# vanilladucky/sde_sampler_lrds

Hardware: AMD Instinct MI355X
Metric: particle-steps/sec (batch*n_steps/wall) + log-Z abs-err vs ref (higher is better)
Workload: dtype f32; 1 GPU; ManyModes d=128 K=4, RDS gmm-ref, VP(0.1,10), EI integrator, 65536 particles x 256 steps per GPU, FourierMLP(4x64) drift, x0 and noise drawn by the engine (Philox); particles_per_gpu=65536, sde_steps=256, parallelism=particle-sharded x1

## Files before the change

### sde_sampler_lrds_amd/csrc/cmcd_inst.hip

```cpp
#include "cmcd_kernel.hpp"

__device__ inline void block_coords(int local, int KB, int& part, int& o, int& i) {
  const int j = local & 7, lane = (local >> 3) & 63, blk = local >> 10;
  part = (local >> 9) & 1;
  const int kb = blk % KB, to = blk / KB;
  o = 16 * to + (lane & 15);
  i = 16 * (2 * kb + (j >> 2)) + 4 * (lane >> 4) + (j & 3);
}
__device__ inline _Float16 split_part(float w, int part) {
  const _Float16 hi = static_cast<_Float16>(w);
  return part == 0 ? hi : static_cast<_Float16>((w - static_cast<float>(hi)) * 2048.0f);
}
__global__ void k_logreg_images(const float* X, const float* y, int n, int dw, int NT, float* image, float* y_pad) {
  const int KB = sd_kb(NT), RKB = sd_lr_row_kb(n);
  const int n_logit = sd_lr_logit_floats(NT, n) * 2, n_grad = sd_lr_grad_floats(NT, n) * 2;
  _Float16* img = reinterpret_cast<_Float16*>(image);
  for (int idx = blockIdx.x * blockDim.x + threadIdx.x; idx < n_logit + n_grad; idx += gridDim.x * blockDim.x) {
    int part, o, i, row, col;
    if (idx < n_logit) {
      block_coords(idx, KB, part, o, i);
      row = o; col = i;
    } else {
      block_coords(idx - n_logit, RKB, part, o, i);
      row = i; col = o;
    }
    float v = 0.0f;
    if (row < n) v = (col < dw) ? X[static_cast<size_t>(row) * dw + col] : (col == dw ? 1.0f : 0.0f);
    img[idx] = split_part(v, part);
    if (idx < 32 * RKB) y_pad[idx] = (idx < n) ? y[idx] : 0.0f;
  }
}
__global__ void k_pack_square(const float* P, const float* loc, int d, int NT, float* out, float* loc_pad) {
  const int KB = sd_kb(NT);
  _Float16* img = reinterpret_cast<_Float16*>(out);
  for (int idx = blockIdx.x * blockDim.x + threadIdx.x; idx < NT * KB * 1024; idx += gridDim.x * blockDim.x) {
    int part, o, i;
    block_coords(idx, KB, part, o, i);
    img[idx] = split_part((o < d && i < d) ? P[static_cast<size_t>(o) * d + i] : 0.0f, part);
    if (idx < 16 * NT) loc_pad[idx] = idx < d ? loc[idx] : 0.0f;
  }
}
int sd_launch_logreg_images(const float* X, const float* y, int n, int dw, int NT, float* image, float* y_pad, hipStream_t s) {
  hipLaunchKernelGGL(k_logreg_images, dim3(96), dim3(256), 0, s, X, y, n, dw, NT, image, y_pad);
  return static_cast<int>(hipGetLastError());
}
int sd_launch_pack_square(const float* P, const float* loc, int d, int NT, float* out, float* loc_pad, hipStream_t s) {
  hipLaunchKernelGGL(k_pack_square, dim3(NT * sd_kb(NT) * 4), dim3(256), 0, s, P, loc, d, NT, out, loc_pad);
  return static_cast<int>(hipGetLastError());
}
```

### sde_sampler_lrds_amd/csrc/prep_kernels.hip

```cpp
#include "sim_device.hpp"
#include "prep_kernels.hpp"

__global__ void __launch_bounds__(256) k_weight_scales(PackArgs a) {
  __shared__ float red[256];
  float* sc = a.out + sd_off_scales(a.NT);
  {
    const int l = blockIdx.x;
    const float* W = l == 0 ? a.w_in : (l == 1 ? a.w_h1 : (l == 2 ? a.w_h2 : a.w_out));
    const int n = (l == 0 || l == 3) ? SD_H * a.d : SD_H * SD_H;
    float m = 0.0f;
    for (int i = threadIdx.x; i < n; i += 256) {
      const float v = __builtin_fabsf(W[i]);
      m = (v <= 3.0e38f) ? fmaxf(m, v) : m;
    }
    red[threadIdx.x] = m;
    __syncthreads();
    for (int s = 128; s > 0; s >>= 1) {
      if (threadIdx.x < s) red[threadIdx.x] = fmaxf(red[threadIdx.x], red[threadIdx.x + s]);
      __syncthreads();
    }
    if (threadIdx.x == 0) {
      const float mx = red[0];
      int e = 0;
      if (mx > 0.0f && (mx < 9.765625e-4f || mx >= 16384.0f)) {
        int ex;
        frexpf(mx, &ex);
        e = 1 - ex;
        e = e > 100 ? 100 : (e < -100 ? -100 : e);
      }
      sc[l] = ldexpf(1.0f, e);
      sc[4 + l] = ldexpf(1.0f, -e);
    }
    __syncthreads();
  }
}

__global__ void k_pack_mlp(PackArgs a) {
  const int NT = a.NT;
  const float* scales = a.transpose ? a.scales : a.out + sd_off_scales(NT);
  const int n_half = sd_lds_weight_floats(NT) * 2;
  const int n_bias = a.transpose ? 0 : 3 * 64 + 16 * NT;
  _Float16* img = reinterpret_cast<_Float16*>(a.out);
  for (int idx = blockIdx.x * blockDim.x + threadIdx.x; idx < n_half + n_bias; idx += gridDim.x * blockDim.x) {
    if (idx < n_half) {
      const int fl = idx >> 1;
      const float* W;
      int n_out, n_in, KB, base, layer;
      if (fl < sd_off_wh1(NT)) {
        W = a.w_in; n_out = SD_H; n_in = a.d; KB = sd_kb(NT); base = sd_off_win(NT); layer = 0;
      } else if (fl < sd_off_wh2(NT)) {
        W = a.w_h1; n_out = SD_H; n_in = SD_H; KB = 2; base = sd_off_wh1(NT); layer = 1;
      } else if (fl < sd_off_wout(NT)) {
        W = a.w_h2; n_out = SD_H; n_in = SD_H; KB = 2; base = sd_off_wh2(NT); layer = 2;
      } else {
        W = a.w_out; n_out = a.d; n_in = SD_H; KB = 2; base = sd_off_wout(NT); layer = 3;
      }
      const int local = idx - 2 * base;
      const int j = local & 7;
      const int lane = (local >> 3) & 63;
      const int part = (local >> 9) & 1;
      const int blk = local >> 10;
      const int kb = blk % KB, to = blk / KB;
      const int o = 16 * to + (lane & 15);
      const int i = 16 * (2 * kb + (j >> 2)) + 4 * (lane >> 4) + (j & 3);
      float w = 0.0f;
      if (o < n_out && i < n_in) {
        if (!a.transpose) {
          w = W[static_cast<size_t>(o) * n_in + i] * scales[layer];
        } else {
          const float* Wt = layer == 0 ? a.w_out : (layer == 1 ? a.w_h2 : (layer == 2 ? a.w_h1 : a.w_in));
          w = Wt[static_cast<size_t>(i) * n_out + o] * scales[3 - layer];
        }
      }
      const _Float16 hi = static_cast<_Float16>(w);
      img[idx] = part == 0 ? hi : static_cast<_Float16>((w - static_cast<float>(hi)) * 2048.0f);
    } else {
      const int b = idx - n_half;
      float v;
      if (b < 64) v = a.b_in[b] * scales[0];
      else if (b < 128) v = a.b_h1[b - 64] * scales[1];
      else if (b < 192) v = a.b_h2[b - 128] * scales[2];
      else v = (b - 192 < a.d) ? a.b_out[b - 192] * scales[3] : 0.0f;
      a.out[sd_off_bias(NT) + b] = v;
    }
  }
}

__device__ inline float gelu_exact(float v) { return (v * 0.5f) * (1.0f + erff(v * 0.70710678118654752440f)); }

__global__ void __launch_bounds__(64) k_time_embed(TimeEmbedArgs a) {
  __shared__ float e[128];
  __shared__ float hbuf[2][64];
  const int k = blockIdx.x, j = threadIdx.x;
  const float t = a.t_direct ? a.t_value : a.coef[static_cast<size_t>(k) * SDENG_NCOEF + a.col];
  const float arg = (a.te.coeff[j] * t) + a.te.phase[j];
  e[j] = sinf(arg);
  e[64 + j] = cosf(arg);
  __syncthreads();
  const float* in = e;
  int n_in = 128, cur = 0;
  for (int l = 0; l < a.te.n_hidden; ++l) {
    const float* W = a.te.w[l] + static_cast<size_t>(j) * n_in;
    float acc = 0.0f;
    for (int i = 0; i < n_in; ++i) acc = __builtin_fmaf(W[i], in[i], acc);
    acc += a.te.b[l][j];
    hbuf[cur][j] = gelu_exact(acc);
    __syncthreads();
    in = hbuf[cur];
    n_in = 64;
    cur ^= 1;
  }
  if (j < a.te.dim_out) {
    const float* W = a.te.w_out + static_cast<size_t>(j) * 64;
    float acc = 0.0f;
    for (int i = 0; i < 64; ++i) acc = __builtin_fmaf(W[i], in[i], acc);
    acc += a.te.b_out[j];
    if (a.clip > 0.0f) acc = clampf(acc, a.clip);
    a.out[static_cast<size_t>(k) * a.te.dim_out + j] = acc;
  }
}

__global__ void __launch_bounds__(128) k_same_var(const float* vars, int K, int d, float* same_var) {
  int differ = 0;
  for (int i = threadIdx.x; i < K * d; i += 128) differ |= vars[i] != vars[i % d];
  differ = __syncthreads_or(differ);
  if (threadIdx.x == 0) same_var[0] = differ ? 0.0f : 1.0f;
}

__global__ void __launch_bounds__(128) k_ref_tables(RefTabArgs a) {
  __shared__ float red[128];
  const int k = blockIdx.x / a.K, c = blockIdx.x % a.K;
  const float S = a.coef[static_cast<size_t>(k) * SDENG_NCOEF + 9];
  const float VA = a.coef[static_cast<size_t>(k) * SDENG_NCOEF + 10];
  const float S2 = a.coef[static_cast<size_t>(k) * SDENG_NCOEF + 11];
  const bool centred = a.centred && a.K == SD_KREG && a.same_var[0] != 0.0f;
  float* tm = a.tab + (static_cast<size_t>(k) * a.K + c) * 2 * a.dpad;
  float* tv = tm + a.dpad;
  float ls = 0.0f, quad = 0.0f;
  for (int f = threadIdx.x; f < a.dpad; f += 128) {
    float mean = 0.0f, iv = 0.0f, cen = 0.0f;
    if (f < a.d) {
      mean = S * a.means[static_cast<size_t>(c) * a.d + f];
      const float var = VA + S2 * a.vars[static_cast<size_t>(c) * a.d + f];
      iv = 1.0f / var;
      ls += logf(var);
      if (centred) {
        float sum = 0.0f;
        for (int j = 0; j < SD_KREG; ++j) sum += a.means[static_cast<size_t>(j) * a.d + f];
        cen = S * (sum * (1.0f / SD_KREG));
      }
    }
    if (centred) {
      const float dm = mean - cen;
      quad = __builtin_fmaf(dm * dm, iv, quad);
      tm[f] = dm * iv;
      tv[f] = c == 0 ? iv : (c == 1 ? cen : 0.0f);
    } else {
      tm[f] = mean;
      tv[f] = iv;
    }
  }
  red[threadIdx.x] = ls;
  __syncthreads();
  for (int s = 64; s > 0; s >>= 1) {
    if (threadIdx.x < s) red[threadIdx.x] += red[threadIdx.x + s];
    __syncthreads();
  }
  const float ls_sum = red[0];
  __syncthreads();
  red[threadIdx.x] = quad;
  __syncthreads();
  for (int s = 64; s > 0; s >>= 1) {
    if (threadIdx.x < s) red[threadIdx.x] += red[threadIdx.x + s];
    __syncthreads();
  }
  if (threadIdx.x == 0) {
    float wsum = 0.0f;
    for (int i = 0; i < a.K; ++i) wsum += a.weights ? a.weights[i] : 1.0f;
    const float w = (a.weights ? a.weights[c] : 1.0f) / wsum;
    float* cs = a.consts + (static_cast<size_t>(k) * a.K + c) * 2;
    cs[0] = 0.5f * ls_sum;
    cs[1] = centred ? logf(w) - 0.5f * red[0] : logf(w);
  }
}

__global__ void __launch_bounds__(256) k_ref_full_tables(RefFullArgs a) {
  __shared__ float invd[128];
  __shared__ float red[256];
  const int k = blockIdx.x / a.K, c = blockIdx.x % a.K;
  const float S = a.coef ? a.coef[static_cast<size_t>(k) * SDENG_NCOEF + 9] : 1.0f;
  const float VA = a.coef ? a.coef[static_cast<size_t>(k) * SDENG_NCOEF + 10] : 0.0f;
  const float S2 = a.coef ? a.coef[static_cast<size_t>(k) * SDENG_NCOEF + 11] : 1.0f;
  const int KB = sd_kb(a.NT);
  const int img_floats = a.NT * KB * 512;
  float ls = 0.0f;
  for (int j = threadIdx.x; j < 128; j += 256) {
    float iv = 0.0f;
    if (j < a.d) {
      const float var = VA + S2 * a.eigvals[static_cast<size_t>(c) * a.d + j];
      iv = 1.0f / var;
      ls += logf(var);
    }
    invd[j] = iv;
  }
  red[threadIdx.x] = ls;
  __syncthreads();
  for (int s = 128; s > 0; s >>= 1) {
    if (threadIdx.x < s) red[threadIdx.x] += red[threadIdx.x + s];
    __syncthreads();
  }
  const size_t blk = static_cast<size_t>(k) * a.K + c;
  if (threadIdx.x == 0) {
    float wsum = 0.0f;
    for (int i = 0; i < a.K; ++i) wsum += a.weights ? a.weights[i] : 1.0f;
    a.consts[blk * 2 + 0] = 0.5f * red[0];
    a.consts[blk * 2 + 1] = logf((a.weights ? a.weights[c] : 1.0f) / wsum);
  }
  for (int f = threadIdx.x; f < a.dpad; f += 256) a.means_out[blk * a.dpad + f] = f < a.d ? S * a.means[static_cast<size_t>(c) * a.d + f] : 0.0f;
  const float* U = a.eigvecs + static_cast<size_t>(c) * a.d * a.d;
  _Float16* img = reinterpret_cast<_Float16*>(a.images + blk * img_floats);
  for (int idx = threadIdx.x; idx < img_floats * 2; idx += 256) {
    const int j8 = idx & 7, lane = (idx >> 3) & 63, part = (idx >> 9) & 1, tb = idx >> 10;
    const int kb = tb % KB, to = tb / KB;
    const int o = 16 * to + (lane & 15);
    const int i = 16 * (2 * kb + (j8 >> 2)) + 4 * (lane >> 4) + (j8 & 3);
    float p = 0.0f;
    if (o < a.d && i < a.d) {
      const float* uo = U + static_cast<size_t>(o) * a.d;
      const float* ui = U + static_cast<size_t>(i) * a.d;
      for (int j = 0; j < a.d; ++j) p = __builtin_fmaf(uo[j] * invd[j], ui[j], p);
    }
    const _Float16 hi = static_cast<_Float16>(p);
    img[idx] = part == 0 ? hi : static_cast<_Float16>((p - static_cast<float>(hi)) * 2048.0f);
  }
}

__global__ void __launch_bounds__(256) k_ref_mm_tables(RefMMArgs a) {
  __shared__ float cbar[128], ivs[128];
  const int k = blockIdx.x;
  const float S = a.coef[static_cast<size_t>(k) * SDENG_NCOEF + 9];
  const float VA = a.coef[static_cast<size_t>(k) * SDENG_NCOEF + 10];
  const float S2 = a.coef[static_cast<size_t>(k) * SDENG_NCOEF + 11];
  const int KBX = sd_kb(a.NT), KBK = (a.kt + 1) / 2;
  for (int f = threadIdx.x; f < 128; f += 256) {
    float c = 0.0f, iv = 0.0f;
    if (f < a.d) {
      for (int j = 0; j < a.K; ++j) c += a.means[static_cast<size_t>(j) * a.d + f];
      c = S * (c / static_cast<float>(a.K));
      iv = 1.0f / (VA + S2 * a.vars[f]);
      if (a.same_var[0] == 0.0f) iv = __builtin_nanf("");
    }
    cbar[f] = c;
    ivs[f] = iv;
    if (f < a.dpad) {
      a.centre[(static_cast<size_t>(k) * 2 + 0) * a.dpad + f] = c;
      a.centre[(static_cast<size_t>(k) * 2 + 1) * a.dpad + f] = iv;
    }
  }
  __syncthreads();
  if (threadIdx.x < 64) {
    const int c = threadIdx.x;
    float b = -INFINITY;
    if (c < a.K) {
      float wsum = 0.0f;
      for (int i = 0; i < a.K; ++i) wsum += a.weights ? a.weights[i] : 1.0f;
      double q = 0.0;
      for (int f = 0; f < a.d; ++f) {
        const float mu = S * a.means[static_cast<size_t>(c) * a.d + f] - cbar[f];
        q += static_cast<double>(mu * mu) * ivs[f];
      }
      b = logf((a.weights ? a.weights[c] : 1.0f) / wsum) - 0.5f * static_cast<float>(q);
    }
    a.consts[static_cast<size_t>(k) * 64 + c] = b;
  }
  const int n_logit = a.kt * KBX * 1024, n_mean = a.NT * KBK * 1024;
  _Float16* img = reinterpret_cast<_Float16*>(a.images + static_cast<size_t>(k) * ((n_logit + n_mean) / 2));
  for (int idx = threadIdx.x; idx < n_logit + n_mean; idx += 256) {
    const bool logit = idx < n_logit;
    const int local = logit ? idx : idx - n_logit, KB = logit ? KBX : KBK;
    const int j8 = local & 7, lane = (local >> 3) & 63, part = (local >> 9) & 1, blk = local >> 10;
    const int kb = blk % KB, to = blk / KB;
    const int o = 16 * to + (lane & 15);
    const int i = 16 * (2 * kb + (j8 >> 2)) + 4 * (lane >> 4) + (j8 & 3);
    const int comp = logit ? o : i, f = logit ? i : o;
    float v = 0.0f;
    if (comp < a.K && f < a.d) {
      const float mu = S * a.means[static_cast<size_t>(comp) * a.d + f] - cbar[f];
      v = logit ? mu * ivs[f] : mu;
    }
    const _Float16 hi = static_cast<_Float16>(v);
    img[idx] = part == 0 ? hi : static_cast<_Float16>((v - static_cast<float>(hi)) * 2048.0f);
  }
}

__global__ void __launch_bounds__(128) k_dist_tables(DistTabArgs a) {
  __shared__ float red[2][128];
  const int c = blockIdx.x;
  float* tm = a.tab + static_cast<size_t>(c) * 2 * a.dpad;
  float* tv = tm + a.dpad;
  float lv = 0.0f, lsig = 0.0f;
  for (int f = threadIdx.x; f < a.dpad; f += 128) {
    float mean = 0.0f, iv = 0.0f;
    if (f < a.d) {
      mean = a.loc[static_cast<size_t>(c) * a.d + f];
      const float sc = a.scale[static_cast<size_t>(c) * a.d + f];
      const float var = sc * sc;
      iv = 1.0f / var;
      lv += logf(var);
      lsig += logf(sc);
    }
    tm[f] = mean;
    tv[f] = iv;
  }
  red[0][threadIdx.x] = lv;
  red[1][threadIdx.x] = lsig;
  __syncthreads();
  for (int s = 64; s > 0; s >>= 1) {
    if (threadIdx.x < s) {
      red[0][threadIdx.x] += red[0][threadIdx.x + s];
      red[1][threadIdx.x] += red[1][threadIdx.x + s];
    }
    __syncthreads();
  }
  if (threadIdx.x == 0) {
    float* cs = a.consts + static_cast<size_t>(c) * 4;
    cs[0] = 0.5f * red[0][0];
    cs[2] = red[1][0] + static_cast<float>(a.d) * 0.91893853320467274178f;
    if (a.weights) {
      float wsum = 0.0f;
      for (int i = 0; i < a.K; ++i) wsum += a.weights[i];
      const float pr = a.weights[c] / wsum;
      cs[1] = logf(pr);
      const float eps = 1.1920928955078125e-07f;
      float lse_m = -INFINITY, lse_s = 0.0f;
      for (int i = 0; i < a.K; ++i) {
        const float li = logf(fminf(fmaxf(a.weights[i] / wsum, eps), 1.0f - eps));
        const float m = fmaxf(lse_m, li);
        lse_s = lse_s * expf(lse_m - m) + expf(li - m);
        lse_m = m;
      }
      const float lc = logf(fminf(fmaxf(pr, eps), 1.0f - eps));
      cs[3] = lc - (lse_m + logf(lse_s));
    } else {
      cs[1] = 0.0f;
      cs[3] = 0.0f;
    }
  }
}

__device__ void gmm_logp_partial(const DistEvalArgs& a, const float* x, int c0, int cs, float& m_run, float& l_run) {
  const DistDev& ds = a.ds;
  m_run = -INFINITY;
  l_run = 0.0f;
  for (int c = c0; c < ds.k; c += cs) {
    const float* tm = ds.tab + static_cast<size_t>(c) * 2 * a.dpad;
    const float* tv = tm + a.dpad;
    double acc = 0.0;
    for (int f = 0; f < a.d; ++f) {
      const float dl = x[f] - tm[f];
      acc += static_cast<double>(dl * dl) * tv[f];
    }
    const float part = static_cast<float>(acc);
    float lp = (-0.5f * part) - ds.consts[4 * c + 2];
    if (ds.kind == SDENG_DIST_GAUSS_DIAG) { m_run = lp; l_run = 1.0f; break; }
    lp += ds.consts[4 * c + 3];
    const float m_new = fmaxf(m_run, lp);
    l_run = l_run * expf(m_run - m_new) + expf(lp - m_new);
    m_run = m_new;
  }
}

__device__ float logreg_loglik_partial(const DistEvalArgs& a, const float* x, int n0, int ns) {
  const DistDev& ds = a.ds;
  const int dw = a.d - 1;
  const float c = x[dw];
  const float eps = 1.1920928955078125e-07f;
  float ll = 0.0f;
  for (int n = n0; n < ds.k; n += ns) {
    const float* Xn = ds.aux0 + static_cast<size_t>(n) * dw;
    float lg = 0.0f;
    for (int f = 0; f < dw; ++f) lg = __builtin_fmaf(Xn[f], x[f], lg);
    lg += c;
    float p = 1.0f / (1.0f + expf(-lg));
    p = fminf(fmaxf(p, ds.p3), 1.0f - ds.p3);
    p = fminf(fmaxf(p, eps), 1.0f - eps);
    const float l2 = logf(p) - log1pf(-p);
    const float y = ds.aux1[n];
    ll -= (1.0f - y) * l2 + (fmaxf(-l2, 0.0f) + log1pf(expf(-fabsf(l2))));
  }
  return ll;
}

__device__ float logreg_logprior(const DistEvalArgs& a, const float* x) {
  const DistDev& ds = a.ds;
  const int dw = a.d - 1;
  float prior = 0.0f;
  const float lws = logf(ds.p0), two_ws2 = 2.0f * (ds.p0 * ds.p0);
  for (int f = 0; f < dw; ++f) prior += (-(x[f] * x[f]) / two_ws2 - lws) - 0.91893853320467274178f;
  const float dc = x[dw] - ds.p1;
  prior += (-(dc * dc) / (2.0f * (ds.p2 * ds.p2)) - logf(ds.p2)) - 0.91893853320467274178f;
  return prior;
}

__device__ float gauss_full_m2_partial(const DistEvalArgs& a, const float* x, int i0, int is) {
  const DistDev& ds = a.ds;
  float m2 = 0.0f;
  for (int i = i0; i < a.d; i += is) {
    float yi = 0.0f;
    const float* Li = ds.aux1 + static_cast<size_t>(i) * a.d;
    for (int j = 0; j <= i; ++j) yi = __builtin_fmaf(Li[j], x[j] - ds.aux0[j], yi);
    m2 = __builtin_fmaf(yi, yi, m2);
  }
  return m2;
}

__device__ float dist_logp_row(const DistEvalArgs& a, const float* x) {
  const int d = a.d;
  const DistDev& ds = a.ds;
  float out = 0.0f;
  if (ds.kind == SDENG_DIST_GMM_DIAG || ds.kind == SDENG_DIST_GAUSS_DIAG) {
    float m_run, l_run;
    gmm_logp_partial(a, x, 0, 1, m_run, l_run);
    out = m_run + logf(l_run);
  } else if (ds.kind == SDENG_DIST_ISO_GAUSS) {
    double acc = 0.0;
    for (int f = 0; f < d; ++f) {
      const float dl = x[f] - ds.p0;
      acc += static_cast<double>(dl) * dl;
    }
    const float part = static_cast<float>(acc);
    out = ds.p2 - (0.5f * part) / ds.p3;
  } else if (ds.kind == SDENG_DIST_PHI4) {
    const float coef = ds.p0 * static_cast<float>(d);
    double gsum = 0.0, vsum = 0.0;
    float prev = 0.0f;
    for (int f = 0; f < d; ++f) {
      const float xv = x[f];
      const float dl = xv - prev;
      gsum += (dl * dl) * 0.5f;
      const float om = 1.0f - xv * xv;
      vsum += (om * om) * 0.25f + ds.p1 * xv;
      prev = xv;
    }
    gsum += (prev * prev) * 0.5f;
    const float grad = static_cast<float>(gsum), V = static_cast<float>(vsum);
    out = (-ds.p2) * (grad * coef + V / coef);
  } else if (ds.kind == SDENG_DIST_GAUSS_FULL) {
    const float m2 = gauss_full_m2_partial(a, x, 0, 1);
    out = -0.5f * (static_cast<float>(d) * 1.8378770664093453f + m2) - ds.p0;
  } else if (ds.kind == SDENG_DIST_LOGREG) {
    out = logreg_loglik_partial(a, x, 0, 1) + logreg_logprior(a, x);
  }
  else if (ds.kind == SDENG_DIST_RINGS) {
    const float r = sqrtf(x[0] * x[0] + x[1] * x[1]);
    float wsum = 0.0f;
    for (int k = 0; k < ds.k; ++k) wsum += ds.aux1[k];
    const float ls = logf(ds.p0), var = ds.p0 * ds.p0;
    float m_run = -INFINITY, l_run = 0.0f;
    for (int k = 0; k < ds.k; ++k) {
      const float dl = r - ds.aux0[k];
      const float lp = ((-(dl * dl) / (2.0f * var)) - ls) - 0.91893853320467274178f + logf(ds.aux1[k] / wsum);
      const float m_new = fmaxf(m_run, lp);
      l_run = l_run * expf(m_run - m_new) + expf(lp - m_new);
      m_run = m_new;
    }
    out = ((m_run + logf(l_run)) - 1.8378770664093453f) - logf(r);
  } else if (ds.kind == SDENG_DIST_CHECKERBOARD) {
    out = -INFINITY;
    for (int k = 0; k < ds.k; ++k) {
      const float* lo = ds.aux0 + 2 * k;
      const float* hi = ds.aux1 + 2 * k;
      const bool in = (lo[0] <= x[0]) & (hi[0] > x[0]) & (lo[1] <= x[1]) & (hi[1] > x[1]);
      out = in ? ds.tab[k] : out;
    }
  }
  if (ds.clip > 0.0f) out = clampf(out, ds.clip);
  return out;
}

__device__ void dist_score_row(const DistEvalArgs& a, const float* x, float* sc) {
  const int d = a.d;
  const DistDev& ds = a.ds;
  if (ds.kind == SDENG_DIST_GMM_DIAG) {
    float m_run = -INFINITY, l_run = 0.0f;
    for (int f = 0; f < d; ++f) sc[f] = 0.0f;
    for (int c = 0; c < ds.k; ++c) {
      const float* tm = ds.tab + static_cast<size_t>(c) * 2 * a.dpad;
      const float* tv = tm + a.dpad;
      float part = 0.0f;
      for (int f = 0; f < d; ++f) {
        const float dl = x[f] - tm[f];
        part = __builtin_fmaf(dl * dl, tv[f], part);
      }
      float lp = ((-0.5f * part) - ds.p0) - ds.consts[4 * c + 0];
      lp = ds.consts[4 * c + 1] + lp;
      const float m_new = fmaxf(m_run, lp);
      const float so = expf(m_run - m_new), pk = expf(lp - m_new);
      l_run = l_run * so + pk;
      m_run = m_new;
      for (int f = 0; f < d; ++f) sc[f] = __builtin_fmaf(pk, (tm[f] - x[f]) * tv[f], sc[f] * so);
    }
    const float inv = 1.0f / l_run;
    for (int f = 0; f < d; ++f) sc[f] *= inv;
  } else if (ds.kind == SDENG_DIST_GAUSS_DIAG) {
    for (int f = 0; f < d; ++f) sc[f] = -((x[f] - ds.tab[f]) * ds.tab[a.dpad + f]);
  } else if (ds.kind == SDENG_DIST_ISO_GAUSS) {
    for (int f = 0; f < d; ++f) sc[f] = (ds.p0 - x[f]) / (ds.p1 * ds.p1);
  } else if (ds.kind == SDENG_DIST_PHI4) {
    const float coef = ds.p0 * static_cast<float>(d);
    for (int f = 0; f < d; ++f) {
      const float xv = x[f];
      const float xl = f > 0 ? x[f - 1] : 0.0f, xr = f < d - 1 ? x[f + 1] : 0.0f;
      float g = (ds.p1 - xv * (1.0f - xv * xv)) / coef;
      g = g + coef * ((2.0f * xv - xr) - xl);
      sc[f] = (-ds.p2) * g;
    }
  } else if (ds.kind == SDENG_DIST_GAUSS_FULL) {
    for (int i = 0; i < d; ++i) {
      float acc = 0.0f;
      const float* Pi = ds.tab + static_cast<size_t>(i) * d;
      for (int j = 0; j < d; ++j) acc = __builtin_fmaf(Pi[j], x[j] - ds.aux0[j], acc);
      sc[i] = -acc;
    }
  } else if (ds.kind == SDENG_DIST_LOGREG) {
    const int dw = d - 1;
    const float c = x[dw];
    const float eps = 1.1920928955078125e-07f;
    for (int f = 0; f < dw; ++f) sc[f] = -x[f] / (ds.p0 * ds.p0);
    float gc = -(c - ds.p1) / (ds.p2 * ds.p2);
    for (int n = 0; n < ds.k; ++n) {
      const float* Xn = ds.aux0 + static_cast<size_t>(n) * dw;
      float lg = 0.0f;
      for (int f = 0; f < dw; ++f) lg = __builtin_fmaf(Xn[f], x[f], lg);
      lg += c;
      const float p = 1.0f / (1.0f + expf(-lg));
      const float pc = fminf(fmaxf(p, ds.p3), 1.0f - ds.p3);
      const float pcc = fminf(fmaxf(pc, eps), 1.0f - eps);
      const bool pass = (p >= ds.p3) && (p <= 1.0f - ds.p3) && (pc >= eps) && (pc <= 1.0f - eps);
      const float l2 = logf(pcc) - log1pf(-pcc);
      const float sg = 1.0f / (1.0f + expf(-l2));
      float r = (ds.aux1[n] - sg) * (1.0f / pcc + 1.0f / (1.0f - pcc)) * (p * (1.0f - p));
      r = pass ? r : 0.0f;
      for (int f = 0; f < dw; ++f) sc[f] = __builtin_fmaf(r, Xn[f], sc[f]);
      gc += r;
    }
    sc[dw] = gc;
  } else if (ds.kind == SDENG_DIST_RINGS) {
    const f32x4 r = rings_score(f32x4{x[0], x[1], 0.0f, 0.0f}, ds, 0);
    sc[0] = r[0];
    sc[1] = r[1];
  } else if (ds.kind == SDENG_DIST_CHECKERBOARD) {
    sc[0] = 0.0f;
    sc[1] = 0.0f;
  }
}

#define SD_EVAL_ROWS 64
#define SD_EVAL_THREADS 256
#define SD_EVAL_RED_FLOATS (SD_EVAL_THREADS * 2)

__device__ inline const float* stage_rows(const float* x, int B, int d, float* sh) {
  const int row0 = blockIdx.x * SD_EVAL_ROWS, stride = d | 1, tid = threadIdx.x;
  const int rows = B - row0 < SD_EVAL_ROWS ? B - row0 : SD_EVAL_ROWS;
  const float* src = x + static_cast<size_t>(row0) * d;
  if ((d & 3) == 0) {
    const int d4 = d >> 2, n4 = rows * d4;
    const float inv = 1.0f / static_cast<float>(d4);
    const f32x4* src4 = reinterpret_cast<const f32x4*>(src);
    for (int base = tid; base < n4; base += 4 * SD_EVAL_THREADS) {
      f32x4 v[4];
#pragma unroll
      for (int j = 0; j < 4; ++j) {
        const int i4 = base + j * SD_EVAL_THREADS;
        v[j] = i4 < n4 ? src4[i4] : f32x4{0.0f, 0.0f, 0.0f, 0.0f};
      }
#pragma unroll
      for (int j = 0; j < 4; ++j) {
        const int i4 = base + j * SD_EVAL_THREADS;
        if (i4 < n4) {
          const int r = static_cast<int>((static_cast<float>(i4) + 0.5f) * inv);
          float* dst = sh + r * stride + 4 * (i4 - r * d4);
          dst[0] = v[j][0]; dst[1] = v[j][1]; dst[2] = v[j][2]; dst[3] = v[j][3];
        }
      }
    }
  } else {
    const int n = rows * d;
    const float inv = 1.0f / static_cast<float>(d);
    for (int base = tid; base < n; base += 8 * SD_EVAL_THREADS) {
      float v[8];
#pragma unroll
      for (int j = 0; j < 8; ++j) {
        const int i = base + j * SD_EVAL_THREADS;
        v[j] = i < n ? src[i] : 0.0f;
      }
#pragma unroll
      for (int j = 0; j < 8; ++j) {
        const int i = base + j * SD_EVAL_THREADS;
        if (i < n) {
          const int r = static_cast<int>((static_cast<float>(i) + 0.5f) * inv);
          sh[r * stride + (i - r * d)] = v[j];
        }
      }
    }
  }
  __syncthreads();
  return sh + (tid & 63) * stride;
}

__device__ float dist_logp_block(const DistEvalArgs& a, const float* x, float* red) {
  const int w = threadIdx.x >> 6, lane = threadIdx.x & 63;
  constexpr int NW = SD_EVAL_THREADS / 64;
  const DistDev& ds = a.ds;
  if (ds.kind == SDENG_DIST_GMM_DIAG && ds.k > 1) {
    float m_run, l_run;
    gmm_logp_partial(a, x, w, NW, m_run, l_run);
    red[2 * threadIdx.x] = m_run;
    red[2 * threadIdx.x + 1] = l_run;
    __syncthreads();
    float out = 0.0f;
    if (w == 0) {
      for (int j = 1; j < NW; ++j) {
        const float mj = red[2 * (64 * j + lane)], lj = red[2 * (64 * j + lane) + 1];
        const float m_new = fmaxf(m_run, mj);
        l_run = l_run * expf(m_run - m_new) + lj * expf(mj - m_new);
        m_run = m_new;
      }
      out = m_run + logf(l_run);
      if (ds.clip > 0.0f) out = clampf(out, ds.clip);
    }
    __syncthreads();
    return out;
  }
  if (ds.kind == SDENG_DIST_LOGREG) {
    const float ll = logreg_loglik_partial(a, x, w, NW);
    red[threadIdx.x] = ll;
    __syncthreads();
    float out = 0.0f;
    if (w == 0) {
      float sum = ll;
      for (int j = 1; j < NW; ++j) sum += red[64 * j + lane];
      out = sum + logreg_logprior(a, x);
      if (ds.clip > 0.0f) out = clampf(out, ds.clip);
    }
    __syncthreads();
    return out;
  }
  if (ds.kind == SDENG_DIST_GAUSS_FULL) {
    const float m2 = gauss_full_m2_partial(a, x, w, NW);
    red[threadIdx.x] = m2;
    __syncthreads();
    float out = 0.0f;
    if (w == 0) {
      float sum = m2;
      for (int j = 1; j < NW; ++j) sum += red[64 * j + lane];
      out = -0.5f * (static_cast<float>(a.d) * 1.8378770664093453f + sum) - ds.p0;
      if (ds.clip > 0.0f) out = clampf(out, ds.clip);
    }
    __syncthreads();
    return out;
  }
  return w == 0 ? dist_logp_row(a, x) : 0.0f;
}

__global__ void __launch_bounds__(SD_EVAL_THREADS) k_dist_eval(DistEvalArgs a) {
  extern __shared__ float sh[];
  float* red = sh + SD_EVAL_ROWS * (a.d | 1);
  const float* x = stage_rows(a.x, a.B, a.d, sh);
  const int row = blockIdx.x * SD_EVAL_ROWS + (threadIdx.x & 63);
  const bool writer = threadIdx.x < 64 && row < a.B;
  if (a.logp_out) {
    const float lp = dist_logp_block(a, x, red);
    if (writer) a.logp_out[row] = lp;
  }
  if (a.score_out && writer) dist_score_row(a, x, a.score_out + static_cast<size_t>(row) * a.d);
}

constexpr int sd_move_rows(int move) { return move == SD_MOVE_RWMH ? 2 : 5; }
__device__ inline void tempered_eval(const MovesArgs& a, float w, const float* y, float* g_out, float* tmp, float& lp_out) {
  const bool both = a.prior.ds.kind != SDENG_DIST_NONE;
  const float lp1 = dist_logp_row(a.target, y);
  dist_score_row(a.target, y, g_out);
  if (!both) {
    lp_out = lp1;
    return;
  }
  const float lp0 = dist_logp_row(a.prior, y);
  dist_score_row(a.prior, y, tmp);
  lp_out = (1.0f - w) * lp0 + w * lp1;
  for (int f = 0; f < a.d; ++f) g_out[f] = (1.0f - w) * tmp[f] + w * g_out[f];
}

template <int MOVE>
__global__ void __launch_bounds__(64) k_chain_moves(MovesArgs a, int chains_per_block) {
  constexpr bool LANGEVIN = MOVE == SD_MOVE_LANGEVIN;
  constexpr uint32_t Z_STREAM = LANGEVIN ? 2u : 6u, U_STREAM = Z_STREAM + 1u;
  extern __shared__ float sh[];
  const int tid = threadIdx.x, d = a.d, stride = d | 1;
  const int chain = blockIdx.x * chains_per_block + tid;
  if (tid >= chains_per_block || chain >= a.B) return;
  const bool ula = LANGEVIN && a.ula;
  float* xr = sh + (tid * sd_move_rows(MOVE) + 0) * stride;
  float* gr = xr + stride;
  float* pr = xr + (LANGEVIN ? 2 : 1) * stride;
  float* gp = pr + stride;
  float* tmp = gp + stride;
  for (int f = 0; f < d; ++f) {
    xr[f] = a.x[static_cast<size_t>(chain) * d + f];
    if constexpr (LANGEVIN) gr[f] = a.grad[static_cast<size_t>(chain) * d + f];
  }
  float lp = a.lp[chain], step = a.step[chain], acc = 0.0f, last = 1.0f;
  const float w = LANGEVIN && a.t ? a.t[chain] : 1.0f;
  const uint32_t cidx = static_cast<uint32_t>(a.chain0 + chain);
  const float log_target = a.target_acc > 0.0f ? logf(a.target_acc) : 0.0f;
  for (int m = 0; m < a.K; ++m) {
    const float sd = sqrtf(2.0f * step);
    for (int f0 = 0; f0 < d; f0 += 4) {
      f32x4 z;
      if (a.z) {
        for (int r = 0; r < 4; ++r) z[r] = f0 + r < d ? a.z[(static_cast<size_t>(m) * a.B + chain) * d + f0 + r] : 0.0f;
      } else {
        z = philox_normal4(cidx, static_cast<uint32_t>(m), static_cast<uint32_t>(f0 >> 2), Z_STREAM, a.seed_lo, a.seed_hi);
      }
      for (int r = 0; r < 4 && f0 + r < d; ++r) {
        if constexpr (LANGEVIN) pr[f0 + r] = sd * z[r] + (xr[f0 + r] + step * gr[f0 + r]);
        else pr[f0 + r] = xr[f0 + r] + step * z[r];
      }
    }
    float lp_p, log_acc = 0.0f;
    if constexpr (LANGEVIN) {
      tempered_eval(a, w, pr, gp, tmp, lp_p);
      if (!ula) {
        float qf = 0.0f, qb = 0.0f;
        for (int f = 0; f < d; ++f) {
          const float df = pr[f] - (xr[f] + step * gr[f]);
          const float db = xr[f] - (pr[f] + step * gp[f]);
          qf += df * df;
          qb += db * db;
        }
        const float var = 2.0f * step;
        const float joint_prop = lp_p - (-0.5f * qf) / var, joint_orig = lp - (-0.5f * qb) / var;
        log_acc = joint_prop - joint_orig;
      }
    } else {
      lp_p = dist_logp_row(a.target, pr);
      log_acc = lp_p - lp;
    }
    bool accept = true;
    if (!ula) {
      float uu;
      if (a.u) {
        uu = a.u[static_cast<size_t>(m) * a.B + chain];
      } else {
        uint32_t r4[4];
        philox4x32_10(cidx, 0u, static_cast<uint32_t>(m), U_STREAM, a.seed_lo, a.seed_hi, r4);
        uu = u01(r4[0]);
      }
      accept = logf(uu) < log_acc;
    }
    if (accept) {
      for (int f = 0; f < d; ++f) {
        xr[f] = pr[f];
        if constexpr (LANGEVIN) gr[f] = gp[f];
      }
      lp = lp_p;
    }
    if (!ula && a.target_acc > 0.0f) {
      if (log_acc - log_target > 0.04879016416943205f) step = step * 1.01f;
      if (log_target - log_acc > 0.05129329438755058f) step = step / 1.01f;
    }
    if (!ula) last = expf(fminf(0.0f, log_acc));
    if (m >= a.keep_from) {
      if (!ula) acc += last;
      if (a.samples) {
        float* dst = a.samples + (static_cast<size_t>(m - a.keep_from) * a.B + chain) * d;
        for (int f = 0; f < d; ++f) dst[f] = xr[f];
      }
    }
  }
  for (int f = 0; f < d; ++f) {
    a.x[static_cast<size_t>(chain) * d + f] = xr[f];
    if constexpr (LANGEVIN) a.grad[static_cast<size_t>(chain) * d + f] = gr[f];
  }
  a.lp[chain] = lp;
  a.step[chain] = step;
  if (a.acc_sum) a.acc_sum[chain] = acc;
  if (a.acc_last) a.acc_last[chain] = last;
}

__global__ void __launch_bounds__(SD_EVAL_THREADS) k_terminal(TerminalArgs a) {
  extern __shared__ float sh[];
  float* red = sh + SD_EVAL_ROWS * (a.d | 1);
  const float* x = stage_rows(a.x, a.B, a.d, sh);
  const int row = blockIdx.x * SD_EVAL_ROWS + (threadIdx.x & 63);
  float term = 0.0f;
  if (a.use_ref) {
    DistEvalArgs e;
    e.ds = a.ref; e.B = a.B; e.d = a.d; e.dpad = a.dpad;
    term = dist_logp_block(e, x, red);
  }
  if (a.use_target) {
    DistEvalArgs e;
    e.ds = a.target; e.B = a.B; e.d = a.d; e.dpad = a.dpad;
    term = term - dist_logp_block(e, x, red);
  }
  if (threadIdx.x < 64 && row < a.B) a.rnd[row] += term;
}

__device__ inline float block_reduce(float v, float* sh, bool is_max) {
  const int lane = threadIdx.x & 63, w = threadIdx.x >> 6;
  for (int o = 32; o > 0; o >>= 1) {
    const float t = __shfl_xor(v, o, 64);
    v = is_max ? fmaxf(v, t) : v + t;
  }
  if (lane == 0) sh[w] = v;
  __syncthreads();
  float r = sh[0];
  for (int i = 1; i < (blockDim.x >> 6); ++i) r = is_max ? fmaxf(r, sh[i]) : r + sh[i];
  __syncthreads();
  return r;
}

__global__ void __launch_bounds__(256) k_logz_partial(const float* rnd, long long B, float* partials) {
  __shared__ float sh[4];
  float mx = -INFINITY, s1 = 0.0f;
  for (long long i = blockIdx.x * 256ll + threadIdx.x; i < B; i += gridDim.x * 256ll) {
    const float v = -rnd[i];
    mx = fmaxf(mx, v);
    s1 += v;
  }
  mx = block_reduce(mx, sh, true);
  s1 = block_reduce(s1, sh, false);
  if (threadIdx.x == 0) {
    partials[2 * blockIdx.x + 0] = mx;
    partials[2 * blockIdx.x + 1] = s1;
  }
}

__global__ void __launch_bounds__(256) k_logz_partial2(const float* rnd, long long B, const float* partials, int nb,
                                                      float* partials2) {
  __shared__ float sh[4];
  float mx = -INFINITY, s1 = 0.0f;
  for (int i = 0; i < nb; ++i) {
    mx = fmaxf(mx, partials[2 * i]);
    s1 += partials[2 * i + 1];
  }
  const float mean = s1 / static_cast<float>(B);
  float se = 0.0f, se2 = 0.0f, sv = 0.0f;
  for (long long i = blockIdx.x * 256ll + threadIdx.x; i < B; i += gridDim.x * 256ll) {
    const float v = -rnd[i];
    const float ex = expf(v - mx);
    se += ex;
    se2 = __builtin_fmaf(ex, ex, se2);
    const float dv = v - mean;
    sv = __builtin_fmaf(dv, dv, sv);
  }
  se = block_reduce(se, sh, false);
  se2 = block_reduce(se2, sh, false);
  sv = block_reduce(sv, sh, false);
  if (threadIdx.x == 0) {
    partials2[3 * blockIdx.x + 0] = se;
    partials2[3 * blockIdx.x + 1] = se2;
    partials2[3 * blockIdx.x + 2] = sv;
  }
}

__global__ void k_logz_final(const float* partials, const float* partials2, int nb, long long B, float* stats) {
  if (threadIdx.x != 0 || blockIdx.x != 0) return;
  float mx = -INFINITY, s1 = 0.0f, se = 0.0f, se2 = 0.0f, sv = 0.0f;
  for (int i = 0; i < nb; ++i) {
    mx = fmaxf(mx, partials[2 * i]);
    s1 += partials[2 * i + 1];
    se += partials2[3 * i];
    se2 += partials2[3 * i + 1];
    sv += partials2[3 * i + 2];
  }
  const float fB = static_cast<float>(B);
  stats[0] = s1 / fB;
  stats[1] = (__builtin_isinf(mx) ? mx : (mx + logf(se))) - logf(fB);
  stats[2] = B > 1 ? sv / (fB - 1.0f) : 0.0f;
  stats[3] = (se * se) / se2 / fB;
  stats[4] = mx;
  stats[5] = se;
  stats[6] = se2;
  stats[7] = s1;
}

__global__ void k_softmax_weights(const float* rnd, long long B, const float* stats, float* w) {
  const long long i = blockIdx.x * static_cast<long long>(blockDim.x) + threadIdx.x;
  if (i >= B) return;
  w[i] = expf((-rnd[i]) - stats[4]) / stats[5];
}

__global__ void k_philox(unsigned seed_lo, unsigned seed_hi, int step, long long particle0, int B, int d, unsigned stream_id,
                         float* out) {
  const int nj = (d + 3) / 4;
  const long long idx = blockIdx.x * static_cast<long long>(blockDim.x) + threadIdx.x;
  if (idx >= static_cast<long long>(B) * nj) return;
  const int row = static_cast<int>(idx / nj), jb = static_cast<int>(idx % nj);
  const f32x4 z = philox_normal4(static_cast<uint32_t>(particle0 + row), static_cast<uint32_t>(step) + blockIdx.y, static_cast<uint32_t>(jb),
                                 stream_id, seed_lo, seed_hi);
  float* o = out + static_cast<size_t>(blockIdx.y) * B * d;
  for (int e = 0; e < 4; ++e)
    if (4 * jb + e < d) o[static_cast<size_t>(row) * d + 4 * jb + e] = z[e];
}

__global__ void k_sample_x0(X0Dev q, unsigned seed_lo, unsigned seed_hi, long long particle0, int B, int d, float* out) {
  const int nj = (d + 3) / 4;
  const long long idx = blockIdx.x * static_cast<long long>(blockDim.x) + threadIdx.x;
  if (idx >= static_cast<long long>(B) * nj) return;
  const int row = static_cast<int>(idx / nj), jb = static_cast<int>(idx % nj);
  const f32x4 x = x0_quad(q, static_cast<uint32_t>(particle0 + row), jb, d, seed_lo, seed_hi);
  for (int e = 0; e < 4; ++e)
    if (4 * jb + e < d) out[static_cast<size_t>(row) * d + 4 * jb + e] = x[e];
}
#define SD_X0_FULL_ROWS 64
__global__ void __launch_bounds__(256) k_sample_x0_full(const float* loc, const float* L, unsigned seed_lo, unsigned seed_hi, long long particle0,
                                                       int B, int d, float* out) {
  extern __shared__ float sh[];
  const int nj = (d + 3) / 4, zs = 4 * nj + 1, ls = d | 1;
  float* z = sh;
  float* Lt = sh + SD_X0_FULL_ROWS * zs;
  const int row0 = blockIdx.x * SD_X0_FULL_ROWS;
  for (int i = threadIdx.x; i < d * d; i += 256) {
    const int f = i / d, j = i - f * d;
    Lt[j * ls + f] = L[i];
  }
  for (int i = threadIdx.x; i < SD_X0_FULL_ROWS * nj; i += 256) {
    const int r = i / nj, jb = i - r * nj;
    const f32x4 v = philox_normal4(static_cast<uint32_t>(particle0 + row0 + r), 0u, static_cast<uint32_t>(jb), SD_X0_STREAM, seed_lo, seed_hi);
    for (int e = 0; e < 4; ++e) z[r * zs + 4 * jb + e] = v[e];
  }
  __syncthreads();
  const int rows = B - row0 < SD_X0_FULL_ROWS ? B - row0 : SD_X0_FULL_ROWS;
  for (int i = threadIdx.x; i < rows * d; i += 256) {
    const int r = i / d, f = i - r * d;
    float acc = 0.0f;
    for (int j = 0; j <= f; ++j) acc = __builtin_fmaf(Lt[j * ls + f], z[r * zs + j], acc);
    out[static_cast<size_t>(row0) * d + i] = loc[f] + acc;
  }
}
int sd_launch_sample_x0(const sdeng_dist& ds, unsigned lo, unsigned hi, long long p0, int B, int d, float* out, hipStream_t s) {
  if (ds.kind == SDENG_DIST_GAUSS_FULL) {
    const size_t lds = (static_cast<size_t>(SD_X0_FULL_ROWS) * (4 * ((d + 3) / 4) + 1) + static_cast<size_t>(d) * (d | 1)) * sizeof(float);
    if (lds > 160 * 1024) return static_cast<int>(hipErrorInvalidValue);
    if (lds > 64 * 1024) (void)hipFuncSetAttribute(reinterpret_cast<const void*>(k_sample_x0_full), hipFuncAttributeMaxDynamicSharedMemorySize, static_cast<int>(lds));
    hipLaunchKernelGGL(k_sample_x0_full, dim3((B + SD_X0_FULL_ROWS - 1) / SD_X0_FULL_ROWS), dim3(256), lds, s, ds.loc, ds.aux, lo, hi, p0, B, d, out);
  } else {
    X0Dev q;
    q.kind = ds.kind; q.loc = ds.loc; q.scale = ds.scale; q.p0 = ds.p0; q.p1 = ds.p1;
    const long long n = static_cast<long long>(B) * ((d + 3) / 4);
    hipLaunchKernelGGL(k_sample_x0, dim3(static_cast<unsigned>((n + 255) / 256)), dim3(256), 0, s, q, lo, hi, p0, B, d, out);
  }
  return static_cast<int>(hipGetLastError());
}

int sd_launch_pack(const PackArgs& a, hipStream_t s) {
  const int total = sd_lds_weight_floats(a.NT) * 2 + (a.transpose ? 0 : 3 * 64 + 16 * a.NT);
  if (!a.transpose) hipLaunchKernelGGL(k_weight_scales, dim3(4), dim3(256), 0, s, a);
  hipLaunchKernelGGL(k_pack_mlp, dim3((total + 255) / 256), dim3(256), 0, s, a);
  return static_cast<int>(hipGetLastError());
}
int sd_launch_time_embed(const TimeEmbedArgs& a, int N, hipStream_t s) {
  hipLaunchKernelGGL(k_time_embed, dim3(N), dim3(64), 0, s, a);
  return static_cast<int>(hipGetLastError());
}
int sd_launch_ref_tables(const RefTabArgs& a, int N, hipStream_t s) {
  hipLaunchKernelGGL(k_same_var, dim3(1), dim3(128), 0, s, a.vars, a.K, a.d, a.same_var);
  hipLaunchKernelGGL(k_ref_tables, dim3(N * a.K), dim3(128), 0, s, a);
  return static_cast<int>(hipGetLastError());
}
int sd_launch_ref_full_tables(const RefFullArgs& a, int N, hipStream_t s) {
  hipLaunchKernelGGL(k_ref_full_tables, dim3(N * a.K), dim3(256), 0, s, a);
  return static_cast<int>(hipGetLastError());
}
int sd_launch_ref_mm_tables(const RefMMArgs& a, int N, hipStream_t s) {
  hipLaunchKernelGGL(k_same_var, dim3(1), dim3(128), 0, s, a.vars, a.K, a.d, a.same_var);
  hipLaunchKernelGGL(k_ref_mm_tables, dim3(N), dim3(256), 0, s, a);
  return static_cast<int>(hipGetLastError());
}
int sd_launch_dist_tables(const DistTabArgs& a, hipStream_t s) {
  hipLaunchKernelGGL(k_dist_tables, dim3(a.K), dim3(128), 0, s, a);
  return static_cast<int>(hipGetLastError());
}
int sd_launch_dist_eval(const DistEvalArgs& a, hipStream_t s) {
  hipLaunchKernelGGL(k_dist_eval, dim3((a.B + SD_EVAL_ROWS - 1) / SD_EVAL_ROWS), dim3(SD_EVAL_THREADS), (SD_EVAL_ROWS * (a.d | 1) + SD_EVAL_RED_FLOATS) * sizeof(float), s, a);
  return static_cast<int>(hipGetLastError());
}
int sd_launch_moves(const MovesArgs& a, int move, hipStream_t s) {
  const size_t row_bytes = static_cast<size_t>(sd_move_rows(move)) * (a.d | 1) * sizeof(float);
  int cpb = 64;
  while (cpb > 8 && cpb * row_bytes > 150 * 1024) cpb /= 2;
  return sd_launch_kernel(move == SD_MOVE_RWMH ? k_chain_moves<SD_MOVE_RWMH> : k_chain_moves<SD_MOVE_LANGEVIN>, (a.B + cpb - 1) / cpb, 64,
                          cpb * row_bytes, s, a, cpb);
}
int sd_launch_terminal(const TerminalArgs& a, hipStream_t s) {
  hipLaunchKernelGGL(k_terminal, dim3((a.B + SD_EVAL_ROWS - 1) / SD_EVAL_ROWS), dim3(SD_EVAL_THREADS), (SD_EVAL_ROWS * (a.d | 1) + SD_EVAL_RED_FLOATS) * sizeof(float), s, a);
  return static_cast<int>(hipGetLastError());
}
int sd_launch_logz(const float* rnd, long long B, float* stats, float* weights, float* scratch, hipStream_t s) {
  int nb = static_cast<int>((B + 256 * 8 - 1) / (256 * 8));
  if (nb > SD_LOGZ_MAX_BLOCKS) nb = SD_LOGZ_MAX_BLOCKS;
  if (nb < 1) nb = 1;
  float* p1 = scratch;
  float* p2 = scratch + 2 * SD_LOGZ_MAX_BLOCKS;
  hipLaunchKernelGGL(k_logz_partial, dim3(nb), dim3(256), 0, s, rnd, B, p1);
  hipLaunchKernelGGL(k_logz_partial2, dim3(nb), dim3(256), 0, s, rnd, B, p1, nb, p2);
  hipLaunchKernelGGL(k_logz_final, dim3(1), dim3(64), 0, s, p1, p2, nb, B, stats);
  if (weights) hipLaunchKernelGGL(k_softmax_weights, dim3(static_cast<unsigned>((B + 255) / 256)), dim3(256), 0, s, rnd, B, stats, weights);
  return static_cast<int>(hipGetLastError());
}
int sd_launch_philox(unsigned lo, unsigned hi, int step, int n_steps, long long p0, int B, int d, unsigned stream_id, float* out, hipStream_t s) {
  const long long n = static_cast<long long>(B) * ((d + 3) / 4);
  for (int done = 0; done < n_steps; done += 65535) {
    const int chunk = n_steps - done < 65535 ? n_steps - done : 65535;
    hipLaunchKernelGGL(k_philox, dim3(static_cast<unsigned>((n + 255) / 256), chunk), dim3(256), 0, s, lo, hi, step + done, p0, B, d, stream_id,
                       out + static_cast<size_t>(done) * B * d);
  }
  return static_cast<int>(hipGetLastError());
}
```

### sde_sampler_lrds_amd/csrc/prep_kernels.hpp

```cpp
#pragma once
#include "sim_common.hpp"
#include "../../include/sdeng.h"

#define SD_LOGZ_MAX_BLOCKS 1024

struct PackArgs {
  int NT, d;
  const float *w_in, *b_in, *w_h1, *b_h1, *w_h2, *b_h2, *w_out, *b_out;
  float* out;
  int transpose;
  const float* scales;
};

struct TimeEmbedArgs {
  sdeng_time_embed te;
  const float* coef;
  int col;
  int t_direct;
  float t_value;
  float clip;
  float* out;
};

struct RefTabArgs {
  int K, d, dpad;
  const float* coef;
  const float *means, *vars, *weights;
  float* tab;
  float* consts;
  float* same_var;
  int centred;
};

struct RefFullArgs {
  int K, d, dpad, NT;
  const float* coef;
  const float *means, *eigvals, *eigvecs, *weights;
  float* images;
  float* means_out;
  float* consts;
};

struct RefMMArgs {
  int K, d, dpad, NT, kt;
  const float* coef;
  const float *means, *vars, *weights;
  float* images;
  float* centre;
  float* consts;
  float* same_var;
};

struct DistTabArgs {
  int K, d, dpad;
  const float *loc, *scale, *weights;
  float* tab;
  float* consts;
};

struct DistEvalArgs {
  DistDev ds;
  int B, d, dpad;
  const float* x;
  float* logp_out;
  float* score_out;
};

enum { SD_MOVE_LANGEVIN = 0, SD_MOVE_RWMH = 1 };
struct MovesArgs {
  DistEvalArgs prior, target;
  int B, d, K, keep_from, ula;
  float target_acc;
  const float* t;
  float *x, *lp, *grad, *step;
  const float *z, *u;
  unsigned seed_lo, seed_hi;
  long long chain0;
  float* samples;
  float* acc_sum;
  float* acc_last;
};
int sd_launch_moves(const MovesArgs& a, int move, hipStream_t s);

struct TerminalArgs {
  DistDev ref, target;
  int use_ref, use_target;
  int B, d, dpad;
  const float* x;
  float* rnd;
};

int sd_launch_pack(const PackArgs& a, hipStream_t s);
int sd_launch_time_embed(const TimeEmbedArgs& a, int N, hipStream_t s);
int sd_launch_ref_tables(const RefTabArgs& a, int N, hipStream_t s);
int sd_launch_ref_full_tables(const RefFullArgs& a, int N, hipStream_t s);
int sd_launch_dist_tables(const DistTabArgs& a, hipStream_t s);
int sd_launch_dist_eval(const DistEvalArgs& a, hipStream_t s);
int sd_launch_terminal(const TerminalArgs& a, hipStream_t s);
int sd_launch_logz(const float* rnd, long long B, float* stats, float* weights, float* scratch, hipStream_t s);
int sd_launch_philox(unsigned lo, unsigned hi, int step, int n_steps, long long p0, int B, int d, unsigned stream_id, float* out, hipStream_t s);
int sd_launch_sample_x0(const sdeng_dist& ds, unsigned lo, unsigned hi, long long p0, int B, int d, float* out, hipStream_t s);
int sd_launch_ref_mm_tables(const RefMMArgs& a, int N, hipStream_t s);
```

### sde_sampler_lrds_amd/csrc/sdeng_api.hip

```cpp
#include <hip/hip_runtime.h>

#include <algorithm>
#include <cmath>
#include <cstdarg>
#include <cstdio>
#include <cstring>
#include <cstdlib>

#include "../../include/sdeng.h"
#include "prep_kernels.hpp"
#include "sim_kernel.hpp"
#include "cmcd_kernel.hpp"
#include "grad_kernel.hpp"
#include "cmcd_adjoint_kernel.hpp"
#include "metric_kernels.hpp"
#include "tilted_kernel.hpp"

int sd_launch_logreg_images(const float* X, const float* y, int n, int dw, int NT, float* image, float* y_pad, hipStream_t s);
int sd_launch_pack_square(const float* P, const float* loc, int d, int NT, float* out, float* loc_pad, hipStream_t s);

static thread_local char g_err[512] = "";
static int fail(int code, const char* fmt, ...) {
  va_list ap;
  va_start(ap, fmt);
  vsnprintf(g_err, sizeof(g_err), fmt, ap);
  va_end(ap);
  return code;
}
#define SD_HIP(expr)                                                                  \
  do {                                                                                \
    int e_ = (expr);                                                                  \
    if (e_ != 0) return fail(SDENG_E_HIP, "%s failed: %s", #expr, hipGetErrorString(static_cast<hipError_t>(e_))); \
  } while (0)
#define SD_TRY(expr)      \
  do {                    \
    int rc_ = (expr);     \
    if (rc_) return rc_;  \
  } while (0)

extern "C" int sdeng_abi_version(void) { return SDENG_ABI_VERSION; }
extern "C" const char* sdeng_last_error(void) { return g_err; }

static inline size_t align64(size_t n_floats) { return (n_floats + 63) & ~static_cast<size_t>(63); }
static inline int pad16(int d) { return 16 * ((d + 15) / 16); }
static inline float half_d_log_2pi(int d) { return static_cast<float>(0.5 * d * std::log(2.0 * M_PI)); }
struct Seed {
  unsigned lo, hi;
};
static inline Seed split_seed(uint64_t seed) { return {static_cast<unsigned>(seed & 0xFFFFFFFFull), static_cast<unsigned>(seed >> 32)}; }
static int check_abi(const sdeng_desc* d) {
  return d->abi_version == SDENG_ABI_VERSION ? 0 : fail(SDENG_E_INVALID, "ABI version %d, library has %d", d->abi_version, SDENG_ABI_VERSION);
}
static int check_lerp_prior(const sdeng_desc* d) {
  if (d->net.ctrl_kind == SDENG_CTRL_LERP && d->prior.kind != SDENG_DIST_ISO_GAUSS)
    return fail(SDENG_E_UNSUPPORTED, "LerpCtrl needs an IsotropicGauss prior (kind %d given)", d->prior.kind);
  return 0;
}
static int ref_components(const sdeng_desc* d) {
  return d->ref.kind == SDENG_REF_NONE ? 0 : (d->ref.kind == SDENG_REF_GAUSS_DIAG ? 1 : d->ref.k);
}
static bool score_like(int ctrl_kind) {
  return ctrl_kind == SDENG_CTRL_SCORE || ctrl_kind == SDENG_CTRL_LERP || ctrl_kind == SDENG_CTRL_CANCEL_DRIFT;
}
static int in_loop_score(int target_kind) {
  if (target_kind == SDENG_DIST_GMM_DIAG || target_kind == SDENG_DIST_RINGS) return SC_GMM;
  if (target_kind == SDENG_DIST_PHI4) return SC_PHI4;
  if (target_kind == SDENG_DIST_LOGREG) return SC_LOGREG;
  return -1;
}

struct KernelKey {
  int fam, nt, p[4];
  sd_launcher fn;
};
static int select_kernel(KernelKey& k, int fam, int nt, int p0 = 0, int p1 = 0, int p2 = 0, int p3 = 0) {
  static const char* const kFamily[] = {"k_simulate", "k_ctrl_forward", "k_simulate_split", "k_euler", "k_simulate_cmcd", "k_ctrl_vjp", "k_kl_adjoint", "k_cmcd_kl_adjoint"};
  k = KernelKey{fam, nt, {p0, p1, p2, p3}, nullptr};
  const uint32_t key = sd_key(fam, nt, p0, p1, p2, p3);
  const SdKernelEntry* end = sd_registry + sd_registry_size;
  const SdKernelEntry* e = std::lower_bound(sd_registry, end, key, [](const SdKernelEntry& x, uint32_t v) { return x.key < v; });
  if (e == end || e->key != key)
    return fail(SDENG_E_UNSUPPORTED, "no kernel instance %s<NT=%d, %d, %d, %d, %d>", kFamily[fam], nt, p0, p1, p2, p3);
  k.fn = e->fn;
  return 0;
}
static int launch_timed(const sdeng_desc* d, const KernelKey& k, const void* args, hipStream_t s) {
  if (d->ev_start) SD_HIP(hipEventRecord(static_cast<hipEvent_t>(d->ev_start), s));
  SD_HIP(k.fn(args, s));
  if (d->ev_stop) SD_HIP(hipEventRecord(static_cast<hipEvent_t>(d->ev_stop), s));
  return 0;
}

static int tiles_exact(int d) { return (d + 15) / 16; }
static int tiles_of(const sdeng_desc* d) {
  const int nt = tiles_exact(d->d);
  return (d->ref.kind == SDENG_REF_GMM_FULL && (nt == 5 || nt == 7)) ? nt + 1 : nt;
}

static size_t dist_floats(const sdeng_dist& ds, int dpad) {
  if (ds.kind == SDENG_DIST_GMM_DIAG) return align64(static_cast<size_t>(ds.k) * 2 * dpad) + align64(static_cast<size_t>(ds.k) * 4);
  if (ds.kind == SDENG_DIST_GAUSS_DIAG) return align64(2 * dpad) + align64(4);
  return 0;
}

static bool split_eligible(const sdeng_desc* d, int DT) {
  return (d->flags & SDENG_FLAG_SPLIT_TILES) && d->B <= 8192 && DT >= 5 && d->net.ctrl_kind == SDENG_CTRL_CLIPPED &&
         (d->form == SDENG_FORM_LIN || d->form == SDENG_FORM_EM) && !d->noise_in &&
         (d->ref.kind == SDENG_REF_NONE || d->ref.kind == SDENG_REF_GAUSS_DIAG || (d->ref.kind == SDENG_REF_GMM_DIAG && d->ref.k <= 4));
}

static int share_room(int DT) { return (160 * 1024 - static_cast<int>(sizeof(float)) * sd_lds_weight_floats(DT)) / 2 / static_cast<int>(sizeof(float)); }
static int mm_piece(int K, int DT) {
  const int kt = (K + 15) / 16;
  return std::max(kt * sd_kb(DT), DT * ((kt + 1) / 2)) * 512;
}
static bool use_mm(const sdeng_desc* d, int DT) {
  static const bool allow = [] { const char* e = getenv("SDENG_REF_MM"); return !(e && e[0] == '0'); }();
  if (!allow || d->ref.kind != SDENG_REF_GMM_DIAG || !d->ref.shared_var) return false;
  const int K = d->ref.k;
  if (K <= 4 && K * 2 * 16 * DT <= SD_REFTAB_FLOATS) return false;
  if (K > 64) return false;
  if (d->net.ctrl_kind != SDENG_CTRL_CLIPPED || (d->form != SDENG_FORM_LIN && d->form != SDENG_FORM_EM)) return false;
  const int piece = mm_piece(K, DT);
  return piece <= share_room(DT) && piece <= sd_share_buf_floats(SD_SHARE_MAX);
}

struct Layout {
  size_t wpack, temb, stheta, ref_tab, ref_mean, ref_consts, target, ref_dist, prior, rnd_init, trash, logz, cmcd, x0, total;
};

static bool make_layout(const sdeng_desc* d, Layout& L) {
  if (!d || d->d < 1 || d->d > 128 || d->N < 0 || d->B < 0) return false;
  const int DT = tiles_of(d), dpad = 16 * DT;
  size_t o = 0;
  L.wpack = o; o += align64(sd_pack_floats(DT));
  L.temb = o; o += align64(static_cast<size_t>(d->N + 1) * SD_H);
  L.stheta = o; o += align64(d->N + 1);
  const int K = ref_components(d);
  if (d->ref.kind == SDENG_REF_GMM_FULL) {
    L.ref_tab = o; o += align64(static_cast<size_t>(d->N) * K * DT * sd_kb(DT) * 512 + 256);
    L.ref_mean = o; o += align64(static_cast<size_t>(d->N) * K * dpad);
  } else if (use_mm(d, DT)) {
    const int kt = (K + 15) / 16;
    L.ref_tab = o; o += align64(static_cast<size_t>(d->N) * (kt * sd_kb(DT) + DT * ((kt + 1) / 2)) * 512 + 1024);
    L.ref_mean = o; o += align64(static_cast<size_t>(d->N) * 2 * dpad);
  } else {
    L.ref_tab = o; o += align64(static_cast<size_t>(d->N) * K * 2 * dpad);
    L.ref_mean = o;
  }
  L.ref_consts = o; o += align64(static_cast<size_t>(d->N) * (K * 2 > 64 ? K * 2 : 64) + 1);
  L.target = o; o += dist_floats(d->target, dpad);
  L.ref_dist = o; o += dist_floats(d->ref_dist, dpad);
  L.prior = o; o += dist_floats(d->prior, dpad);
  L.rnd_init = o; o += align64(d->B);
  L.trash = o; o += align64((SD_WAVES_MAX > SD_WAVES ? SD_WAVES_MAX : SD_WAVES) * 64 * 4);
  L.logz = o; o += align64(5 * SD_LOGZ_MAX_BLOCKS);
  L.cmcd = o;
  {
    const bool lr_used = d->target.kind == SDENG_DIST_LOGREG && d->target.k > 0 &&
                         (d->form == SDENG_FORM_CMCD || d->form == SDENG_FORM_CMCD_EUBO || d->net.ctrl_kind != SDENG_CTRL_CLIPPED);
    const int n = lr_used ? d->target.k : 0;
    o += align64(sd_lr_floats(DT, n)) + align64(32 * sd_lr_row_kb(n));
    if (d->form == SDENG_FORM_CMCD || d->form == SDENG_FORM_CMCD_EUBO) o += align64(DT * sd_kb(DT) * 512) + align64(16 * DT);
  }
  L.x0 = o;
  if (!d->x_in && !d->x0_out) o += align64(static_cast<size_t>(d->B) * d->d);
  L.total = o;
  return true;
}

static bool slot_target(const sdeng_desc* d, sdeng_desc& out) {
  if (!d || d->target.kind != SDENG_DIST_GMM_FULL) return false;
  out = *d;
  out.ref.kind = SDENG_REF_GMM_FULL;
  out.ref.k = d->target.k;
  out.ref.means_init = d->target.loc;
  out.ref.vars_init = d->target.scale;
  out.ref.eigvecs = d->target.aux;
  out.ref.weights = d->target.w;
  out.ref.shared_var = 0;
  memset(&out.target, 0, sizeof(out.target));
  return true;
}
static int check_slot_target(const sdeng_desc* d) {
  if (d->ref.kind != SDENG_REF_NONE)
    return fail(SDENG_E_UNSUPPORTED, "full-covariance mixture target of a score control together with a reference drift (ref.kind %d)", d->ref.kind);
  if (!score_like(d->net.ctrl_kind))
    return fail(SDENG_E_UNSUPPORTED, "SDENG_DIST_GMM_FULL is the target of a Score / Lerp / CancelDrift control only (ctrl_kind %d)", d->net.ctrl_kind);
  if (d->form != SDENG_FORM_LIN && d->form != SDENG_FORM_EM)
    return fail(SDENG_E_UNSUPPORTED, "full-covariance mixture target of a score control: forward forms only (form %d)", d->form);
  if (d->flags & (SDENG_FLAG_TERM_TARGET | SDENG_FLAG_REMOVE_REF))
    return fail(SDENG_E_UNSUPPORTED, "SDENG_DIST_GMM_FULL: no log-density kernel (FLAG_TERM_TARGET) and no RemoveReferenceCtrl");
  if (d->target.k < 1 || !d->target.loc || !d->target.scale || !d->target.aux)
    return fail(SDENG_E_INVALID, "SDENG_DIST_GMM_FULL: null means / eigenvalues / eigenvectors or k < 1");
  return 0;
}

extern "C" size_t sdeng_workspace_bytes(const sdeng_desc* desc) {
  Layout L;
  sdeng_desc ds;
  if (slot_target(desc, ds)) desc = &ds;
  if (!make_layout(desc, L)) return 0;
  return L.total * sizeof(float);
}

static int check_dist(const sdeng_dist& in, int d) {
  switch (in.kind) {
    case SDENG_DIST_NONE:
    case SDENG_DIST_ISO_GAUSS:
    case SDENG_DIST_PHI4:
      return 0;
    case SDENG_DIST_GMM_DIAG:
    case SDENG_DIST_GAUSS_DIAG: {
      const int K = in.kind == SDENG_DIST_GMM_DIAG ? in.k : 1;
      if (K < 1 || !in.loc || !in.scale || (in.kind == SDENG_DIST_GMM_DIAG && !in.w))
        return fail(SDENG_E_INVALID, "diagonal Gaussian/mixture needs loc, scale%s", in.kind == SDENG_DIST_GMM_DIAG ? ", w and k >= 1" : "");
      return 0;
    }
    case SDENG_DIST_GAUSS_FULL:
      return (in.loc && in.scale && in.w) ? 0 : fail(SDENG_E_INVALID, "GAUSS_FULL needs loc, precision, inverse Cholesky factor");
    case SDENG_DIST_LOGREG:
      return (in.loc && in.scale && in.k >= 1) ? 0 : fail(SDENG_E_INVALID, "LOGREG needs X, y and k >= 1 rows");
    case SDENG_DIST_RINGS:
      if (d != 2) return fail(SDENG_E_INVALID, "RINGS is two-dimensional (d = %d)", d);
      if (!in.loc || !in.w || in.k < 1 || in.k > 8 || !(in.p0 > 0.0f)) return fail(SDENG_E_INVALID, "RINGS needs radii, weights, 1 <= k <= 8, scale > 0");
      return 0;
    case SDENG_DIST_CHECKERBOARD:
      if (d != 2) return fail(SDENG_E_INVALID, "CHECKERBOARD is two-dimensional (d = %d)", d);
      if (!in.loc || !in.scale || !in.w || in.k < 1) return fail(SDENG_E_INVALID, "CHECKERBOARD needs the low / high corner tables, the per-square constants and k >= 1");
      return 0;
    default:
      return fail(SDENG_E_UNSUPPORTED, "unknown distribution kind %d", in.kind);
  }
}
static int build_dist(const sdeng_dist& in, int d, int dpad, float* ws, DistDev& out, hipStream_t s) {
  SD_TRY(check_dist(in, d));
  memset(&out, 0, sizeof(out));
  out.kind = in.kind;
  out.k = in.k;
  out.p0 = in.p0; out.p1 = in.p1; out.p2 = in.p2; out.p3 = in.p3;
  out.clip = in.clip;
  switch (in.kind) {
    case SDENG_DIST_GMM_DIAG:
    case SDENG_DIST_GAUSS_DIAG: {
      DistTabArgs t;
      t.K = in.kind == SDENG_DIST_GMM_DIAG ? in.k : 1; t.d = d; t.dpad = dpad;
      t.loc = in.loc; t.scale = in.scale; t.weights = in.kind == SDENG_DIST_GMM_DIAG ? in.w : nullptr;
      t.tab = ws; t.consts = ws + align64(static_cast<size_t>(t.K) * 2 * dpad);
      SD_HIP(sd_launch_dist_tables(t, s));
      out.k = t.K;
      out.tab = t.tab; out.consts = t.consts;
      out.p0 = half_d_log_2pi(d);
      return 0;
    }
    case SDENG_DIST_GAUSS_FULL: out.aux0 = in.loc; out.tab = in.scale; out.aux1 = in.w; return 0;
    case SDENG_DIST_LOGREG: out.aux0 = in.loc; out.aux1 = in.scale; return 0;
    case SDENG_DIST_RINGS: out.aux0 = in.loc; out.aux1 = in.w; return 0;
    case SDENG_DIST_CHECKERBOARD: out.aux0 = in.loc; out.aux1 = in.scale; out.tab = in.w; return 0;
    default: return 0;
  }
}
static int dist_eval(const DistDev& ds, int B, int d, int dpad, const float* x, float* logp, float* score, hipStream_t s) {
  DistEvalArgs e;
  e.ds = ds; e.B = B; e.d = d; e.dpad = dpad; e.x = x; e.logp_out = logp; e.score_out = score;
  SD_HIP(sd_launch_dist_eval(e, s));
  return 0;
}
static int terminal(const sdeng_desc* d, int dpad, const DistDev& ref, const DistDev& target, bool use_ref, bool use_target, const float* x,
                    float* rnd, hipStream_t s) {
  TerminalArgs t;
  t.ref = ref; t.target = target; t.use_ref = use_ref; t.use_target = use_target;
  t.B = d->B; t.d = d->d; t.dpad = dpad; t.x = x; t.rnd = rnd;
  SD_HIP(sd_launch_terminal(t, s));
  return 0;
}

static int check_net(const sdeng_net& n) {
  if (!n.w_in || !n.b_in || !n.w_h1 || !n.b_h1 || !n.w_h2 || !n.b_h2 || !n.w_out || !n.b_out)
    return fail(SDENG_E_INVALID, "drift net: null weight pointer");
  const sdeng_time_embed& te = n.t_embed;
  if (!te.coeff || !te.phase || te.n_hidden != 1 || te.dim_out != SD_H || !te.w[0] || !te.b[0] || !te.w_out || !te.b_out)
    return fail(SDENG_E_UNSUPPORTED, "drift net time embedding must be TimeEmbed(num_layers=2, channels=64)");
  if (n.ctrl_kind != SDENG_CTRL_CLIPPED) {
    const sdeng_time_embed& sm = n.score_model;
    if (sm.n_hidden > 0) {
      if (sm.n_hidden > 4 || sm.dim_out != 1 || !sm.coeff || !sm.phase || !sm.w_out || !sm.b_out)
        return fail(SDENG_E_UNSUPPORTED, "score_model must be TimeEmbed(dim_out=1, num_layers<=5)");
      for (int i = 0; i < sm.n_hidden; ++i)
        if (!sm.w[i] || !sm.b[i]) return fail(SDENG_E_INVALID, "score_model: null weight pointer");
    }
  }
  return 0;
}
static int pack_net(const sdeng_desc* d, int DT, float* out, float* out_t, hipStream_t s) {
  const sdeng_net& n = d->net;
  PackArgs pk;
  pk.NT = DT; pk.d = d->d;
  pk.w_in = n.w_in; pk.b_in = n.b_in; pk.w_h1 = n.w_h1; pk.b_h1 = n.b_h1; pk.w_h2 = n.w_h2; pk.b_h2 = n.b_h2; pk.w_out = n.w_out; pk.b_out = n.b_out;
  pk.out = out; pk.transpose = 0; pk.scales = nullptr;
  SD_HIP(sd_launch_pack(pk, s));
  if (out_t) {
    pk.out = out_t; pk.transpose = 1; pk.scales = out + sd_off_scales(DT);
    SD_HIP(sd_launch_pack(pk, s));
  }
  return 0;
}
static int embed_times(const sdeng_desc* d, int n_times, bool t_direct, float t_value, float* temb, float* stheta_ws, const float** stheta,
                       hipStream_t s) {
  TimeEmbedArgs te;
  te.te = d->net.t_embed; te.coef = d->coef; te.col = 0; te.t_direct = t_direct; te.t_value = t_value; te.clip = 0.0f; te.out = temb;
  SD_HIP(sd_launch_time_embed(te, n_times, s));
  *stheta = nullptr;
  if (d->net.ctrl_kind != SDENG_CTRL_CLIPPED && d->net.score_model.n_hidden > 0) {
    te.te = d->net.score_model;
    te.clip = d->net.clip_model;
    te.out = stheta_ws;
    SD_HIP(sd_launch_time_embed(te, n_times, s));
    *stheta = stheta_ws;
  }
  return 0;
}
static int prepare_net(const sdeng_desc* d, const Layout& L, float* ws, int DT, SimArgs& a, hipStream_t s, int n_times, bool t_direct,
                       float t_value) {
  SD_TRY(pack_net(d, DT, ws + L.wpack, nullptr, s));
  a.wpack = ws + L.wpack;
  if (n_times > 0) SD_TRY(embed_times(d, n_times, t_direct, t_value, ws + L.temb, ws + L.stheta, &a.stheta, s));
  a.temb = ws + L.temb;
  a.ctrl_kind = d->net.ctrl_kind;
  a.clip_model = d->net.clip_model;
  a.clip_score = d->net.clip_score;
  a.scale_score = d->net.scale_score;
  return 0;
}

static int score_kind(const sdeng_desc* d, int& sc) {
  sc = SC_NONE;
  if (d->net.ctrl_kind == SDENG_CTRL_CLIPPED) return 0;
  if (!score_like(d->net.ctrl_kind)) return fail(SDENG_E_UNSUPPORTED, "unknown ctrl_kind %d", d->net.ctrl_kind);
  sc = in_loop_score(d->target.kind);
  if (sc < 0) return fail(SDENG_E_UNSUPPORTED, "ScoreCtrl/LerpCtrl: no in-loop score kernel for target kind %d", d->target.kind);
  return check_lerp_prior(d);
}

static int prepare_logreg(const sdeng_desc* d, const Layout& L, float* ws, int DT, SimArgs& a, hipStream_t s, float** next) {
  const int n = d->target.k;
  float* image = ws + L.cmcd;
  float* y_pad = image + align64(sd_lr_floats(DT, n));
  *next = y_pad + align64(32 * sd_lr_row_kb(n));
  SD_HIP(sd_launch_logreg_images(d->target.loc, d->target.scale, n, d->d - 1, DT, image, y_pad, s));
  a.lr.image = image; a.lr.y_pad = y_pad; a.lr.n_rows = n;
  a.lr.in_lds = static_cast<size_t>(cmcd_lds_floats(DT, n)) * sizeof(float) <= 160 * 1024 ? 1 : 0;
  a.lr.inv_w_scale2 = 1.0f / (d->target.p0 * d->target.p0); a.lr.c_mean = d->target.p1; a.lr.inv_c_scale2 = 1.0f / (d->target.p2 * d->target.p2);
  const float thr = d->target.p3, eps = 1.1920928955078125e-07f;
  a.lr.p_lo = thr > eps ? thr : eps;
  a.lr.p_hi = (1.0f - thr) < (1.0f - eps) ? (1.0f - thr) : (1.0f - eps);
  return 0;
}

static int check_x0_dist(const sdeng_desc* d) {
  const sdeng_dist& q = d->x0_dist;
  if (d->form == SDENG_FORM_EUBO || d->form == SDENG_FORM_CMCD_EUBO)
    return fail(SDENG_E_INVALID, "the noising loops start from samples of the TARGET: x_in is required");
  if (q.kind == SDENG_DIST_ISO_GAUSS) return 0;
  if (q.kind == SDENG_DIST_GAUSS_DIAG) return q.loc ? 0 : fail(SDENG_E_INVALID, "x0_dist GAUSS_DIAG needs loc (scale may be NULL: x0 = loc)");
  if (q.kind == SDENG_DIST_GAUSS_FULL) return (q.loc && q.aux) ? 0 : fail(SDENG_E_INVALID, "x0_dist GAUSS_FULL needs loc and the Cholesky factor (aux)");
  return fail(SDENG_E_UNSUPPORTED, "x_in == NULL: no sampler for x0_dist kind %d (ISO_GAUSS, GAUSS_DIAG, GAUSS_FULL)", q.kind);
}

struct SimPlan {
  const sdeng_desc* d;
  sdeng_desc slot;
  bool in_slot;
  Layout L;
  int DT, rf, sc;
  KernelKey k;
};

static int plan_cmcd(SimPlan& p) {
  const sdeng_desc* d = p.d;
  const bool logreg = d->target.kind == SDENG_DIST_LOGREG;
  const bool toy = d->target.kind == SDENG_DIST_RINGS || d->target.kind == SDENG_DIST_CHECKERBOARD;
  if (!logreg && !toy && d->target.kind != SDENG_DIST_GMM_DIAG && d->target.kind != SDENG_DIST_GAUSS_DIAG && d->target.kind != SDENG_DIST_PHI4)
    return fail(SDENG_E_UNSUPPORTED, "CMCD kernel: target must be LOGREG, GMM_DIAG, GAUSS_DIAG, PHI4, RINGS or CHECKERBOARD (kind %d)", d->target.kind);
  if (logreg && p.DT > 4) return fail(SDENG_E_UNSUPPORTED, "CMCD kernel: logistic regression with d <= 64 (got %d)", d->d);
  if (logreg && d->target.k < 1) return fail(SDENG_E_INVALID, "CMCD kernel: logistic regression without data rows");
  if (d->prior.kind != SDENG_DIST_GAUSS_FULL && d->prior.kind != SDENG_DIST_ISO_GAUSS && d->prior.kind != SDENG_DIST_GAUSS_DIAG)
    return fail(SDENG_E_UNSUPPORTED, "CMCD kernel: prior must be GAUSS_FULL, GAUSS_DIAG or ISO_GAUSS (kind %d)", d->prior.kind);
  if (d->net.ctrl_kind != SDENG_CTRL_CLIPPED && d->net.ctrl_kind != SDENG_CTRL_SCORE)
    return fail(SDENG_E_UNSUPPORTED, "CMCD kernel: ClippedCtrl or ScoreCtrl");
  if (!(d->flags & SDENG_FLAG_INIT_LOGP) || !(d->flags & SDENG_FLAG_TERM_TARGET))
    return fail(SDENG_E_UNSUPPORTED, "CMCD kernel implements the eval path (rnd0 = log p_prior, terminal -log pi)");
  SD_TRY(check_net(d->net));
  SD_TRY(check_dist(d->target, d->d));
  SD_TRY(check_dist(d->prior, d->d));
  const bool eubo = d->form == SDENG_FORM_CMCD_EUBO;
  if (eubo && d->target.kind != SDENG_DIST_GMM_DIAG && d->target.kind != SDENG_DIST_GAUSS_DIAG && !toy)
    return fail(SDENG_E_UNSUPPORTED, "CMCD compute_eubo kernels: diagonal Gaussian / mixture, rings or checkerboard targets (kind %d)", d->target.kind);
  const int tgt = d->target.kind == SDENG_DIST_RINGS ? CT_RINGS : d->target.kind == SDENG_DIST_CHECKERBOARD ? CT_ZERO : eubo ? CT_GMM :
                  d->target.kind == SDENG_DIST_PHI4 ? CT_PHI4 : logreg ? CT_LOGREG : CT_GMM;
  return select_kernel(p.k, SD_FAM_CMCD, p.DT, tgt, eubo, (d->noise_in || d->xs_out) ? 1 : 0);
}

static int plan_euler(SimPlan& p) {
  const sdeng_desc* d = p.d;
  if (d->form != SDENG_FORM_EM) return fail(SDENG_E_UNSUPPORTED, "CTRL_NONE (no drift net) runs the Euler-Maruyama form only (form %d given)", d->form);
  if (d->ref.kind != SDENG_REF_NONE) return fail(SDENG_E_UNSUPPORTED, "CTRL_NONE with a reference drift");
  if (d->flags & (SDENG_FLAG_TERM_REF | SDENG_FLAG_TERM_TARGET | SDENG_FLAG_INIT_LOGP))
    return fail(SDENG_E_UNSUPPORTED, "CTRL_NONE carries no log-weight: terminal / initial cost flags are not accepted");
  SD_TRY(check_dist(d->target, d->d));
  const int sc = d->target.kind == SDENG_DIST_NONE ? SC_NONE : in_loop_score(d->target.kind);
  if (sc < 0 || sc == SC_LOGREG) return fail(SDENG_E_UNSUPPORTED, "Langevin drift: no in-loop score kernel for target kind %d", d->target.kind);
  return select_kernel(p.k, SD_FAM_EULER, p.DT, sc);
}

static int plan_sim(SimPlan& p) {
  const sdeng_desc* d = p.d;
  const int DT = p.DT;
  SD_TRY(check_net(d->net));
  if (p.in_slot) {
    p.sc = SC_REFSLOT;
    SD_TRY(check_lerp_prior(d));
  } else {
    SD_TRY(score_kind(d, p.sc));
  }
  const int sc = p.sc;
  int& rf = p.rf;
  if (d->ref.kind == SDENG_REF_GAUSS_DIAG || d->ref.kind == SDENG_REF_GMM_DIAG) {
    const int K = ref_components(d);
    rf = d->ref.kind == SDENG_REF_GAUSS_DIAG ? RF_GAUSS : ((K <= 4 && K * 2 * 16 * DT <= SD_REFTAB_FLOATS) ? RF_GMM : RF_GMM_BIG);
    if (K < 1 || !d->ref.means_init || !d->ref.vars_init) return fail(SDENG_E_INVALID, "reference: null means/vars or k < 1");
    if (use_mm(d, DT)) rf = RF_GMM_MM;
  } else if (d->ref.kind == SDENG_REF_GMM_FULL) {
    rf = RF_GMM_FULL;
    if (d->ref.k < 1 || !d->ref.means_init || !d->ref.vars_init || !d->ref.eigvecs)
      return fail(SDENG_E_INVALID, "full-covariance reference: null means / eigenvalues / eigenvectors or k < 1");
  } else if (d->ref.kind != SDENG_REF_NONE) {
    return fail(SDENG_E_UNSUPPORTED, "reference kind %d", d->ref.kind);
  }
  SD_TRY(check_dist(d->target, d->d));
  SD_TRY(check_dist(d->ref_dist, d->d));
  SD_TRY(check_dist(d->prior, d->d));
  const bool eubo = d->form == SDENG_FORM_EUBO, init_logp = d->flags & SDENG_FLAG_INIT_LOGP;
  if (init_logp && !eubo && d->prior.kind == SDENG_DIST_NONE) return fail(SDENG_E_INVALID, "FLAG_INIT_LOGP without a prior");
  if ((d->flags & SDENG_FLAG_TERM_REF) && d->ref_dist.kind == SDENG_DIST_NONE) return fail(SDENG_E_INVALID, "FLAG_TERM_REF without ref_dist");
  if ((d->flags & SDENG_FLAG_TERM_TARGET) && d->target.kind == SDENG_DIST_NONE) return fail(SDENG_E_INVALID, "FLAG_TERM_TARGET without target");
  if ((d->flags & SDENG_FLAG_REMOVE_REF) && (sc == SC_NONE || sc == SC_LOGREG || sc == SC_REFSLOT || rf == RF_NONE || rf == RF_GMM_MM || eubo))
    return fail(SDENG_E_UNSUPPORTED, "FLAG_REMOVE_REF (RemoveReferenceCtrl): forward forms with a Score / Lerp / CancelDrift control on a mixture or "
                                     "phi^4 target and a Gaussian / mixture reference (ctrl_kind %d, ref.kind %d, form %d)",
                d->net.ctrl_kind, d->ref.kind, d->form);
  if (eubo) {
    if (rf == RF_NONE && sc == SC_NONE)
      return fail(SDENG_E_UNSUPPORTED, "compute_eubo kernels: a reference drift, or no reference with a Score/LerpCtrl "
                                       "(ref.kind %d, ctrl_kind %d)", d->ref.kind, d->net.ctrl_kind);
    if (sc == SC_LOGREG) return fail(SDENG_E_UNSUPPORTED, "compute_eubo kernels: no logistic-regression control score");
    if (init_logp && d->prior.kind == SDENG_DIST_NONE) return fail(SDENG_E_INVALID, "FLAG_INIT_LOGP without a prior");
  } else if (sc == SC_LOGREG) {
    if (rf != RF_NONE) return fail(SDENG_E_UNSUPPORTED, "in-loop logistic-regression score together with a reference drift");
    if (DT > 4) return fail(SDENG_E_UNSUPPORTED, "in-loop logistic-regression score: d <= 64 (got %d)", d->d);
  }
  if (rf == RF_GMM_MM && (sc != SC_NONE || eubo))
    return fail(SDENG_E_UNSUPPORTED, "matrix-pipe mixture reference: forward forms with a ClippedCtrl only");
  const bool pert = d->flags & (SDENG_FLAG_CTRL_NOISE | SDENG_FLAG_CTRL_DROPOUT);
  if (split_eligible(d, DT) && (rf == RF_NONE || rf == RF_GAUSS || rf == RF_GMM)) return select_kernel(p.k, SD_FAM_SPLIT, DT, rf, d->form, pert);
  return select_kernel(p.k, SD_FAM_SIM, DT, rf, sc, d->form, pert ? 2 : (d->noise_in || d->xs_out) ? 1 : 0);
}

static int plan_simulate(const sdeng_desc* d, SimPlan& p) {
  if (!d) return fail(SDENG_E_INVALID, "null descriptor");
  SD_TRY(check_abi(d));
  p.in_slot = d->target.kind == SDENG_DIST_GMM_FULL;
  if (p.in_slot) {
    SD_TRY(check_slot_target(d));
    slot_target(d, p.slot);
    d = &p.slot;
  }
  p.d = d;
  if (!make_layout(d, p.L)) return fail(SDENG_E_INVALID, "bad sizes: B=%d d=%d N=%d (need 1 <= d <= 128)", d->B, d->d, d->N);
  if (d->B == 0) return 0;
  if ((!d->coef && d->N > 0) || !d->x_out || !d->rnd_out) return fail(SDENG_E_INVALID, "null coef/x_out/rnd_out");
  if (!d->x_in) SD_TRY(check_x0_dist(d));
  if (static_cast<long long>(d->B) * d->d >= (1ll << 31)) return fail(SDENG_E_UNSUPPORTED, "B*d >= 2^31");
  if (d->form != SDENG_FORM_LIN && d->form != SDENG_FORM_EM && d->form != SDENG_FORM_CMCD && d->form != SDENG_FORM_EUBO &&
      d->form != SDENG_FORM_CMCD_EUBO)
    return fail(SDENG_E_INVALID, "unknown form %d", d->form);
  if ((d->flags & (SDENG_FLAG_CTRL_NOISE | SDENG_FLAG_CTRL_DROPOUT)) &&
      ((d->form != SDENG_FORM_LIN && d->form != SDENG_FORM_EM) || d->net.ctrl_kind == SDENG_CTRL_NONE))
    return fail(SDENG_E_UNSUPPORTED, "FLAG_CTRL_NOISE / FLAG_CTRL_DROPOUT: forward forms (LIN / EM) with a drift net only (form %d, ctrl_kind %d)",
                d->form, d->net.ctrl_kind);
  p.DT = tiles_of(d);
  p.rf = RF_NONE;
  p.sc = SC_NONE;
  if (d->form == SDENG_FORM_CMCD || d->form == SDENG_FORM_CMCD_EUBO) return plan_cmcd(p);
  if (d->net.ctrl_kind == SDENG_CTRL_NONE) return plan_euler(p);
  return plan_sim(p);
}

static int run_cmcd(const SimPlan& p, const sdeng_desc* d, float* ws, SimArgs& a, hipStream_t s) {
  const Layout& L = p.L;
  const int DT = p.DT, dpad = 16 * DT;
  SD_TRY(prepare_net(d, L, ws, DT, a, s, d->N + 1, false, 0.0f));
  DistDev target, prior;
  SD_TRY(build_dist(d->target, d->d, dpad, ws + L.target, target, s));
  SD_TRY(build_dist(d->prior, d->d, dpad, ws + L.prior, prior, s));
  CmcdArgs c;
  memset(&c, 0, sizeof(c));
  float* prec = ws + L.cmcd;
  if (d->target.kind == SDENG_DIST_LOGREG) SD_TRY(prepare_logreg(d, L, ws, DT, a, s, &prec));
  float* locp = prec + align64(DT * sd_kb(DT) * 512);
  if (d->prior.kind == SDENG_DIST_GAUSS_FULL) {
    SD_HIP(sd_launch_pack_square(d->prior.scale, d->prior.loc, d->d, DT, prec, locp, s));
    c.prec_pack = prec; c.prior_loc = locp;
  } else if (d->prior.kind == SDENG_DIST_ISO_GAUSS) {
    c.iso_loc = d->prior.p0; c.inv_iso_var = 1.0f / d->prior.p3;
  }
  const bool eubo = d->form == SDENG_FORM_CMCD_EUBO;
  if (eubo) {
    SD_HIP(hipMemsetAsync(ws + L.rnd_init, 0, sizeof(float) * d->B, s));
    SD_TRY(terminal(d, dpad, target, target, false, true, d->x_in, ws + L.rnd_init, s));
  } else {
    SD_TRY(dist_eval(prior, d->B, d->d, dpad, d->x_in, ws + L.rnd_init, nullptr, s));
  }
  a.rnd_init = ws + L.rnd_init;
  a.cmcd_g = d->cmcd_g; a.cmcd_clip = d->cmcd_clip;
  a.target = target; a.prior = prior;
  c.s = a;
  SD_TRY(launch_timed(d, p.k, &c, s));
  if (eubo) return terminal(d, dpad, prior, prior, true, false, d->x_out, d->rnd_out, s);
  return terminal(d, dpad, target, target, false, true, d->x_out, d->rnd_out, s);
}

static int run_euler(const SimPlan& p, const sdeng_desc* d, float* ws, SimArgs& a, hipStream_t s) {
  SD_TRY(build_dist(d->target, d->d, 16 * p.DT, ws + p.L.target, a.target, s));
  a.clip_score = d->net.clip_score;
  return launch_timed(d, p.k, &a, s);
}

static int prepare_ref(const SimPlan& p, const sdeng_desc* d, float* ws, SimArgs& a, hipStream_t s) {
  const Layout& L = p.L;
  const int DT = p.DT, dpad = 16 * DT, K = ref_components(d), rf = p.rf;
  if (rf == RF_NONE) return 0;
  a.ref_k = K;
  a.ref_tab = ws + L.ref_tab; a.ref_consts = ws + L.ref_consts;
  a.ref_c1 = half_d_log_2pi(d->d);
  if (rf == RF_GMM_FULL) {
    if (d->N > 0) {
      RefFullArgs r;
      r.K = K; r.d = d->d; r.dpad = dpad; r.NT = DT; r.coef = p.in_slot ? nullptr : d->coef;
      r.means = d->ref.means_init; r.eigvals = d->ref.vars_init; r.eigvecs = d->ref.eigvecs; r.weights = d->ref.weights;
      r.images = ws + L.ref_tab; r.means_out = ws + L.ref_mean; r.consts = ws + L.ref_consts;
      SD_HIP(sd_launch_ref_full_tables(r, d->N, s));
    }
    a.ref_mean = ws + L.ref_mean;
    const int piece = (DT > 4 ? DT / 2 : DT) * sd_kb(DT) * 512;
    a.ref_share = (piece / 256 + SD_WAVES - 1) / SD_WAVES;
    return 0;
  }
  if (rf == RF_GMM_MM) {
    const int kt = (K + 15) / 16;
    if (d->N > 0) {
      RefMMArgs r;
      r.K = K; r.d = d->d; r.dpad = dpad; r.NT = DT; r.kt = kt; r.coef = d->coef;
      r.means = d->ref.means_init; r.vars = d->ref.vars_init; r.weights = d->ref.weights;
      r.images = ws + L.ref_tab; r.centre = ws + L.ref_mean; r.consts = ws + L.ref_consts;
      r.same_var = ws + L.ref_consts + static_cast<size_t>(d->N) * 64;
      SD_HIP(sd_launch_ref_mm_tables(r, d->N, s));
    }
    a.ref_kc = kt;
    a.ref_mean = ws + L.ref_mean;
    a.ref_share = (mm_piece(K, DT) / 256 + SD_WAVES - 1) / SD_WAVES;
    return 0;
  }
  if (d->N > 0) {
    RefTabArgs r;
    r.K = K; r.d = d->d; r.dpad = dpad; r.coef = d->coef;
    r.means = d->ref.means_init; r.vars = d->ref.vars_init; r.weights = rf != RF_GAUSS ? d->ref.weights : nullptr;
    r.tab = ws + L.ref_tab; r.consts = ws + L.ref_consts;
    r.same_var = ws + L.ref_consts + static_cast<size_t>(d->N) * K * 2;
    r.centred = (rf == RF_GMM && p.k.fam != SD_FAM_SPLIT) ? 1 : 0;
    SD_HIP(sd_launch_ref_tables(r, d->N, s));
  }
  a.ref_same_var = ws + L.ref_consts + static_cast<size_t>(d->N) * K * 2;
  if (rf == RF_GMM_BIG) {
    static const bool allow = [] { const char* e = getenv("SDENG_REF_SHARE"); return !(e && e[0] == '0'); }();
    const int cap = std::min(share_room(DT), sd_share_buf_floats(SD_SHARE_MAX)) / 256 * 256;
    const int kc_max = cap / (2 * dpad);
    if (allow && kc_max >= 1) {
      const int nch = (K + kc_max - 1) / kc_max;
      const int kc = (K + nch - 1) / nch;
      const int chunks = (kc * 2 * dpad + 255) / 256;
      a.ref_share = (chunks + SD_WAVES - 1) / SD_WAVES;
      a.ref_kc = kc;
    }
  }
  return 0;
}

static int run_sim(const SimPlan& p, const sdeng_desc* d, float* ws, SimArgs& a, hipStream_t s) {
  const Layout& L = p.L;
  const int DT = p.DT, dpad = 16 * DT;
  SD_TRY(prepare_net(d, L, ws, DT, a, s, d->N, false, 0.0f));
  SD_TRY(prepare_ref(p, d, ws, a, s));
  DistDev target, ref_dist, prior;
  SD_TRY(build_dist(d->target, d->d, dpad, ws + L.target, target, s));
  SD_TRY(build_dist(d->ref_dist, d->d, dpad, ws + L.ref_dist, ref_dist, s));
  SD_TRY(build_dist(d->prior, d->d, dpad, ws + L.prior, prior, s));
  a.target = target;
  a.prior = prior;
  const bool eubo = d->form == SDENG_FORM_EUBO;
  const bool tr = d->flags & SDENG_FLAG_TERM_REF, tt = d->flags & SDENG_FLAG_TERM_TARGET;
  if ((d->flags & SDENG_FLAG_INIT_LOGP) && !eubo) {
    SD_TRY(dist_eval(prior, d->B, d->d, dpad, d->x_in, ws + L.rnd_init, nullptr, s));
    a.rnd_init = ws + L.rnd_init;
  }
  if (eubo && (tr || tt)) {
    SD_HIP(hipMemsetAsync(ws + L.rnd_init, 0, sizeof(float) * d->B, s));
    SD_TRY(terminal(d, dpad, ref_dist, target, tr, tt, d->x_in, ws + L.rnd_init, s));
    a.rnd_init = ws + L.rnd_init;
  }
  if (p.sc == SC_LOGREG) {
    float* unused;
    SD_TRY(prepare_logreg(d, L, ws, DT, a, s, &unused));
  }
  SD_TRY(launch_timed(d, p.k, &a, s));
  if (!eubo && (tr || tt)) SD_TRY(terminal(d, dpad, ref_dist, target, tr, tt, d->x_out, d->rnd_out, s));
  if (eubo && (d->flags & SDENG_FLAG_INIT_LOGP)) SD_TRY(terminal(d, dpad, prior, prior, true, false, d->x_out, d->rnd_out, s));
  return 0;
}

extern "C" int sdeng_simulate(const sdeng_desc* desc, void* stream) {
  hipStream_t s = static_cast<hipStream_t>(stream);
  SimPlan p;
  int rc = plan_simulate(desc, p);
  if (rc || desc->B == 0) return rc;
  const sdeng_desc* d = p.d;
  if (!d->workspace || d->workspace_bytes < p.L.total * sizeof(float))
    return fail(SDENG_E_WORKSPACE, "workspace %zu bytes, need %zu", d->workspace_bytes, p.L.total * sizeof(float));
  float* ws = static_cast<float*>(d->workspace);
  SimArgs a;
  memset(&a, 0, sizeof(a));
  a.form = d->form; a.flags = d->flags;
  a.B = d->B; a.d = d->d; a.N = d->N;
  a.particle0 = d->particle0;
  const Seed seed = split_seed(d->seed);
  a.seed_lo = seed.lo; a.seed_hi = seed.hi;
  a.coef = d->coef; a.x_in = d->x_in; a.x_out = d->x_out; a.rnd_out = d->rnd_out;
  a.xs_out = d->xs_out; a.noise_in = d->noise_in;
  a.trash = ws + p.L.trash;
  a.ntiles = (d->B + 15) / 16;
  sdeng_desc dm;
  if (!d->x_in) {
    float* x0 = d->x0_out ? d->x0_out : ws + p.L.x0;
    SD_HIP(sd_launch_sample_x0(d->x0_dist, seed.lo, seed.hi, d->particle0, d->B, d->d, x0, s));
    dm = *d;
    dm.x_in = x0;
    d = &dm;
    a.x_in = x0;
  }
  if (p.k.fam == SD_FAM_CMCD) return run_cmcd(p, d, ws, a, s);
  if (p.k.fam == SD_FAM_EULER) return run_euler(p, d, ws, a, s);
  return run_sim(p, d, ws, a, s);
}

extern "C" int sdeng_sample_x0(const sdeng_dist* dist, uint64_t seed, int64_t particle0, int32_t B, int32_t d, float* out, void* stream) {
  if (!dist || !out || B < 0 || d < 1 || d > 128) return fail(SDENG_E_INVALID, "bad argument");
  if (B == 0) return 0;
  sdeng_desc tmp;
  memset(&tmp, 0, sizeof(tmp));
  tmp.x0_dist = *dist;
  SD_TRY(check_x0_dist(&tmp));
  const Seed sd = split_seed(seed);
  SD_HIP(sd_launch_sample_x0(*dist, sd.lo, sd.hi, particle0, B, d, out, static_cast<hipStream_t>(stream)));
  return 0;
}

extern "C" int sdeng_ctrl_forward(const sdeng_desc* d, float t_net, float score_gain, float lerp_w, const float* x, float* u_out,
                                  void* stream) {
  hipStream_t s = static_cast<hipStream_t>(stream);
  if (!d || !x || !u_out) return fail(SDENG_E_INVALID, "null argument");
  Layout L;
  if (!make_layout(d, L)) return fail(SDENG_E_INVALID, "bad sizes");
  const bool ws_ok = d->workspace && d->workspace_bytes >= L.total * sizeof(float);
  if (d->B == 0) return ws_ok ? 0 : fail(SDENG_E_WORKSPACE, "workspace too small");
  const int DT = tiles_of(d), dpad = 16 * DT;
  int sc;
  KernelKey k;
  SD_TRY(check_net(d->net));
  SD_TRY(score_kind(d, sc));
  SD_TRY(check_dist(d->target, d->d));
  SD_TRY(check_dist(d->prior, d->d));
  if (sc == SC_LOGREG) return fail(SDENG_E_UNSUPPORTED, "ctrl_forward: no in-loop logistic-regression score (the step loop's only)");
  SD_TRY(select_kernel(k, SD_FAM_CTRL, DT, sc));
  if (!ws_ok) return fail(SDENG_E_WORKSPACE, "workspace too small");
  float* ws = static_cast<float*>(d->workspace);
  SimArgs a;
  memset(&a, 0, sizeof(a));
  a.B = d->B; a.d = d->d; a.N = 1;
  a.x_in = x; a.x_out = u_out;
  a.trash = ws + L.trash;
  a.ntiles = (d->B + 15) / 16;
  SD_TRY(prepare_net(d, L, ws, DT, a, s, 1, true, t_net));
  SD_TRY(build_dist(d->target, d->d, dpad, ws + L.target, a.target, s));
  SD_TRY(build_dist(d->prior, d->d, dpad, ws + L.prior, a.prior, s));
  float host_coef[SDENG_NCOEF] = {0};
  host_coef[0] = t_net; host_coef[7] = score_gain; host_coef[8] = lerp_w;
  float* dev_coef = ws + L.logz;
  SD_HIP(hipMemcpyAsync(dev_coef, host_coef, sizeof(host_coef), hipMemcpyHostToDevice, s));
  a.coef = dev_coef;
  SD_HIP(k.fn(&a, s));
  return 0;
}

struct VjpLayout {
  size_t wt, temb, trash, total;
};
static VjpLayout vjp_layout(int DT, int n_times) {
  VjpLayout v;
  size_t o = align64(sd_pack_floats(DT));
  v.wt = o; o += align64(sd_lds_weight_floats(DT));
  v.temb = o; o += align64(static_cast<size_t>(n_times) * SD_H);
  v.trash = o; o += align64(SD_WAVES_MAX * 64 * 4);
  v.total = o;
  return v;
}
extern "C" size_t sdeng_ctrl_vjp_workspace_bytes(int32_t d, int32_t n_times) {
  if (d < 1 || d > 128 || n_times < 1) return 0;
  return vjp_layout(tiles_exact(d), n_times).total * sizeof(float);
}
struct VjpOut { float *a0, *a1, *a2, *d0, *d1, *d2, *dout; };
static int prepare_vjp(const sdeng_desc* d, int DT, const VjpLayout& V, size_t total, bool pack, int n_times, int rows_per_time, const float* x,
                       const VjpOut& o, size_t stheta_off, const float** stheta, VjpArgs& v, hipStream_t s) {
  const size_t need = total * sizeof(float);
  if (!d->workspace || d->workspace_bytes < need) return fail(SDENG_E_WORKSPACE, "workspace %zu bytes, need %zu", d->workspace_bytes, need);
  float* ws = static_cast<float*>(d->workspace);
  if (pack) SD_TRY(pack_net(d, DT, ws, ws + V.wt, s));
  SD_TRY(embed_times(d, n_times, false, 0.0f, ws + V.temb, ws + stheta_off, stheta, s));
  v.M = n_times * rows_per_time; v.B = rows_per_time; v.d = d->d; v.N = n_times;
  v.x = x; v.wpack = ws; v.wpack_t = ws + V.wt; v.temb = ws + V.temb;
  v.clip_model = d->net.clip_model;
  v.a0 = o.a0; v.a1 = o.a1; v.a2 = o.a2; v.d0 = o.d0; v.d1 = o.d1; v.d2 = o.d2; v.dout = o.dout;
  v.trash = ws + V.trash;
  return 0;
}
extern "C" int sdeng_ctrl_vjp(const sdeng_desc* d, int32_t n_times, int32_t rows_per_time, const float* x, const float* cot, float* a0,
                              float* a1, float* a2, float* d0, float* d1, float* d2, float* dout, float* gx, float* u_out, void* stream) {
  hipStream_t s = static_cast<hipStream_t>(stream);
  if (!d || !x) return fail(SDENG_E_INVALID, "null argument");
  if (cot && (!a0 || !a1 || !a2 || !d0 || !d1 || !d2 || !dout)) return fail(SDENG_E_INVALID, "backward pass: every per-row output is required");
  if (!cot && !u_out) return fail(SDENG_E_INVALID, "nothing to compute: no cotangent and no u_out");
  SD_TRY(check_abi(d));
  if (d->d < 1 || d->d > 128 || n_times < 1 || rows_per_time < 1 || !d->coef) return fail(SDENG_E_INVALID, "bad sizes (1 <= d <= 128, n_times, rows_per_time >= 1) or null coef");
  if (d->net.ctrl_kind != SDENG_CTRL_CLIPPED) return fail(SDENG_E_UNSUPPORTED, "ctrl_vjp: ClippedCtrl around the FourierMLP (ctrl_kind %d given)", d->net.ctrl_kind);
  const long long M = static_cast<long long>(n_times) * rows_per_time;
  if (M * d->d >= (1ll << 31)) return fail(SDENG_E_UNSUPPORTED, "rows * d >= 2^31");
  SD_TRY(check_net(d->net));
  const int DT = tiles_exact(d->d);
  KernelKey k;
  SD_TRY(select_kernel(k, SD_FAM_VJP, DT, gx ? 1 : 0));
  const VjpLayout V = vjp_layout(DT, n_times);
  VjpArgs a;
  memset(&a, 0, sizeof(a));
  const float* no_stheta;
  SD_TRY(prepare_vjp(d, DT, V, V.total, !(d->flags & SDENG_FLAG_REUSE_PACK), n_times, rows_per_time, x, {a0, a1, a2, d0, d1, d2, dout}, 0, &no_stheta, a, s));
  a.cot = cot; a.gx = gx; a.u_out = u_out;
  a.ntiles = static_cast<int>((M + 15) / 16);
  SD_HIP(k.fn(&a, s));
  return 0;
}

struct AdjLayout {
  VjpLayout v;
  size_t tab, consts, stheta, target, total;
};
static AdjLayout adjoint_layout(const sdeng_desc* d, int DT) {
  AdjLayout A;
  A.v = vjp_layout(DT, d->N);
  size_t o = A.v.total;
  const int K = ref_components(d);
  A.tab = o; o += align64(static_cast<size_t>(d->N) * K * 2 * 16 * DT);
  A.consts = o; o += align64(static_cast<size_t>(d->N) * K * 2 + 1);
  A.stheta = o; o += align64(static_cast<size_t>(d->N));
  A.target = o; o += dist_floats(d->target, 16 * DT);
  A.total = o;
  return A;
}
static int check_adjoint(const sdeng_desc* d, bool ext_score) {
  if (!d) return fail(SDENG_E_INVALID, "null descriptor");
  SD_TRY(check_abi(d));
  if (d->d < 1 || d->d > 128 || d->N < 1 || d->B < 1 || !d->coef) return fail(SDENG_E_INVALID, "bad sizes (1 <= d <= 128, N, B >= 1) or null coef");
  if (d->form != SDENG_FORM_LIN && d->form != SDENG_FORM_EM) return fail(SDENG_E_UNSUPPORTED, "kl_adjoint: forward forms LIN / EM (form %d)", d->form);
  if (d->net.ctrl_kind != SDENG_CTRL_CLIPPED &&
      !(score_like(d->net.ctrl_kind) && (ext_score || d->target.kind == SDENG_DIST_GMM_DIAG || d->target.kind == SDENG_DIST_PHI4)))
    return fail(SDENG_E_UNSUPPORTED, "kl_adjoint: ClippedCtrl, or Score / Lerp / CancelDrift control on a diagonal mixture / phi^4 target (ctrl_kind %d, "
                                     "target kind %d)", d->net.ctrl_kind, d->target.kind);
  SD_TRY(check_lerp_prior(d));
  if (d->target.kind == SDENG_DIST_CHECKERBOARD || d->prior.kind == SDENG_DIST_CHECKERBOARD)
    return fail(SDENG_E_UNSUPPORTED, "kl_adjoint: no adjoint for a checkerboard target (KL training takes the per-step path)");
  if (d->ref.kind != SDENG_REF_NONE && d->ref.kind != SDENG_REF_GAUSS_DIAG && d->ref.kind != SDENG_REF_GMM_DIAG)
    return fail(SDENG_E_UNSUPPORTED, "kl_adjoint: no reference, or a diagonal Gaussian / mixture reference (ref.kind %d)", d->ref.kind);
  if (d->ref.kind != SDENG_REF_NONE && ((d->ref.kind == SDENG_REF_GMM_DIAG && d->ref.k < 1) || !d->ref.means_init || !d->ref.vars_init))
    return fail(SDENG_E_INVALID, "reference: null means/vars or k < 1");
  if (static_cast<long long>(d->N) * d->B * d->d >= (1ll << 31)) return fail(SDENG_E_UNSUPPORTED, "N * B * d >= 2^31");
  return check_net(d->net);
}
extern "C" size_t sdeng_kl_adjoint_workspace_bytes(const sdeng_desc* d) {
  if (!d || d->d < 1 || d->d > 128 || d->N < 1) return 0;
  return adjoint_layout(d, tiles_exact(d->d)).total * sizeof(float);
}
extern "C" int sdeng_kl_adjoint(const sdeng_desc* d, const sdeng_adjoint* adj, void* stream) {
  hipStream_t s = static_cast<hipStream_t>(stream);
  SD_TRY(check_adjoint(d, adj && adj->score));
  if (!adj || !adj->xs || !adj->w || !adj->lam_in || !adj->a0 || !adj->a1 || !adj->a2 || !adj->d0 || !adj->d1 || !adj->d2 || !adj->dout)
    return fail(SDENG_E_INVALID, "kl_adjoint: null states / weights / lambda_N / per-row outputs");
  const bool ito = d->flags & SDENG_FLAG_ITO;
  if (ito && !adj->noise) return fail(SDENG_E_INVALID, "kl_adjoint: FLAG_ITO needs the normals of the trajectory");
  const bool score = d->net.ctrl_kind != SDENG_CTRL_CLIPPED;
  if (score && !adj->dst) return fail(SDENG_E_INVALID, "kl_adjoint: a score control needs the dst output");
  if (score && !adj->score) SD_TRY(check_dist(d->target, d->d));
  const int has_score = !score ? ADJ_NONE : adj->score ? ADJ_EXT : (d->target.kind == SDENG_DIST_PHI4 ? ADJ_PHI4 : ADJ_GMM);
  const int DT = tiles_exact(d->d), dpad = 16 * DT;
  KernelKey k;
  SD_TRY(select_kernel(k, SD_FAM_ADJ, DT, has_score));
  const AdjLayout A = adjoint_layout(d, DT);
  AdjArgs a;
  memset(&a, 0, sizeof(a));
  SD_TRY(prepare_vjp(d, DT, A.v, A.total, true, d->N, d->B, adj->xs, {adj->a0, adj->a1, adj->a2, adj->d0, adj->d1, adj->d2, adj->dout}, A.stheta, &a.stheta,
                     a.v, s));
  float* ws = static_cast<float*>(d->workspace);
  if (d->ref.kind != SDENG_REF_NONE) {
    const int K = ref_components(d);
    RefTabArgs r;
    r.K = K; r.d = d->d; r.dpad = dpad; r.coef = d->coef;
    r.means = d->ref.means_init; r.vars = d->ref.vars_init; r.weights = d->ref.kind == SDENG_REF_GMM_DIAG ? d->ref.weights : nullptr;
    r.tab = ws + A.tab; r.consts = ws + A.consts;
    r.same_var = ws + A.consts + static_cast<size_t>(d->N) * K * 2;
    r.centred = 0;
    SD_HIP(sd_launch_ref_tables(r, d->N, s));
    a.ref_tab = ws + A.tab; a.ref_consts = ws + A.consts; a.ref_k = K;
    a.ref_c1 = half_d_log_2pi(d->d);
  }
  a.has_score = has_score;
  if (score) {
    a.score_ext = adj->score;
    if (!adj->score) SD_TRY(build_dist(d->target, d->d, dpad, ws + A.target, a.target, s));
    a.scale_score = d->net.scale_score; a.clip_score = d->net.clip_score;
    a.ctrl_kind = d->net.ctrl_kind;
    a.prior_loc = d->prior.p0; a.prior_scale = d->net.ctrl_kind == SDENG_CTRL_LERP ? d->prior.p1 : 1.0f;
    a.score_detached = adj->detach_score ? 1 : 0;
    a.dst = adj->dst;
  }
  a.coef = d->coef; a.noise = ito ? adj->noise : nullptr; a.w = adj->w; a.lam_in = adj->lam_in; a.lam_out = adj->lam_out;
  a.lin = d->form == SDENG_FORM_LIN ? 1 : 0;
  a.ntiles_b = (d->B + 15) / 16;
  SD_HIP(k.fn(&a, s));
  return 0;
}

struct CmcdAdjLayout {
  VjpLayout v;
  size_t stheta, target, prior, total;
};
static CmcdAdjLayout cmcd_adjoint_layout(const sdeng_desc* d, int DT) {
  CmcdAdjLayout A;
  A.v = vjp_layout(DT, d->N + 1);
  size_t o = A.v.total;
  A.stheta = o; o += align64(static_cast<size_t>(d->N) + 1);
  A.target = o; o += dist_floats(d->target, 16 * DT);
  A.prior = o; o += dist_floats(d->prior, 16 * DT);
  A.total = o;
  return A;
}
static int check_cmcd_adjoint(const sdeng_desc* d, bool ext_score) {
  if (!d) return fail(SDENG_E_INVALID, "null descriptor");
  SD_TRY(check_abi(d));
  if (d->d > 128) return fail(SDENG_E_UNSUPPORTED, "cmcd_kl_adjoint: d <= 128 (got %d)", d->d);
  if (d->d < 1 || d->N < 1 || d->B < 1 || !d->coef) return fail(SDENG_E_INVALID, "bad sizes (1 <= d, N, B >= 1) or null coef");
  if (d->net.ctrl_kind != SDENG_CTRL_CLIPPED && d->net.ctrl_kind != SDENG_CTRL_SCORE)
    return fail(SDENG_E_UNSUPPORTED, "cmcd_kl_adjoint: ClippedCtrl or ScoreCtrl (ctrl_kind %d)", d->net.ctrl_kind);
  if (d->prior.kind == SDENG_DIST_GAUSS_FULL)
    return fail(SDENG_E_UNSUPPORTED, "cmcd_kl_adjoint: no adjoint for a full-covariance prior (KL training takes the per-step path)");
  if (d->prior.kind != SDENG_DIST_ISO_GAUSS && d->prior.kind != SDENG_DIST_GAUSS_DIAG)
    return fail(SDENG_E_UNSUPPORTED, "cmcd_kl_adjoint: prior must be ISO_GAUSS or GAUSS_DIAG (kind %d)", d->prior.kind);
  switch (d->target.kind) {
    case SDENG_DIST_GAUSS_FULL:
    case SDENG_DIST_GMM_FULL:
      return fail(SDENG_E_UNSUPPORTED, "cmcd_kl_adjoint: no adjoint for a full-covariance target (kind %d)", d->target.kind);
    case SDENG_DIST_RINGS:
      return fail(SDENG_E_UNSUPPORTED, "cmcd_kl_adjoint: no adjoint for a rings target (KL training takes the per-step path)");
    case SDENG_DIST_CHECKERBOARD:
      return fail(SDENG_E_UNSUPPORTED, "cmcd_kl_adjoint: no adjoint for a checkerboard target (KL training takes the per-step path)");
    case SDENG_DIST_LOGREG:
      if (!ext_score) return fail(SDENG_E_INVALID, "cmcd_kl_adjoint: a logistic-regression target needs the score of every row (adj->score)");
      if (d->d > 64) return fail(SDENG_E_UNSUPPORTED, "cmcd_kl_adjoint: logistic regression with d <= 64 (got %d), as its step loop", d->d);
      break;
    case SDENG_DIST_GMM_DIAG:
    case SDENG_DIST_GAUSS_DIAG:
    case SDENG_DIST_PHI4:
      if (ext_score) return fail(SDENG_E_INVALID, "cmcd_kl_adjoint: adj->score is for targets with a graph-less score (LOGREG); kind %d has a closed form", d->target.kind);
      break;
    default:
      return fail(SDENG_E_UNSUPPORTED, "cmcd_kl_adjoint: target must be GMM_DIAG, GAUSS_DIAG, PHI4 or LOGREG (kind %d)", d->target.kind);
  }
  if ((static_cast<long long>(d->N) + 1) * d->B * d->d >= (1ll << 31)) return fail(SDENG_E_UNSUPPORTED, "(N + 1) * B * d >= 2^31");
  SD_TRY(check_net(d->net));
  SD_TRY(check_dist(d->prior, d->d));
  return ext_score ? 0 : check_dist(d->target, d->d);
}
extern "C" size_t sdeng_cmcd_kl_adjoint_workspace_bytes(const sdeng_desc* d) {
  if (!d || d->d < 1 || d->d > 128 || d->N < 1) return 0;
  return cmcd_adjoint_layout(d, tiles_exact(d->d)).total * sizeof(float);
}
extern "C" int sdeng_cmcd_kl_adjoint(const sdeng_desc* d, const sdeng_cmcd_adjoint* adj, void* stream) {
  hipStream_t s = static_cast<hipStream_t>(stream);
  SD_TRY(check_cmcd_adjoint(d, adj && adj->score));
  if (!adj || !adj->xs || !adj->cbar || !adj->w || !adj->lam_in || !adj->a0 || !adj->a1 || !adj->a2 || !adj->d0 || !adj->d1 || !adj->d2 || !adj->dout)
    return fail(SDENG_E_INVALID, "cmcd_kl_adjoint: null states / costs / weights / lam_in / per-row outputs");
  const bool score = d->net.ctrl_kind == SDENG_CTRL_SCORE;
  if (score && !adj->dst) return fail(SDENG_E_INVALID, "cmcd_kl_adjoint: a ScoreCtrl needs the dst output");
  const int tgt = adj->score ? CADJ_EXT : (d->target.kind == SDENG_DIST_PHI4 ? CADJ_PHI4 : CADJ_GMM);
  const int DT = tiles_exact(d->d), dpad = 16 * DT;
  KernelKey k;
  SD_TRY(select_kernel(k, SD_FAM_CADJ, DT, tgt));
  const CmcdAdjLayout A = cmcd_adjoint_layout(d, DT);
  CmcdAdjArgs a;
  memset(&a, 0, sizeof(a));
  SD_TRY(prepare_vjp(d, DT, A.v, A.total, true, d->N + 1, d->B, adj->xs, {adj->a0, adj->a1, adj->a2, adj->d0, adj->d1, adj->d2, adj->dout}, A.stheta,
                     &a.stheta, a.v, s));
  float* ws = static_cast<float*>(d->workspace);
  if (tgt != CADJ_EXT) SD_TRY(build_dist(d->target, d->d, dpad, ws + A.target, a.target, s));
  if (d->prior.kind == SDENG_DIST_GAUSS_DIAG) {
    DistDev prior;
    SD_TRY(build_dist(d->prior, d->d, dpad, ws + A.prior, prior, s));
    a.prior_tab = prior.tab;
  } else {
    a.iso_loc = d->prior.p0; a.inv_iso_var = 1.0f / d->prior.p3;
  }
  a.g = d->cmcd_g; a.clip = d->cmcd_clip;
  a.has_score = score ? 1 : 0;
  if (score) {
    a.scale_score = d->net.scale_score; a.clip_score = d->net.clip_score;
    a.score_detached = adj->detach_score ? 1 : 0;
    a.dst = adj->dst;
  }
  a.score_ext = adj->score;
  a.coef = d->coef; a.cbar = adj->cbar; a.w = adj->w; a.lam_in = adj->lam_in; a.lam_out = adj->lam_out;
  a.steps = d->N;
  a.ntiles_b = (d->B + 15) / 16;
  SD_HIP(k.fn(&a, s));
  return 0;
}

extern "C" int sdeng_dist_eval(const sdeng_dist* dist, int32_t B, int32_t d, const float* x, float* logp_out, float* score_out,
                               void* workspace, size_t workspace_bytes, void* stream) {
  hipStream_t s = static_cast<hipStream_t>(stream);
  if (!dist || !x || d < 1 || B < 0) return fail(SDENG_E_INVALID, "bad argument");
  if (d > 255) return fail(SDENG_E_UNSUPPORTED, "dist_eval: d <= 255 (rows are staged through LDS), got %d", d);
  if (B == 0) return 0;
  const int dpad = pad16(d);
  const size_t need = dist_floats(*dist, dpad) * sizeof(float);
  if (need > 0 && (!workspace || workspace_bytes < need)) return fail(SDENG_E_WORKSPACE, "workspace %zu bytes, need %zu", workspace_bytes, need);
  DistDev dd;
  SD_TRY(build_dist(*dist, d, dpad, static_cast<float*>(workspace), dd, s));
  return dist_eval(dd, B, d, dpad, x, logp_out, score_out, s);
}

static size_t moves_workspace_bytes(const sdeng_dist* prior, const sdeng_dist* target, int32_t d) {
  if (!target || d < 1) return 0;
  const int dpad = pad16(d);
  return (dist_floats(*target, dpad) + (prior ? dist_floats(*prior, dpad) : 0) + 64) * sizeof(float);
}
static int run_moves(int move, const char* who, const sdeng_dist* prior, const sdeng_dist* target, int32_t B, int32_t d, int32_t n_moves,
                     int32_t keep_from, int32_t unadjusted, float target_acceptance, const float* t, float* x, float* lp, float* grad,
                     float* step, const float* z, const float* u, uint64_t seed, int64_t chain0, float* samples, float* acc_sum,
                     float* acc_last, void* workspace, size_t workspace_bytes, void* stream) {
  hipStream_t s = static_cast<hipStream_t>(stream);
  const bool langevin = move == SD_MOVE_LANGEVIN;
  if (!target || !x || !lp || (langevin && !grad) || !step || B < 0 || d < 1 || n_moves < 0 || keep_from < 0 || keep_from > n_moves)
    return fail(SDENG_E_INVALID, "%s: bad argument", who);
  if (target->kind == SDENG_DIST_NONE) return fail(SDENG_E_INVALID, "%s: no target distribution", who);
  if (d > 255) return fail(SDENG_E_UNSUPPORTED, "%s: d <= 255 (chain rows live in LDS), got %d", who, d);
  if ((z == nullptr) != (u == nullptr) && !unadjusted)
    return fail(SDENG_E_INVALID, "%s: inject both the normals and the uniforms, or neither (unadjusted moves: the normals alone)", who);
  if (langevin && (target->kind == SDENG_DIST_CHECKERBOARD || (prior && prior->kind == SDENG_DIST_CHECKERBOARD)))
    return fail(SDENG_E_UNSUPPORTED, "%s: no moves on a checkerboard (its log-density is -inf on a set of positive mass)", who);
  const bool has_prior = prior && prior->kind != SDENG_DIST_NONE;
  SD_TRY(check_dist(*target, d));
  if (has_prior) SD_TRY(check_dist(*prior, d));
  if (B == 0 || n_moves == 0) return 0;
  const int dpad = pad16(d);
  const size_t need = moves_workspace_bytes(prior, target, d);
  if (!workspace || workspace_bytes < need) return fail(SDENG_E_WORKSPACE, "%s: workspace %zu bytes, need %zu", who, workspace_bytes, need);
  float* ws = static_cast<float*>(workspace);
  MovesArgs a;
  memset(&a, 0, sizeof(a));
  SD_TRY(build_dist(*target, d, dpad, ws, a.target.ds, s));
  a.target.d = d; a.target.dpad = dpad; a.target.B = B;
  a.prior.ds.kind = SDENG_DIST_NONE;
  if (has_prior) SD_TRY(build_dist(*prior, d, dpad, ws + dist_floats(*target, dpad), a.prior.ds, s));
  a.prior.d = d; a.prior.dpad = dpad; a.prior.B = B;
  a.B = B; a.d = d; a.K = n_moves; a.keep_from = keep_from; a.ula = unadjusted ? 1 : 0; a.target_acc = target_acceptance;
  a.t = t; a.x = x; a.lp = lp; a.grad = grad; a.step = step; a.z = z; a.u = u;
  const Seed sd = split_seed(seed);
  a.seed_lo = sd.lo; a.seed_hi = sd.hi; a.chain0 = chain0;
  a.samples = samples; a.acc_sum = acc_sum; a.acc_last = acc_last;
  SD_HIP(sd_launch_moves(a, move, s));
  return 0;
}

extern "C" size_t sdeng_langevin_moves_workspace_bytes(const sdeng_dist* prior, const sdeng_dist* target, int32_t d) {
  return moves_workspace_bytes(prior, target, d);
}
extern "C" int sdeng_langevin_moves(const sdeng_dist* prior, const sdeng_dist* target, int32_t B, int32_t d, int32_t n_moves, int32_t keep_from,
                                    int32_t unadjusted, float target_acceptance, const float* t, float* x, float* lp, float* grad, float* step,
                                    const float* z, const float* u, uint64_t seed, int64_t chain0, float* samples, float* acc_sum,
                                    float* acc_last, void* workspace, size_t workspace_bytes, void* stream) {
  return run_moves(SD_MOVE_LANGEVIN, "langevin_moves", prior, target, B, d, n_moves, keep_from, unadjusted, target_acceptance, t, x, lp, grad, step,
                   z, u, seed, chain0, samples, acc_sum, acc_last, workspace, workspace_bytes, stream);
}
extern "C" size_t sdeng_rwmh_moves_workspace_bytes(const sdeng_dist* target, int32_t d) { return moves_workspace_bytes(nullptr, target, d); }
extern "C" int sdeng_rwmh_moves(const sdeng_dist* target, int32_t B, int32_t d, int32_t n_moves, int32_t keep_from, float target_acceptance,
                                float* x, float* lp, float* step, const float* z, const float* u, uint64_t seed, int64_t chain0,
                                float* samples, float* acc_sum, float* acc_last, void* workspace, size_t workspace_bytes, void* stream) {
  return run_moves(SD_MOVE_RWMH, "rwmh_moves", nullptr, target, B, d, n_moves, keep_from, 0, target_acceptance, nullptr, x, lp, nullptr, step, z, u,
                   seed, chain0, samples, acc_sum, acc_last, workspace, workspace_bytes, stream);
}

extern "C" size_t sdeng_dist_workspace_bytes(const sdeng_dist* dist, int32_t d) {
  if (!dist || d < 1) return 0;
  return dist_floats(*dist, pad16(d)) * sizeof(float);
}

extern "C" size_t sdeng_logz_workspace_bytes(void) { return 5 * SD_LOGZ_MAX_BLOCKS * sizeof(float); }

extern "C" int sdeng_logz(const float* rnd, int64_t B, float* stats, float* weights_out, void* workspace, size_t workspace_bytes,
                          void* stream) {
  if (!rnd || !stats || B < 1) return fail(SDENG_E_INVALID, "bad argument");
  if (!workspace || workspace_bytes < sdeng_logz_workspace_bytes()) return fail(SDENG_E_WORKSPACE, "logz workspace too small");
  SD_HIP(sd_launch_logz(rnd, B, stats, weights_out, static_cast<float*>(workspace), static_cast<hipStream_t>(stream)));
  return 0;
}

extern "C" int sdeng_philox_normal(uint64_t seed, int32_t step, int64_t particle0, int32_t B, int32_t d, uint32_t stream_id, float* out,
                                   void* stream) {
  return sdeng_philox_normal_steps(seed, step, 1, particle0, B, d, stream_id, out, stream);
}
extern "C" int sdeng_philox_normal_steps(uint64_t seed, int32_t step0, int32_t n_steps, int64_t particle0, int32_t B, int32_t d,
                                         uint32_t stream_id, float* out, void* stream) {
  if (!out || B < 0 || d < 1 || n_steps < 0) return fail(SDENG_E_INVALID, "bad argument");
  if (B == 0 || n_steps == 0) return 0;
  const Seed sd = split_seed(seed);
  SD_HIP(sd_launch_philox(sd.lo, sd.hi, step0, n_steps, particle0, B, d, stream_id, out, static_cast<hipStream_t>(stream)));
  return 0;
}

static bool sk_fits(int32_t n, int32_t m) { return sizeof(float) * static_cast<size_t>(n) * m <= SDENG_SINKHORN_MATRIX_MAX_BYTES; }
extern "C" size_t sdeng_sinkhorn_workspace_bytes(int32_t n, int32_t m, int32_t d, int32_t materialise) {
  if (n < 1 || m < 1 || d < 1) return 0;
  const SkLayout L = sd_sk_layout(n, m);
  return materialise && sk_fits(n, m) ? L.total_bytes : L.small_bytes;
}
extern "C" int sdeng_sinkhorn(const float* x, const float* y, int32_t n, int32_t m, int32_t d, int32_t p, double eps, int32_t max_iters,
                              double stop_thresh, const float* w_x, const float* w_y, float* u_out, float* v_out, int32_t* corr_x_to_y,
                              int32_t* corr_y_to_x, sdeng_sinkhorn_result* result, void* workspace, size_t workspace_bytes, void* stream) {
  if (!x || !y || !result || n < 1 || m < 1 || d < 1 || max_iters < 1 || !(eps > 0.0)) return fail(SDENG_E_INVALID, "sinkhorn: bad argument");
  if ((w_x == nullptr) != (w_y == nullptr)) return fail(SDENG_E_INVALID, "sinkhorn: give both weight vectors, or neither");
  if (p != 1 && p != 2) return fail(SDENG_E_UNSUPPORTED, "sinkhorn: p in {1, 2}, got %d", p);
  const SkLayout L = sd_sk_layout(n, m);
  if (!workspace || workspace_bytes < L.small_bytes) return fail(SDENG_E_WORKSPACE, "workspace %zu bytes, need %zu", workspace_bytes, L.small_bytes);
  char* ws = static_cast<char*>(workspace);
  SkArgs a;
  memset(&a, 0, sizeof(a));
  a.x = x; a.y = y; a.w_x = w_x; a.w_y = w_y; a.n = n; a.m = m; a.d = d; a.p = p; a.eps = eps; a.inv_eps = 1.0 / eps;
  a.u = reinterpret_cast<double*>(ws + L.u); a.v = reinterpret_cast<double*>(ws + L.v);
  a.loga = reinterpret_cast<double*>(ws + L.loga); a.logb = reinterpret_cast<double*>(ws + L.logb);
  a.du = reinterpret_cast<double*>(ws + L.du); a.dv = reinterpret_cast<double*>(ws + L.dv);
  a.rowsum = reinterpret_cast<double*>(ws + L.rowsum); a.part = reinterpret_cast<double*>(ws + L.part);
  a.part_idx = reinterpret_cast<int*>(ws + L.part_idx); a.errs = reinterpret_cast<double*>(ws + L.errs);
  a.chunks = L.chunks; a.rows_per_chunk = L.rows_per_chunk;
  a.u_out = u_out; a.v_out = v_out; a.corr_xy = corr_x_to_y; a.corr_yx = corr_y_to_x;
  float* M = sk_fits(n, m) && workspace_bytes >= L.total_bytes ? reinterpret_cast<float*>(ws + L.M) : nullptr;
  SD_HIP(sd_run_sinkhorn(a, M, max_iters, stop_thresh, result, static_cast<hipStream_t>(stream)));
  return 0;
}

extern "C" size_t sdeng_mmd_median_workspace_bytes(int32_t n, int32_t d) {
  if (n < 2 || d < 1) return 0;
  return sd_mmd_layout(n).total_bytes;
}
extern "C" int sdeng_mmd_median(const float* X, const float* Y, int32_t n, int32_t m, int32_t d, float* out, void* workspace,
                                size_t workspace_bytes, void* stream) {
  if (!X || !Y || !out || d < 1) return fail(SDENG_E_INVALID, "mmd_median: bad argument");
  if (n != m || n < 2) return fail(SDENG_E_INVALID, "mmd_median: n == m >= 2 (additions/mmd.py:33-36), got %d and %d", n, m);
  if (n > (1 << 29)) return fail(SDENG_E_UNSUPPORTED, "mmd_median: n <= 2^29");
  const MmdLayout L = sd_mmd_layout(n);
  if (!workspace || workspace_bytes < L.total_bytes) return fail(SDENG_E_WORKSPACE, "workspace %zu bytes, need %zu", workspace_bytes, L.total_bytes);
  char* ws = static_cast<char*>(workspace);
  MmdArgs a;
  a.X = X; a.Y = Y; a.n = n; a.d = d; a.tiles = L.tiles; a.groups = L.groups;
  a.hist = reinterpret_cast<unsigned long long*>(ws + L.hist); a.state = reinterpret_cast<unsigned long long*>(ws + L.state);
  a.part = reinterpret_cast<double*>(ws + L.part); a.out = out;
  SD_HIP(sd_run_mmd_median(a, static_cast<hipStream_t>(stream)));
  return 0;
}

struct TiltedLayout {
  size_t pack, consts, trash, hbuf, total;
  int ntiles, waves, grid, nimg;
};
static TiltedLayout tilted_layout(const sdeng_tilted* t, bool train = false) {
  TiltedLayout L;
  L.ntiles = (t->M + 15) / 16;
  L.waves = sd_tilted_waves(L.ntiles);
  L.grid = sd_tilted_grid(L.ntiles, L.waves);
  L.nimg = TL_EIG + (t->full_cov ? 2 * t->k : 0);
  size_t o = 0;
  L.pack = o; o += static_cast<size_t>(L.nimg) * TL_SLOT;
  L.consts = o; o += align64(TL_C_TOTAL);
  L.trash = o; o += align64(512 * 4);
  L.hbuf = o; o += (t->grad || train) ? static_cast<size_t>(L.grid) * L.waves * TL_HBUF_FLOATS : 0;
  L.total = o;
  return L;
}
static int check_tilted(const sdeng_tilted* t, const char* who = "tilted_eval", bool train = false, bool moves = false) {
  if (!t) return fail(SDENG_E_INVALID, "%s: null descriptor", who);
  if (t->abi_version != SDENG_ABI_VERSION) return fail(SDENG_E_INVALID, "ABI version %d, library has %d", t->abi_version, SDENG_ABI_VERSION);
  if (t->d < 1 || t->d > 128) return fail(SDENG_E_INVALID, "%s: d = %d outside [1, 128]", who, t->d);
  if (t->k < 1 || t->k > TL_KMAX) return fail(SDENG_E_INVALID, "%s: k = %d components outside [1, %d]", who, t->k, TL_KMAX);
  if (t->M < 1 || t->n_times < 1 || t->rows_per_time < 1 || static_cast<long long>(t->n_times) * t->rows_per_time != t->M)
    return fail(SDENG_E_INVALID, "%s: M = %d rows is not n_times * rows_per_time = %d * %d", who, t->M, t->n_times, t->rows_per_time);
  if (static_cast<long long>(t->M) * t->d >= (1ll << 31)) return fail(SDENG_E_UNSUPPORTED, "%s: rows * d >= 2^31", who);
  if (t->num_layers != 6 || t->channels != TL_H)
    return fail(SDENG_E_UNSUPPORTED, "%s: the kernel is built for FourierMLP(num_layers=6, channels=128), got num_layers=%d channels=%d", who,
                t->num_layers, t->channels);
  if (t->tilt_type != SDENG_TILT_DOT) return fail(SDENG_E_UNSUPPORTED, "%s: tilt_type 'dot' only (type %d given)", who, t->tilt_type);
  if (t->use_scaling_factor) return fail(SDENG_E_UNSUPPORTED, "%s: use_scaling_factor (the DRL scaling argument) is not supported", who);
  const void* need[] = {moves ? t->tinfo : t->x, t->tinfo, t->w_in, t->b_in, t->w_out, t->b_out, t->te_coeff, t->te_phase, t->te_w1, t->te_b1, t->te_w2, t->te_b2,
                        t->mean_gauss, t->var_gauss, t->weights, t->means, t->vars, t->w_h[0], t->w_h[1], t->w_h[2], t->w_h[3],
                        t->b_h[0], t->b_h[1], t->b_h[2], t->b_h[3]};
  for (const void* p : need)
    if (!p) return fail(SDENG_E_INVALID, "%s: null pointer in the descriptor", who);
  if (t->full_cov && !t->eigvecs) return fail(SDENG_E_INVALID, "%s: full_cov without eigvecs", who);
  if (!train && !moves && !t->log_prob && !t->grad) return fail(SDENG_E_INVALID, "%s: nothing to compute (log_prob and grad are both NULL)", who);
  return 0;
}
extern "C" size_t sdeng_tilted_eval_workspace_bytes(const sdeng_tilted* t) {
  if (check_tilted(t)) return 0;
  return tilted_layout(t).total * sizeof(float);
}
static int pack_tilted(const sdeng_tilted* t, const TiltedLayout& L, float* ws, hipStream_t s) {
  const int d = t->d, H = TL_H;
  TiltedPackArgs p;
  memset(&p, 0, sizeof(p));
  p.pack = ws + L.pack; p.consts = ws + L.consts;
  p.coeff = t->te_coeff; p.phase = t->te_phase; p.mean_gauss = t->mean_gauss; p.var_gauss = t->var_gauss;
  p.weights = t->weights; p.means = t->means; p.vars = t->vars; p.d = d; p.K = t->k;
  int n = 0;
  auto job = [&](int slot, const float* W, int n_out, int n_in, int ld, int col0, int transpose, int scale_n, const float* bias, int bias_off) {
    TiltedPackJob& j = p.job[n++];
    j.src = W; j.scale_src = W; j.bias = bias; j.n_out = n_out; j.n_in = n_in; j.ld = ld; j.col0 = col0; j.transpose = transpose;
    j.scale_n = scale_n; j.slot = slot; j.bias_off = bias ? bias_off : -1;
  };
  job(TL_TE1S, t->te_w1, H, H, 2 * H, 0, 0, 2 * H * H, t->te_b1, TL_C_BTE1);
  job(TL_TE1C, t->te_w1, H, H, 2 * H, H, 0, 2 * H * H, nullptr, 0);
  job(TL_TE2, t->te_w2, H, H, H, 0, 0, H * H, t->te_b2, TL_C_BTE2);
  job(TL_WIN, t->w_in, H, d, d, 0, 0, H * d, t->b_in, TL_C_BIN);
  for (int l = 0; l < 4; ++l) job(TL_WH + l, t->w_h[l], H, H, H, 0, 0, H * H, t->b_h[l], TL_C_BH + 128 * l);
  job(TL_WOUT, t->w_out, d, H, H, 0, 0, d * H, t->b_out, TL_C_BOUT);
  job(TL_WOUT_T, t->w_out, H, d, H, 0, 1, d * H, nullptr, 0);
  for (int l = 0; l < 4; ++l) job(TL_WH_T + l, t->w_h[l], H, H, H, 0, 1, H * H, nullptr, 0);
  job(TL_WIN_T, t->w_in, d, H, d, 0, 1, H * d, nullptr, 0);
  if (t->full_cov)
    for (int k = 0; k < t->k; ++k) {
      const float* P = t->eigvecs + static_cast<size_t>(k) * d * d;
      job(TL_EIG + 2 * k, P, d, d, d, 0, 1, d * d, nullptr, 0);
      job(TL_EIG + 2 * k + 1, P, d, d, d, 0, 0, d * d, nullptr, 0);
    }
  p.njobs = n;
  SD_HIP(sd_launch_tilted_pack(p, s));
  return 0;
}
static int run_tilted(const sdeng_tilted* t, const TiltedRows* rows, void* stream) {
  hipStream_t s = static_cast<hipStream_t>(stream);
  const TiltedLayout L = tilted_layout(t, rows != nullptr);
  const size_t need = L.total * sizeof(float);
  if (!t->workspace || t->workspace_bytes < need) return fail(SDENG_E_WORKSPACE, "workspace %zu bytes, need %zu", t->workspace_bytes, need);
  float* ws = static_cast<float*>(t->workspace);
  const int d = t->d;
  if (!(t->flags & SDENG_FLAG_REUSE_PACK)) SD_TRY(pack_tilted(t, L, ws, s));
  TiltedArgs a;
  memset(&a, 0, sizeof(a));
  a.M = t->M; a.B = t->rows_per_time; a.d = d; a.N = t->n_times; a.K = t->k; a.full = t->full_cov ? 1 : 0;
  a.use_st = t->use_s_t_scaling ? 1 : 0; a.ntiles = L.ntiles;
  a.x = t->x; a.tinfo = t->tinfo; a.pack = ws + L.pack; a.consts = ws + L.consts;
  a.hbuf = (t->grad || rows) ? ws + L.hbuf : nullptr; a.log_prob = t->log_prob; a.grad = t->grad; a.trash = ws + L.trash;
  if (rows) SD_HIP(sd_launch_tilted_train(a, *rows, tiles_exact(d), L.grid, L.waves, s));
  else SD_HIP(sd_launch_tilted(a, tiles_exact(d), L.grid, L.waves, s));
  return 0;
}
extern "C" int sdeng_tilted_eval(const sdeng_tilted* t, void* stream) {
  SD_TRY(check_tilted(t));
  return run_tilted(t, nullptr, stream);
}
static int check_tilted_rows(const sdeng_tilted_rows* r) {
  if (!r) return fail(SDENG_E_INVALID, "tilted_vjp: null rows");
  for (int l = 0; l < 5; ++l) {
    if (!r->a[l]) return fail(SDENG_E_INVALID, "tilted_vjp: rows->a[%d] is NULL", l);
    if (!r->d[l]) return fail(SDENG_E_INVALID, "tilted_vjp: rows->d[%d] is NULL", l);
  }
  if (!r->xs) return fail(SDENG_E_INVALID, "tilted_vjp: rows->xs is NULL");
  if (!r->dv) return fail(SDENG_E_INVALID, "tilted_vjp: rows->dv is NULL");
  return 0;
}
extern "C" size_t sdeng_tilted_vjp_workspace_bytes(const sdeng_tilted* t) {
  if (check_tilted(t, "tilted_vjp", true)) return 0;
  return tilted_layout(t, true).total * sizeof(float);
}
extern "C" int sdeng_tilted_vjp(const sdeng_tilted* t, const sdeng_tilted_rows* r, void* stream) {
  SD_TRY(check_tilted(t, "tilted_vjp", true));
  SD_TRY(check_tilted_rows(r));
  TiltedRows rows;
  for (int l = 0; l < 5; ++l) { rows.a[l] = r->a[l]; rows.d[l] = r->d[l]; }
  rows.xs = r->xs; rows.dv = r->dv;
  return run_tilted(t, &rows, stream);
}

struct TiltedMovesLayout {
  TiltedLayout L;
  size_t prop, gprop, total;
};
static TiltedMovesLayout tilted_moves_layout(const sdeng_tilted* t) {
  TiltedMovesLayout ml;
  ml.L = tilted_layout(t, true);
  size_t o = ml.L.hbuf + static_cast<size_t>(ml.L.grid) * ml.L.waves * TLM_HBUF_FLOATS;
  const size_t rows = align64(static_cast<size_t>(t->M) * t->d);
  ml.prop = o; o += rows;
  ml.gprop = o; o += rows;
  ml.total = o;
  return ml;
}
static int check_tilted_moves(const sdeng_tilted* t, const sdeng_tilted_moves_state* mv) {
  const char* who = "tilted_moves";
  SD_TRY(check_tilted(t, who, false, true));
  if (!mv) return fail(SDENG_E_INVALID, "%s: null move state", who);
  if (!mv->x || !mv->lp || !mv->grad || !mv->step) return fail(SDENG_E_INVALID, "%s: x, lp, grad and step are all required", who);
  if (mv->n_moves < 0) return fail(SDENG_E_INVALID, "%s: n_moves = %d < 0", who, mv->n_moves);
  if (mv->keep_from < 0 || mv->keep_from > mv->n_moves)
    return fail(SDENG_E_INVALID, "%s: keep_from = %d outside [0, n_moves = %d]", who, mv->keep_from, mv->n_moves);
  if ((mv->z == nullptr) != (mv->u == nullptr) && !mv->unadjusted)
    return fail(SDENG_E_INVALID, "%s: inject both the normals and the uniforms, or neither (unadjusted moves: the normals alone)", who);
  return 0;
}
extern "C" size_t sdeng_tilted_moves_workspace_bytes(const sdeng_tilted* t) {
  if (check_tilted(t, "tilted_moves", false, true)) return 0;
  return tilted_moves_layout(t).total * sizeof(float);
}
extern "C" int sdeng_tilted_moves(const sdeng_tilted* t, const sdeng_tilted_moves_state* mv, void* stream) {
  SD_TRY(check_tilted_moves(t, mv));
  hipStream_t s = static_cast<hipStream_t>(stream);
  const TiltedMovesLayout ml = tilted_moves_layout(t);
  const TiltedLayout& L = ml.L;
  const size_t need = ml.total * sizeof(float);
  if (!t->workspace || t->workspace_bytes < need)
    return fail(SDENG_E_WORKSPACE, "tilted_moves: workspace %zu bytes, need %zu", t->workspace_bytes, need);
  if (mv->n_moves == 0) return 0;
  float* ws = static_cast<float*>(t->workspace);
  if (!(t->flags & SDENG_FLAG_REUSE_PACK)) SD_TRY(pack_tilted(t, L, ws, s));
  TiltedArgs a;
  memset(&a, 0, sizeof(a));
  a.M = t->M; a.B = t->rows_per_time; a.d = t->d; a.N = t->n_times; a.K = t->k; a.full = t->full_cov ? 1 : 0;
  a.use_st = t->use_s_t_scaling ? 1 : 0; a.ntiles = L.ntiles;
  a.tinfo = t->tinfo; a.pack = ws + L.pack; a.consts = ws + L.consts; a.hbuf = ws + L.hbuf; a.trash = ws + L.trash;
  TiltedMovesArgs m;
  memset(&m, 0, sizeof(m));
  m.x = mv->x; m.grad = mv->grad; m.lp = mv->lp; m.step = mv->step; m.prop = ws + ml.prop; m.gprop = ws + ml.gprop;
  m.z = mv->z; m.u = mv->unadjusted ? nullptr : mv->u; m.samples = mv->samples; m.acc_sum = mv->acc_sum; m.acc_last = mv->acc_last;
  m.K = mv->n_moves; m.keep_from = mv->keep_from; m.ula = mv->unadjusted ? 1 : 0; m.target_acc = mv->target_acceptance;
  const Seed sd = split_seed(mv->seed);
  m.seed_lo = sd.lo; m.seed_hi = sd.hi; m.chain0 = mv->chain0;
  SD_HIP(sd_launch_tilted_moves(a, m, tiles_exact(t->d), L.grid, L.waves, s));
  return 0;
}
```

Before: 3.609 billion particle-steps/s.

## Batch prep kernels into one multi-role launch via Prep job queue

Turns the separate setup kernels (weight scales, MLP packing, time embedding, same-var check, reference tables, distribution tables, x0 sampling) into device role functions. A Prep object collects them and flushes them as a combined launch instead of many small dispatches. To drop the dependency between the scale kernel and the pack kernel, each pack block recomputes the weight-scale reductions it needs, and the reference-table blocks recompute the same-variance check. This cuts kernel launch count and serialization before the main simulation, at the cost of redundant reduction work per block.

Result: no change. 3.632 billion particle-steps/s, median of 6 (+0.6%).

```diff
diff --git a/sde_sampler_lrds_amd/csrc/cmcd_inst.hip b/sde_sampler_lrds_amd/csrc/cmcd_inst.hip
--- a/sde_sampler_lrds_amd/csrc/cmcd_inst.hip
+++ b/sde_sampler_lrds_amd/csrc/cmcd_inst.hip
@@ -1,50 +1 @@
 #include "cmcd_kernel.hpp"
-
-__device__ inline void block_coords(int local, int KB, int& part, int& o, int& i) {
-  const int j = local & 7, lane = (local >> 3) & 63, blk = local >> 10;
-  part = (local >> 9) & 1;
-  const int kb = blk % KB, to = blk / KB;
-  o = 16 * to + (lane & 15);
-  i = 16 * (2 * kb + (j >> 2)) + 4 * (lane >> 4) + (j & 3);
-}
-__device__ inline _Float16 split_part(float w, int part) {
-  const _Float16 hi = static_cast<_Float16>(w);
-  return part == 0 ? hi : static_cast<_Float16>((w - static_cast<float>(hi)) * 2048.0f);
-}
-__global__ void k_logreg_images(const float* X, const float* y, int n, int dw, int NT, float* image, float* y_pad) {
-  const int KB = sd_kb(NT), RKB = sd_lr_row_kb(n);
-  const int n_logit = sd_lr_logit_floats(NT, n) * 2, n_grad = sd_lr_grad_floats(NT, n) * 2;
-  _Float16* img = reinterpret_cast<_Float16*>(image);
-  for (int idx = blockIdx.x * blockDim.x + threadIdx.x; idx < n_logit + n_grad; idx += gridDim.x * blockDim.x) {
-    int part, o, i, row, col;
-    if (idx < n_logit) {
-      block_coords(idx, KB, part, o, i);
-      row = o; col = i;
-    } else {
-      block_coords(idx - n_logit, RKB, part, o, i);
-      row = i; col = o;
-    }
-    float v = 0.0f;
-    if (row < n) v = (col < dw) ? X[static_cast<size_t>(row) * dw + col] : (col == dw ? 1.0f : 0.0f);
-    img[idx] = split_part(v, part);
-    if (idx < 32 * RKB) y_pad[idx] = (idx < n) ? y[idx] : 0.0f;
-  }
-}
-__global__ void k_pack_square(const float* P, const float* loc, int d, int NT, float* out, float* loc_pad) {
-  const int KB = sd_kb(NT);
-  _Float16* img = reinterpret_cast<_Float16*>(out);
-  for (int idx = blockIdx.x * blockDim.x + threadIdx.x; idx < NT * KB * 1024; idx += gridDim.x * blockDim.x) {
-    int part, o, i;
-    block_coords(idx, KB, part, o, i);
-    img[idx] = split_part((o < d && i < d) ? P[static_cast<size_t>(o) * d + i] : 0.0f, part);
-    if (idx < 16 * NT) loc_pad[idx] = idx < d ? loc[idx] : 0.0f;
-  }
-}
-int sd_launch_logreg_images(const float* X, const float* y, int n, int dw, int NT, float* image, float* y_pad, hipStream_t s) {
-  hipLaunchKernelGGL(k_logreg_images, dim3(96), dim3(256), 0, s, X, y, n, dw, NT, image, y_pad);
-  return static_cast<int>(hipGetLastError());
-}
-int sd_launch_pack_square(const float* P, const float* loc, int d, int NT, float* out, float* loc_pad, hipStream_t s) {
-  hipLaunchKernelGGL(k_pack_square, dim3(NT * sd_kb(NT) * 4), dim3(256), 0, s, P, loc, d, NT, out, loc_pad);
-  return static_cast<int>(hipGetLastError());
-}
diff --git a/sde_sampler_lrds_amd/csrc/prep_kernels.hip b/sde_sampler_lrds_amd/csrc/prep_kernels.hip
--- a/sde_sampler_lrds_amd/csrc/prep_kernels.hip
+++ b/sde_sampler_lrds_amd/csrc/prep_kernels.hip
@@ -1,97 +1,112 @@
 #include "sim_device.hpp"
 #include "prep_kernels.hpp"
 
-__global__ void __launch_bounds__(256) k_weight_scales(PackArgs a) {
-  __shared__ float red[256];
+__device__ inline int weight_scale_exp(const PackArgs& a, int l, int t, float* red) {
+  const float* W = l == 0 ? a.w_in : (l == 1 ? a.w_h1 : (l == 2 ? a.w_h2 : a.w_out));
+  const int n = (l == 0 || l == 3) ? SD_H * a.d : SD_H * SD_H;
+  float m = 0.0f;
+  for (int i = t; i < n; i += 256) {
+    const float v = __builtin_fabsf(W[i]);
+    m = (v <= 3.0e38f) ? fmaxf(m, v) : m;
+  }
+  red[t] = m;
+  __syncthreads();
+  for (int s = 128; s > 0; s >>= 1) {
+    if (t < s) red[t] = fmaxf(red[t], red[t + s]);
+    __syncthreads();
+  }
+  const float mx = red[0];
+  __syncthreads();
+  int e = 0;
+  if (mx > 0.0f && (mx < 9.765625e-4f || mx >= 16384.0f)) {
+    int ex;
+    frexpf(mx, &ex);
+    e = 1 - ex;
+    e = e > 100 ? 100 : (e < -100 ? -100 : e);
+  }
+  return e;
+}
+
+__device__ inline void role_weight_scales(const PackArgs& a, int l, int t, float* red) {
   float* sc = a.out + sd_off_scales(a.NT);
-  {
-    const int l = blockIdx.x;
-    const float* W = l == 0 ? a.w_in : (l == 1 ? a.w_h1 : (l == 2 ? a.w_h2 : a.w_out));
-    const int n = (l == 0 || l == 3) ? SD_H * a.d : SD_H * SD_H;
-    float m = 0.0f;
-    for (int i = threadIdx.x; i < n; i += 256) {
-      const float v = __builtin_fabsf(W[i]);
-      m = (v <= 3.0e38f) ? fmaxf(m, v) : m;
-    }
-    red[threadIdx.x] = m;
-    __syncthreads();
-    for (int s = 128; s > 0; s >>= 1) {
-      if (threadIdx.x < s) red[threadIdx.x] = fmaxf(red[threadIdx.x], red[threadIdx.x + s]);
-      __syncthreads();
-    }
-    if (threadIdx.x == 0) {
-      const float mx = red[0];
-      int e = 0;
-      if (mx > 0.0f && (mx < 9.765625e-4f || mx >= 16384.0f)) {
-        int ex;
-        frexpf(mx, &ex);
-        e = 1 - ex;
-        e = e > 100 ? 100 : (e < -100 ? -100 : e);
-      }
-      sc[l] = ldexpf(1.0f, e);
-      sc[4 + l] = ldexpf(1.0f, -e);
-    }
-    __syncthreads();
-  }
-}
-
-__global__ void k_pack_mlp(PackArgs a) {
+  const int e = weight_scale_exp(a, l, t, red);
+  if (t == 0) {
+    sc[l] = ldexpf(1.0f, e);
+    sc[4 + l] = ldexpf(1.0f, -e);
+  }
+}
+
+__device__ inline void role_pack(const PackArgs& a, int lb, int t, float* red) {
   const int NT = a.NT;
-  const float* scales = a.transpose ? a.scales : a.out + sd_off_scales(NT);
   const int n_half = sd_lds_weight_floats(NT) * 2;
   const int n_bias = a.transpose ? 0 : 3 * 64 + 16 * NT;
   _Float16* img = reinterpret_cast<_Float16*>(a.out);
-  for (int idx = blockIdx.x * blockDim.x + threadIdx.x; idx < n_half + n_bias; idx += gridDim.x * blockDim.x) {
-    if (idx < n_half) {
-      const int fl = idx >> 1;
-      const float* W;
-      int n_out, n_in, KB, base, layer;
-      if (fl < sd_off_wh1(NT)) {
-        W = a.w_in; n_out = SD_H; n_in = a.d; KB = sd_kb(NT); base = sd_off_win(NT); layer = 0;
-      } else if (fl < sd_off_wh2(NT)) {
-        W = a.w_h1; n_out = SD_H; n_in = SD_H; KB = 2; base = sd_off_wh1(NT); layer = 1;
-      } else if (fl < sd_off_wout(NT)) {
-        W = a.w_h2; n_out = SD_H; n_in = SD_H; KB = 2; base = sd_off_wh2(NT); layer = 2;
+  const int first = lb * 256, idx = first + t;
+  int slot = 0;
+  if (first < n_half) {
+    const int fl = first >> 1;
+    slot = fl < sd_off_wh1(NT) ? 0 : (fl < sd_off_wh2(NT) ? 1 : (fl < sd_off_wout(NT) ? 2 : 3));
+  }
+  const int need = first >= n_half ? 0xF : 1 << (a.transpose ? 3 - slot : slot);
+  float s0 = 1.0f, s1 = 1.0f, s2 = 1.0f, s3 = 1.0f;
+  if (need & 1) s0 = ldexpf(1.0f, weight_scale_exp(a, 0, t, red));
+  if (need & 2) s1 = ldexpf(1.0f, weight_scale_exp(a, 1, t, red));
+  if (need & 4) s2 = ldexpf(1.0f, weight_scale_exp(a, 2, t, red));
+  if (need & 8) s3 = ldexpf(1.0f, weight_scale_exp(a, 3, t, red));
+  if (idx >= n_half + n_bias) return;
+  if (idx < n_half) {
+    const int layer = slot;
+    const float* W;
+    int n_out, n_in, KB, base;
+    if (layer == 0) {
+      W = a.w_in; n_out = SD_H; n_in = a.d; KB = sd_kb(NT); base = sd_off_win(NT);
+    } else if (layer == 1) {
+      W = a.w_h1; n_out = SD_H; n_in = SD_H; KB = 2; base = sd_off_wh1(NT);
+    } else if (layer == 2) {
+      W = a.w_h2; n_out = SD_H; n_in = SD_H; KB = 2; base = sd_off_wh2(NT);
+    } else {
+      W = a.w_out; n_out = a.d; n_in = SD_H; KB = 2; base = sd_off_wout(NT);
+    }
+    const int local = idx - 2 * base;
+    const int j = local & 7;
+    const int lane = (local >> 3) & 63;
+    const int part = (local >> 9) & 1;
+    const int blk = local >> 10;
+    const int kb = blk % KB, to = blk / KB;
+    const int o = 16 * to + (lane & 15);
+    const int i = 16 * (2 * kb + (j >> 2)) + 4 * (lane >> 4) + (j & 3);
+    const int mat = a.transpose ? 3 - layer : layer;
+    const float scale = mat == 0 ? s0 : (mat == 1 ? s1 : (mat == 2 ? s2 : s3));
+    float w = 0.0f;
+    if (o < n_out && i < n_in) {
+      if (!a.transpose) {
+        w = W[static_cast<size_t>(o) * n_in + i] * scale;
       } else {
-        W = a.w_out; n_out = a.d; n_in = SD_H; KB = 2; base = sd_off_wout(NT); layer = 3;
-      }
-      const int local = idx - 2 * base;
-      const int j = local & 7;
-      const int lane = (local >> 3) & 63;
-      const int part = (local >> 9) & 1;
-      const int blk = local >> 10;
-      const int kb = blk % KB, to = blk / KB;
-      const int o = 16 * to + (lane & 15);
-      const int i = 16 * (2 * kb + (j >> 2)) + 4 * (lane >> 4) + (j & 3);
-      float w = 0.0f;
-      if (o < n_out && i < n_in) {
-        if (!a.transpose) {
-          w = W[static_cast<size_t>(o) * n_in + i] * scales[layer];
-        } else {
-          const float* Wt = layer == 0 ? a.w_out : (layer == 1 ? a.w_h2 : (layer == 2 ? a.w_h1 : a.w_in));
-          w = Wt[static_cast<size_t>(i) * n_out + o] * scales[3 - layer];
-        }
-      }
-      const _Float16 hi = static_cast<_Float16>(w);
-      img[idx] = part == 0 ? hi : static_cast<_Float16>((w - static_cast<float>(hi)) * 2048.0f);
-    } else {
-      const int b = idx - n_half;
-      float v;
-      if (b < 64) v = a.b_in[b] * scales[0];
-      else if (b < 128) v = a.b_h1[b - 64] * scales[1];
-      else if (b < 192) v = a.b_h2[b - 128] * scales[2];
-      else v = (b - 192 < a.d) ? a.b_out[b - 192] * scales[3] : 0.0f;
-      a.out[sd_off_bias(NT) + b] = v;
-    }
-  }
+        const float* Wt = layer == 0 ? a.w_out : (layer == 1 ? a.w_h2 : (layer == 2 ? a.w_h1 : a.w_in));
+        w = Wt[static_cast<size_t>(i) * n_out + o] * scale;
+      }
+    }
+    const _Float16 hi = static_cast<_Float16>(w);
+    img[idx] = part == 0 ? hi : static_cast<_Float16>((w - static_cast<float>(hi)) * 2048.0f);
+  } else {
+    const int b = idx - n_half;
+    float v;
+    if (b < 64) v = a.b_in[b] * s0;
+    else if (b < 128) v = a.b_h1[b - 64] * s1;
+    else if (b < 192) v = a.b_h2[b - 128] * s2;
+    else v = (b - 192 < a.d) ? a.b_out[b - 192] * s3 : 0.0f;
+    a.out[sd_off_bias(NT) + b] = v;
+  }
+}
+int sd_prep_pack_blocks(const PackArgs& a) {
+  return (sd_lds_weight_floats(a.NT) * 2 + (a.transpose ? 0 : 3 * 64 + 16 * a.NT) + 255) / 256;
 }
 
 __device__ inline float gelu_exact(float v) { return (v * 0.5f) * (1.0f + erff(v * 0.70710678118654752440f)); }
 
-__global__ void __launch_bounds__(64) k_time_embed(TimeEmbedArgs a) {
-  __shared__ float e[128];
-  __shared__ float hbuf[2][64];
-  const int k = blockIdx.x, j = threadIdx.x;
+__device__ inline void role_time_embed(const TimeEmbedArgs& a, int k, bool on, int j, float* lds) {
+  float* e = lds;
+  float (*hbuf)[64] = reinterpret_cast<float (*)[64]>(lds + 128);
   const float t = a.t_direct ? a.t_value : a.coef[static_cast<size_t>(k) * SDENG_NCOEF + a.col];
   const float arg = (a.te.coeff[j] * t) + a.te.phase[j];
   e[j] = sinf(arg);
@@ -110,7 +125,7 @@
     n_in = 64;
     cur ^= 1;
   }
-  if (j < a.te.dim_out) {
+  if (on && j < a.te.dim_out) {
     const float* W = a.te.w_out + static_cast<size_t>(j) * 64;
     float acc = 0.0f;
     for (int i = 0; i < 64; ++i) acc = __builtin_fmaf(W[i], in[i], acc);
@@ -120,24 +135,26 @@
   }
 }
 
-__global__ void __launch_bounds__(128) k_same_var(const float* vars, int K, int d, float* same_var) {
+__device__ inline bool same_var_all(const float* vars, int K, int d) {
   int differ = 0;
-  for (int i = threadIdx.x; i < K * d; i += 128) differ |= vars[i] != vars[i % d];
-  differ = __syncthreads_or(differ);
-  if (threadIdx.x == 0) same_var[0] = differ ? 0.0f : 1.0f;
-}
-
-__global__ void __launch_bounds__(128) k_ref_tables(RefTabArgs a) {
-  __shared__ float red[128];
-  const int k = blockIdx.x / a.K, c = blockIdx.x % a.K;
+  for (int i = threadIdx.x; i < K * d; i += SD_PREP_THREADS) differ |= vars[i] != vars[i % d];
+  return !__syncthreads_or(differ);
+}
+__device__ inline void role_same_var(const SameVarArgs& a) {
+  const bool same = same_var_all(a.vars, a.K, a.d);
+  if (threadIdx.x == 0) a.same_var[0] = same ? 1.0f : 0.0f;
+}
+
+__device__ inline void role_ref_tables(const RefTabArgs& a, int lb, bool on, int t, float* red) {
+  const int k = lb / a.K, c = lb % a.K;
   const float S = a.coef[static_cast<size_t>(k) * SDENG_NCOEF + 9];
   const float VA = a.coef[static_cast<size_t>(k) * SDENG_NCOEF + 10];
   const float S2 = a.coef[static_cast<size_t>(k) * SDENG_NCOEF + 11];
-  const bool centred = a.centred && a.K == SD_KREG && a.same_var[0] != 0.0f;
+  const bool centred = same_var_all(a.vars, a.K, a.d) && a.centred && a.K == SD_KREG;
   float* tm = a.tab + (static_cast<size_t>(k) * a.K + c) * 2 * a.dpad;
   float* tv = tm + a.dpad;
   float ls = 0.0f, quad = 0.0f;
-  for (int f = threadIdx.x; f < a.dpad; f += 128) {
+  for (int f = t; f < a.dpad; f += 128) {
     float mean = 0.0f, iv = 0.0f, cen = 0.0f;
     if (f < a.d) {
       mean = S * a.means[static_cast<size_t>(c) * a.d + f];
@@ -153,28 +170,30 @@
     if (centred) {
       const float dm = mean - cen;
       quad = __builtin_fmaf(dm * dm, iv, quad);
-      tm[f] = dm * iv;
-      tv[f] = c == 0 ? iv : (c == 1 ? cen : 0.0f);
-    } else {
+      if (on) {
+        tm[f] = dm * iv;
+        tv[f] = c == 0 ? iv : (c == 1 ? cen : 0.0f);
+      }
+    } else if (on) {
       tm[f] = mean;
       tv[f] = iv;
     }
   }
-  red[threadIdx.x] = ls;
+  red[t] = ls;
   __syncthreads();
   for (int s = 64; s > 0; s >>= 1) {
-    if (threadIdx.x < s) red[threadIdx.x] += red[threadIdx.x + s];
+    if (t < s) red[t] += red[t + s];
     __syncthreads();
   }
   const float ls_sum = red[0];
   __syncthreads();
-  red[threadIdx.x] = quad;
+  red[t] = quad;
   __syncthreads();
   for (int s = 64; s > 0; s >>= 1) {
-    if (threadIdx.x < s) red[threadIdx.x] += red[threadIdx.x + s];
-    __syncthreads();
-  }
-  if (threadIdx.x == 0) {
+    if (t < s) red[t] += red[t + s];
+    __syncthreads();
+  }
+  if (on && t == 0) {
     float wsum = 0.0f;
     for (int i = 0; i < a.K; ++i) wsum += a.weights ? a.weights[i] : 1.0f;
     const float w = (a.weights ? a.weights[c] : 1.0f) / wsum;
@@ -183,6 +202,8 @@
     cs[1] = centred ? logf(w) - 0.5f * red[0] : logf(w);
   }
 }
+
+__global__ void __launch_bounds__(SD_PREP_THREADS) k_same_var(SameVarArgs a) { role_same_var(a); }
 
 __global__ void __launch_bounds__(256) k_ref_full_tables(RefFullArgs a) {
   __shared__ float invd[128];
@@ -293,13 +314,12 @@
   }
 }
 
-__global__ void __launch_bounds__(128) k_dist_tables(DistTabArgs a) {
-  __shared__ float red[2][128];
-  const int c = blockIdx.x;
+__device__ inline void role_dist_tables(const DistTabArgs& a, int c, bool on, int t, float* lds) {
+  float (*red)[128] = reinterpret_cast<float (*)[128]>(lds);
   float* tm = a.tab + static_cast<size_t>(c) * 2 * a.dpad;
   float* tv = tm + a.dpad;
   float lv = 0.0f, lsig = 0.0f;
-  for (int f = threadIdx.x; f < a.dpad; f += 128) {
+  for (int f = t; f < a.dpad; f += 128) {
     float mean = 0.0f, iv = 0.0f;
     if (f < a.d) {
       mean = a.loc[static_cast<size_t>(c) * a.d + f];
@@ -309,20 +329,22 @@
       lv += logf(var);
       lsig += logf(sc);
     }
-    tm[f] = mean;
-    tv[f] = iv;
-  }
-  red[0][threadIdx.x] = lv;
-  red[1][threadIdx.x] = lsig;
+    if (on) {
+      tm[f] = mean;
+      tv[f] = iv;
+    }
+  }
+  red[0][t] = lv;
+  red[1][t] = lsig;
   __syncthreads();
   for (int s = 64; s > 0; s >>= 1) {
-    if (threadIdx.x < s) {
-      red[0][threadIdx.x] += red[0][threadIdx.x + s];
-      red[1][threadIdx.x] += red[1][threadIdx.x + s];
-    }
-    __syncthreads();
-  }
-  if (threadIdx.x == 0) {
+    if (t < s) {
+      red[0][t] += red[0][t + s];
+      red[1][t] += red[1][t + s];
+    }
+    __syncthreads();
+  }
+  if (on && t == 0) {
     float* cs = a.consts + static_cast<size_t>(c) * 4;
     cs[0] = 0.5f * red[0][0];
     cs[2] = red[1][0] + static_cast<float>(a.d) * 0.91893853320467274178f;
@@ -905,14 +927,14 @@
     if (4 * jb + e < d) o[static_cast<size_t>(row) * d + 4 * jb + e] = z[e];
 }
 
-__global__ void k_sample_x0(X0Dev q, unsigned seed_lo, unsigned seed_hi, long long particle0, int B, int d, float* out) {
-  const int nj = (d + 3) / 4;
-  const long long idx = blockIdx.x * static_cast<long long>(blockDim.x) + threadIdx.x;
-  if (idx >= static_cast<long long>(B) * nj) return;
+__device__ inline void role_sample_x0(const X0Args& a, int lb, int t) {
+  const int d = a.d, nj = (d + 3) / 4;
+  const long long idx = lb * 256ll + t;
+  if (idx >= static_cast<long long>(a.B) * nj) return;
   const int row = static_cast<int>(idx / nj), jb = static_cast<int>(idx % nj);
-  const f32x4 x = x0_quad(q, static_cast<uint32_t>(particle0 + row), jb, d, seed_lo, seed_hi);
+  const f32x4 x = x0_quad(a.q, static_cast<uint32_t>(a.particle0 + row), jb, d, a.seed_lo, a.seed_hi);
   for (int e = 0; e < 4; ++e)
-    if (4 * jb + e < d) out[static_cast<size_t>(row) * d + 4 * jb + e] = x[e];
+    if (4 * jb + e < d) a.out[static_cast<size_t>(row) * d + 4 * jb + e] = x[e];
 }
 #define SD_X0_FULL_ROWS 64
 __global__ void __launch_bounds__(256) k_sample_x0_full(const float* loc, const float* L, unsigned seed_lo, unsigned seed_hi, long long particle0,
@@ -940,34 +962,92 @@
     out[static_cast<size_t>(row0) * d + i] = loc[f] + acc;
   }
 }
-int sd_launch_sample_x0(const sdeng_dist& ds, unsigned lo, unsigned hi, long long p0, int B, int d, float* out, hipStream_t s) {
-  if (ds.kind == SDENG_DIST_GAUSS_FULL) {
-    const size_t lds = (static_cast<size_t>(SD_X0_FULL_ROWS) * (4 * ((d + 3) / 4) + 1) + static_cast<size_t>(d) * (d | 1)) * sizeof(float);
-    if (lds > 160 * 1024) return static_cast<int>(hipErrorInvalidValue);
-    if (lds > 64 * 1024) (void)hipFuncSetAttribute(reinterpret_cast<const void*>(k_sample_x0_full), hipFuncAttributeMaxDynamicSharedMemorySize, static_cast<int>(lds));
-    hipLaunchKernelGGL(k_sample_x0_full, dim3((B + SD_X0_FULL_ROWS - 1) / SD_X0_FULL_ROWS), dim3(256), lds, s, ds.loc, ds.aux, lo, hi, p0, B, d, out);
-  } else {
-    X0Dev q;
-    q.kind = ds.kind; q.loc = ds.loc; q.scale = ds.scale; q.p0 = ds.p0; q.p1 = ds.p1;
-    const long long n = static_cast<long long>(B) * ((d + 3) / 4);
-    hipLaunchKernelGGL(k_sample_x0, dim3(static_cast<unsigned>((n + 255) / 256)), dim3(256), 0, s, q, lo, hi, p0, B, d, out);
-  }
+int sd_launch_sample_x0_full(const sdeng_dist& ds, unsigned lo, unsigned hi, long long p0, int B, int d, float* out, hipStream_t s) {
+  const size_t lds = (static_cast<size_t>(SD_X0_FULL_ROWS) * (4 * ((d + 3) / 4) + 1) + static_cast<size_t>(d) * (d | 1)) * sizeof(float);
+  if (lds > 160 * 1024) return static_cast<int>(hipErrorInvalidValue);
+  if (lds > 64 * 1024) (void)hipFuncSetAttribute(reinterpret_cast<const void*>(k_sample_x0_full), hipFuncAttributeMaxDynamicSharedMemorySize, static_cast<int>(lds));
+  hipLaunchKernelGGL(k_sample_x0_full, dim3((B + SD_X0_FULL_ROWS - 1) / SD_X0_FULL_ROWS), dim3(256), lds, s, ds.loc, ds.aux, lo, hi, p0, B, d, out);
   return static_cast<int>(hipGetLastError());
 }
 
-int sd_launch_pack(const PackArgs& a, hipStream_t s) {
-  const int total = sd_lds_weight_floats(a.NT) * 2 + (a.transpose ? 0 : 3 * 64 + 16 * a.NT);
-  if (!a.transpose) hipLaunchKernelGGL(k_weight_scales, dim3(4), dim3(256), 0, s, a);
-  hipLaunchKernelGGL(k_pack_mlp, dim3((total + 255) / 256), dim3(256), 0, s, a);
-  return static_cast<int>(hipGetLastError());
-}
-int sd_launch_time_embed(const TimeEmbedArgs& a, int N, hipStream_t s) {
-  hipLaunchKernelGGL(k_time_embed, dim3(N), dim3(64), 0, s, a);
-  return static_cast<int>(hipGetLastError());
-}
-int sd_launch_ref_tables(const RefTabArgs& a, int N, hipStream_t s) {
-  hipLaunchKernelGGL(k_same_var, dim3(1), dim3(128), 0, s, a.vars, a.K, a.d, a.same_var);
-  hipLaunchKernelGGL(k_ref_tables, dim3(N * a.K), dim3(128), 0, s, a);
+__device__ inline void block_coords(int local, int KB, int& part, int& o, int& i) {
+  const int j = local & 7, lane = (local >> 3) & 63, blk = local >> 10;
+  part = (local >> 9) & 1;
+  const int kb = blk % KB, to = blk / KB;
+  o = 16 * to + (lane & 15);
+  i = 16 * (2 * kb + (j >> 2)) + 4 * (lane >> 4) + (j & 3);
+}
+__device__ inline _Float16 split_part(float w, int part) {
+  const _Float16 hi = static_cast<_Float16>(w);
+  return part == 0 ? hi : static_cast<_Float16>((w - static_cast<float>(hi)) * 2048.0f);
+}
+__device__ inline void role_logreg_images(const LogregImgArgs& a, int lb, int nb, int t) {
+  const int KB = sd_kb(a.NT), RKB = sd_lr_row_kb(a.n);
+  const int n_logit = sd_lr_logit_floats(a.NT, a.n) * 2, n_grad = sd_lr_grad_floats(a.NT, a.n) * 2;
+  _Float16* img = reinterpret_cast<_Float16*>(a.image);
+  for (int idx = lb * 256 + t; idx < n_logit + n_grad; idx += nb * 256) {
+    int part, o, i, row, col;
+    if (idx < n_logit) {
+      block_coords(idx, KB, part, o, i);
+      row = o; col = i;
+    } else {
+      block_coords(idx - n_logit, RKB, part, o, i);
+      row = i; col = o;
+    }
+    float v = 0.0f;
+    if (row < a.n) v = (col < a.dw) ? a.X[static_cast<size_t>(row) * a.dw + col] : (col == a.dw ? 1.0f : 0.0f);
+    img[idx] = split_part(v, part);
+    if (idx < 32 * RKB) a.y_pad[idx] = (idx < a.n) ? a.y[idx] : 0.0f;
+  }
+}
+__device__ inline void role_pack_square(const SquareArgs& a, int lb, int nb, int t) {
+  const int KB = sd_kb(a.NT), d = a.d;
+  _Float16* img = reinterpret_cast<_Float16*>(a.out);
+  for (int idx = lb * 256 + t; idx < a.NT * KB * 1024; idx += nb * 256) {
+    int part, o, i;
+    block_coords(idx, KB, part, o, i);
+    img[idx] = split_part((o < d && i < d) ? a.P[static_cast<size_t>(o) * d + i] : 0.0f, part);
+    if (idx < 16 * a.NT) a.loc_pad[idx] = idx < d ? a.loc[idx] : 0.0f;
+  }
+}
+
+__global__ void __launch_bounds__(SD_PREP_THREADS) k_prepare(const PrepJobs jobs) {
+  __shared__ float lds[1024];
+  int j = 0;
+  while (j + 1 < jobs.n && static_cast<int>(blockIdx.x) >= jobs.job[j + 1].first) ++j;
+  const PrepJob& jb = jobs.job[j];
+  const int pb = blockIdx.x - jb.first, tid = threadIdx.x, n = jb.count;
+  switch (jb.role) {
+    case SD_PREP_SCALES: role_weight_scales(jb.a.pack, pb, tid, lds); break;
+    case SD_PREP_SAME_VAR: role_same_var(jb.a.same); break;
+    case SD_PREP_DIST: {
+      const int lb = 2 * pb + (tid >> 7);
+      role_dist_tables(jb.a.dist, lb < n ? lb : 0, lb < n, tid & 127, lds + 256 * (tid >> 7));
+      break;
+    }
+    case SD_PREP_TIME_EMBED: {
+      const int lb = 4 * pb + (tid >> 6);
+      role_time_embed(jb.a.temb, lb < n ? lb : 0, lb < n, tid & 63, lds + 256 * (tid >> 6));
+      break;
+    }
+    case SD_PREP_PACK: role_pack(jb.a.pack, pb, tid, lds); break;
+    case SD_PREP_REF: {
+      const int lb = 2 * pb + (tid >> 7);
+      role_ref_tables(jb.a.ref, lb < n ? lb : 0, lb < n, tid & 127, lds + 128 * (tid >> 7));
+      break;
+    }
+    case SD_PREP_SQUARE: role_pack_square(jb.a.sq, pb, n, tid); break;
+    case SD_PREP_LOGREG: role_logreg_images(jb.a.lr, pb, n, tid); break;
+    case SD_PREP_X0: role_sample_x0(jb.a.x0, pb, tid); break;
+    default: break;
+  }
+}
+
+int sd_launch_prepare(const PrepJobs& jobs, hipStream_t s) {
+  if (jobs.n < 1) return 0;
+  const PrepJob& last = jobs.job[jobs.n - 1];
+  const int hosts = sd_prep_hosts(last.role);
+  hipLaunchKernelGGL(k_prepare, dim3(last.first + (last.count + hosts - 1) / hosts), dim3(SD_PREP_THREADS), 0, s, jobs);
   return static_cast<int>(hipGetLastError());
 }
 int sd_launch_ref_full_tables(const RefFullArgs& a, int N, hipStream_t s) {
@@ -975,12 +1055,10 @@
   return static_cast<int>(hipGetLastError());
 }
 int sd_launch_ref_mm_tables(const RefMMArgs& a, int N, hipStream_t s) {
-  hipLaunchKernelGGL(k_same_var, dim3(1), dim3(128), 0, s, a.vars, a.K, a.d, a.same_var);
+  SameVarArgs sv;
+  sv.vars = a.vars; sv.K = a.K; sv.d = a.d; sv.same_var = a.same_var;
+  hipLaunchKernelGGL(k_same_var, dim3(1), dim3(SD_PREP_THREADS), 0, s, sv);
   hipLaunchKernelGGL(k_ref_mm_tables, dim3(N), dim3(256), 0, s, a);
-  return static_cast<int>(hipGetLastError());
-}
-int sd_launch_dist_tables(const DistTabArgs& a, hipStream_t s) {
-  hipLaunchKernelGGL(k_dist_tables, dim3(a.K), dim3(128), 0, s, a);
   return static_cast<int>(hipGetLastError());
 }
 int sd_launch_dist_eval(const DistEvalArgs& a, hipStream_t s) {
diff --git a/sde_sampler_lrds_amd/csrc/prep_kernels.hpp b/sde_sampler_lrds_amd/csrc/prep_kernels.hpp
--- a/sde_sampler_lrds_amd/csrc/prep_kernels.hpp
+++ b/sde_sampler_lrds_amd/csrc/prep_kernels.hpp
@@ -9,7 +9,6 @@
   const float *w_in, *b_in, *w_h1, *b_h1, *w_h2, *b_h2, *w_out, *b_out;
   float* out;
   int transpose;
-  const float* scales;
 };
 
 struct TimeEmbedArgs {
@@ -90,14 +89,61 @@
   float* rnd;
 };
 
-int sd_launch_pack(const PackArgs& a, hipStream_t s);
-int sd_launch_time_embed(const TimeEmbedArgs& a, int N, hipStream_t s);
-int sd_launch_ref_tables(const RefTabArgs& a, int N, hipStream_t s);
+enum { SD_PREP_SCALES = 0, SD_PREP_SAME_VAR, SD_PREP_DIST, SD_PREP_TIME_EMBED, SD_PREP_PACK, SD_PREP_REF, SD_PREP_SQUARE, SD_PREP_LOGREG,
+       SD_PREP_X0, SD_PREP_ROLES };
+#define SD_PREP_THREADS 256
+#define SD_PREP_MAX_JOBS 12
+inline int sd_prep_hosts(int role) {
+  return role == SD_PREP_TIME_EMBED ? 4 : (role == SD_PREP_REF || role == SD_PREP_DIST) ? 2 : 1;
+}
+struct X0Args {
+  X0Dev q;
+  unsigned seed_lo, seed_hi;
+  long long particle0;
+  int B, d;
+  float* out;
+};
+struct LogregImgArgs {
+  const float *X, *y;
+  int n, dw, NT;
+  float *image, *y_pad;
+};
+struct SquareArgs {
+  const float *P, *loc;
+  int d, NT;
+  float *out, *loc_pad;
+};
+struct SameVarArgs {
+  const float* vars;
+  int K, d;
+  float* same_var;
+};
+union PrepArg {
+  PackArgs pack;
+  TimeEmbedArgs temb;
+  SameVarArgs same;
+  RefTabArgs ref;
+  DistTabArgs dist;
+  LogregImgArgs lr;
+  SquareArgs sq;
+  X0Args x0;
+};
+struct PrepJob {
+  int role, first, count;
+  PrepArg a;
+};
+struct PrepJobs {
+  int n;
+  PrepJob job[SD_PREP_MAX_JOBS];
+};
+static_assert(sizeof(PrepJobs) <= 4096, "the job table travels as kernel arguments");
+int sd_prep_pack_blocks(const PackArgs& a);
+int sd_launch_prepare(const PrepJobs& jobs, hipStream_t s);
+
 int sd_launch_ref_full_tables(const RefFullArgs& a, int N, hipStream_t s);
-int sd_launch_dist_tables(const DistTabArgs& a, hipStream_t s);
 int sd_launch_dist_eval(const DistEvalArgs& a, hipStream_t s);
 int sd_launch_terminal(const TerminalArgs& a, hipStream_t s);
 int sd_launch_logz(const float* rnd, long long B, float* stats, float* weights, float* scratch, hipStream_t s);
 int sd_launch_philox(unsigned lo, unsigned hi, int step, int n_steps, long long p0, int B, int d, unsigned stream_id, float* out, hipStream_t s);
-int sd_launch_sample_x0(const sdeng_dist& ds, unsigned lo, unsigned hi, long long p0, int B, int d, float* out, hipStream_t s);
+int sd_launch_sample_x0_full(const sdeng_dist& ds, unsigned lo, unsigned hi, long long p0, int B, int d, float* out, hipStream_t s);
 int sd_launch_ref_mm_tables(const RefMMArgs& a, int N, hipStream_t s);
diff --git a/sde_sampler_lrds_amd/csrc/sdeng_api.hip b/sde_sampler_lrds_amd/csrc/sdeng_api.hip
--- a/sde_sampler_lrds_amd/csrc/sdeng_api.hip
+++ b/sde_sampler_lrds_amd/csrc/sdeng_api.hip
@@ -15,9 +15,6 @@
 #include "cmcd_adjoint_kernel.hpp"
 #include "metric_kernels.hpp"
 #include "tilted_kernel.hpp"
-
-int sd_launch_logreg_images(const float* X, const float* y, int n, int dw, int NT, float* image, float* y_pad, hipStream_t s);
-int sd_launch_pack_square(const float* P, const float* loc, int d, int NT, float* out, float* loc_pad, hipStream_t s);
 
 static thread_local char g_err[512] = "";
 static int fail(int code, const char* fmt, ...) {
@@ -40,6 +37,54 @@
 
 extern "C" int sdeng_abi_version(void) { return SDENG_ABI_VERSION; }
 extern "C" const char* sdeng_last_error(void) { return g_err; }
+
+struct Prep {
+  hipStream_t s;
+  bool per_job;
+  PrepJobs jobs;
+  Prep(hipStream_t stream, bool one_by_one) : s(stream), per_job(one_by_one) {
+    jobs.n = 0;
+    const char* e = getenv("SDENG_PREP_PER_JOB");
+    if (e && e[0] == '1') per_job = true;
+  }
+  PrepJob& job(int role, int count) {
+    PrepJob& j = jobs.job[jobs.n];
+    memset(&j, 0, sizeof(j));
+    j.role = role; j.count = count;
+    return j;
+  }
+  int add() {
+    ++jobs.n;
+    return (per_job || jobs.n == SD_PREP_MAX_JOBS) ? flush() : 0;
+  }
+  int flush() {
+    if (jobs.n == 0) return 0;
+    PrepJobs out;
+    out.n = 0;
+    int first = 0;
+#ifdef SD_PREP_X0_OWN
+    for (int pass = 0; pass < 2; ++pass) {
+      if (pass == 1) { SD_HIP(sd_launch_prepare(out, s)); out.n = 0; first = 0; }
+      for (int role = 0; role < SD_PREP_ROLES; ++role) {
+        if ((role == SD_PREP_X0) != (pass == 1)) continue;
+#else
+    {
+      for (int role = 0; role < SD_PREP_ROLES; ++role) {
+#endif
+        for (int i = 0; i < jobs.n; ++i) {
+          if (jobs.job[i].role != role || jobs.job[i].count < 1) continue;
+          PrepJob& j = out.job[out.n++];
+          j = jobs.job[i];
+          j.first = first;
+          first += (j.count + sd_prep_hosts(role) - 1) / sd_prep_hosts(role);
+        }
+      }
+    }
+    jobs.n = 0;
+    SD_HIP(sd_launch_prepare(out, s));
+    return 0;
+  }
+};
 
 static inline size_t align64(size_t n_floats) { return (n_floats + 63) & ~static_cast<size_t>(63); }
 static inline int pad16(int d) { return 16 * ((d + 15) / 16); }
@@ -233,7 +278,7 @@
       return fail(SDENG_E_UNSUPPORTED, "unknown distribution kind %d", in.kind);
   }
 }
-static int build_dist(const sdeng_dist& in, int d, int dpad, float* ws, DistDev& out, hipStream_t s) {
+static int build_dist(const sdeng_dist& in, int d, int dpad, float* ws, DistDev& out, Prep& pj) {
   SD_TRY(check_dist(in, d));
   memset(&out, 0, sizeof(out));
   out.kind = in.kind;
@@ -243,13 +288,14 @@
   switch (in.kind) {
     case SDENG_DIST_GMM_DIAG:
     case SDENG_DIST_GAUSS_DIAG: {
-      DistTabArgs t;
+      const int K = in.kind == SDENG_DIST_GMM_DIAG ? in.k : 1;
+      DistTabArgs& t = pj.job(SD_PREP_DIST, K).a.dist;
       t.K = in.kind == SDENG_DIST_GMM_DIAG ? in.k : 1; t.d = d; t.dpad = dpad;
       t.loc = in.loc; t.scale = in.scale; t.weights = in.kind == SDENG_DIST_GMM_DIAG ? in.w : nullptr;
       t.tab = ws; t.consts = ws + align64(static_cast<size_t>(t.K) * 2 * dpad);
-      SD_HIP(sd_launch_dist_tables(t, s));
       out.k = t.K;
       out.tab = t.tab; out.consts = t.consts;
+      SD_TRY(pj.add());
       out.p0 = half_d_log_2pi(d);
       return 0;
     }
@@ -292,39 +338,45 @@
   }
   return 0;
 }
-static int pack_net(const sdeng_desc* d, int DT, float* out, float* out_t, hipStream_t s) {
+static int pack_net(const sdeng_desc* d, int DT, float* out, float* out_t, Prep& pj) {
   const sdeng_net& n = d->net;
   PackArgs pk;
   pk.NT = DT; pk.d = d->d;
   pk.w_in = n.w_in; pk.b_in = n.b_in; pk.w_h1 = n.w_h1; pk.b_h1 = n.b_h1; pk.w_h2 = n.w_h2; pk.b_h2 = n.b_h2; pk.w_out = n.w_out; pk.b_out = n.b_out;
-  pk.out = out; pk.transpose = 0; pk.scales = nullptr;
-  SD_HIP(sd_launch_pack(pk, s));
+  pk.out = out; pk.transpose = 0;
+  pj.job(SD_PREP_SCALES, 4).a.pack = pk;
+  SD_TRY(pj.add());
+  pj.job(SD_PREP_PACK, sd_prep_pack_blocks(pk)).a.pack = pk;
+  SD_TRY(pj.add());
   if (out_t) {
-    pk.out = out_t; pk.transpose = 1; pk.scales = out + sd_off_scales(DT);
-    SD_HIP(sd_launch_pack(pk, s));
+    pk.out = out_t; pk.transpose = 1;
+    pj.job(SD_PREP_PACK, sd_prep_pack_blocks(pk)).a.pack = pk;
+    SD_TRY(pj.add());
   }
   return 0;
 }
 static int embed_times(const sdeng_desc* d, int n_times, bool t_direct, float t_value, float* temb, float* stheta_ws, const float** stheta,
-                       hipStream_t s) {
+                       Prep& pj) {
   TimeEmbedArgs te;
   te.te = d->net.t_embed; te.coef = d->coef; te.col = 0; te.t_direct = t_direct; te.t_value = t_value; te.clip = 0.0f; te.out = temb;
-  SD_HIP(sd_launch_time_embed(te, n_times, s));
+  pj.job(SD_PREP_TIME_EMBED, n_times).a.temb = te;
+  SD_TRY(pj.add());
   *stheta = nullptr;
   if (d->net.ctrl_kind != SDENG_CTRL_CLIPPED && d->net.score_model.n_hidden > 0) {
     te.te = d->net.score_model;
     te.clip = d->net.clip_model;
     te.out = stheta_ws;
-    SD_HIP(sd_launch_time_embed(te, n_times, s));
+    pj.job(SD_PREP_TIME_EMBED, n_times).a.temb = te;
+    SD_TRY(pj.add());
     *stheta = stheta_ws;
   }
   return 0;
 }
-static int prepare_net(const sdeng_desc* d, const Layout& L, float* ws, int DT, SimArgs& a, hipStream_t s, int n_times, bool t_direct,
+static int prepare_net(const sdeng_desc* d, const Layout& L, float* ws, int DT, SimArgs& a, Prep& pj, int n_times, bool t_direct,
                        float t_value) {
-  SD_TRY(pack_net(d, DT, ws + L.wpack, nullptr, s));
+  SD_TRY(pack_net(d, DT, ws + L.wpack, nullptr, pj));
   a.wpack = ws + L.wpack;
-  if (n_times > 0) SD_TRY(embed_times(d, n_times, t_direct, t_value, ws + L.temb, ws + L.stheta, &a.stheta, s));
+  if (n_times > 0) SD_TRY(embed_times(d, n_times, t_direct, t_value, ws + L.temb, ws + L.stheta, &a.stheta, pj));
   a.temb = ws + L.temb;
   a.ctrl_kind = d->net.ctrl_kind;
   a.clip_model = d->net.clip_model;
@@ -342,12 +394,14 @@
   return check_lerp_prior(d);
 }
 
-static int prepare_logreg(const sdeng_desc* d, const Layout& L, float* ws, int DT, SimArgs& a, hipStream_t s, float** next) {
+static int prepare_logreg(const sdeng_desc* d, const Layout& L, float* ws, int DT, SimArgs& a, Prep& pj, float** next) {
   const int n = d->target.k;
   float* image = ws + L.cmcd;
   float* y_pad = image + align64(sd_lr_floats(DT, n));
   *next = y_pad + align64(32 * sd_lr_row_kb(n));
-  SD_HIP(sd_launch_logreg_images(d->target.loc, d->target.scale, n, d->d - 1, DT, image, y_pad, s));
+  LogregImgArgs& li = pj.job(SD_PREP_LOGREG, 96).a.lr;
+  li.X = d->target.loc; li.y = d->target.scale; li.n = n; li.dw = d->d - 1; li.NT = DT; li.image = image; li.y_pad = y_pad;
+  SD_TRY(pj.add());
   a.lr.image = image; a.lr.y_pad = y_pad; a.lr.n_rows = n;
   a.lr.in_lds = static_cast<size_t>(cmcd_lds_floats(DT, n)) * sizeof(float) <= 160 * 1024 ? 1 : 0;
   a.lr.inv_w_scale2 = 1.0f / (d->target.p0 * d->target.p0); a.lr.c_mean = d->target.p1; a.lr.inv_c_scale2 = 1.0f / (d->target.p2 * d->target.p2);
@@ -495,24 +549,28 @@
   return plan_sim(p);
 }
 
-static int run_cmcd(const SimPlan& p, const sdeng_desc* d, float* ws, SimArgs& a, hipStream_t s) {
+static int run_cmcd(const SimPlan& p, const sdeng_desc* d, float* ws, SimArgs& a, Prep& pj) {
+  hipStream_t s = pj.s;
   const Layout& L = p.L;
   const int DT = p.DT, dpad = 16 * DT;
-  SD_TRY(prepare_net(d, L, ws, DT, a, s, d->N + 1, false, 0.0f));
+  SD_TRY(prepare_net(d, L, ws, DT, a, pj, d->N + 1, false, 0.0f));
   DistDev target, prior;
-  SD_TRY(build_dist(d->target, d->d, dpad, ws + L.target, target, s));
-  SD_TRY(build_dist(d->prior, d->d, dpad, ws + L.prior, prior, s));
+  SD_TRY(build_dist(d->target, d->d, dpad, ws + L.target, target, pj));
+  SD_TRY(build_dist(d->prior, d->d, dpad, ws + L.prior, prior, pj));
   CmcdArgs c;
   memset(&c, 0, sizeof(c));
   float* prec = ws + L.cmcd;
-  if (d->target.kind == SDENG_DIST_LOGREG) SD_TRY(prepare_logreg(d, L, ws, DT, a, s, &prec));
+  if (d->target.kind == SDENG_DIST_LOGREG) SD_TRY(prepare_logreg(d, L, ws, DT, a, pj, &prec));
   float* locp = prec + align64(DT * sd_kb(DT) * 512);
   if (d->prior.kind == SDENG_DIST_GAUSS_FULL) {
-    SD_HIP(sd_launch_pack_square(d->prior.scale, d->prior.loc, d->d, DT, prec, locp, s));
+    SquareArgs& sq = pj.job(SD_PREP_SQUARE, DT * sd_kb(DT) * 4).a.sq;
+    sq.P = d->prior.scale; sq.loc = d->prior.loc; sq.d = d->d; sq.NT = DT; sq.out = prec; sq.loc_pad = locp;
+    SD_TRY(pj.add());
     c.prec_pack = prec; c.prior_loc = locp;
   } else if (d->prior.kind == SDENG_DIST_ISO_GAUSS) {
     c.iso_loc = d->prior.p0; c.inv_iso_var = 1.0f / d->prior.p3;
   }
+  SD_TRY(pj.flush());
   const bool eubo = d->form == SDENG_FORM_CMCD_EUBO;
   if (eubo) {
     SD_HIP(hipMemsetAsync(ws + L.rnd_init, 0, sizeof(float) * d->B, s));
@@ -529,13 +587,23 @@
   return terminal(d, dpad, target, target, false, true, d->x_out, d->rnd_out, s);
 }
 
-static int run_euler(const SimPlan& p, const sdeng_desc* d, float* ws, SimArgs& a, hipStream_t s) {
-  SD_TRY(build_dist(d->target, d->d, 16 * p.DT, ws + p.L.target, a.target, s));
+static int run_euler(const SimPlan& p, const sdeng_desc* d, float* ws, SimArgs& a, Prep& pj) {
+  SD_TRY(build_dist(d->target, d->d, 16 * p.DT, ws + p.L.target, a.target, pj));
+  SD_TRY(pj.flush());
   a.clip_score = d->net.clip_score;
-  return launch_timed(d, p.k, &a, s);
-}
-
-static int prepare_ref(const SimPlan& p, const sdeng_desc* d, float* ws, SimArgs& a, hipStream_t s) {
+  return launch_timed(d, p.k, &a, pj.s);
+}
+
+static int add_ref_tables(const RefTabArgs& r, int N, Prep& pj) {
+  SameVarArgs& sv = pj.job(SD_PREP_SAME_VAR, 1).a.same;
+  sv.vars = r.vars; sv.K = r.K; sv.d = r.d; sv.same_var = r.same_var;
+  SD_TRY(pj.add());
+  pj.job(SD_PREP_REF, N * r.K).a.ref = r;
+  return pj.add();
+}
+
+static int prepare_ref(const SimPlan& p, const sdeng_desc* d, float* ws, SimArgs& a, Prep& pj) {
+  hipStream_t s = pj.s;
   const Layout& L = p.L;
   const int DT = p.DT, dpad = 16 * DT, K = ref_components(d), rf = p.rf;
   if (rf == RF_NONE) return 0;
@@ -577,7 +645,7 @@
     r.tab = ws + L.ref_tab; r.consts = ws + L.ref_consts;
     r.same_var = ws + L.ref_consts + static_cast<size_t>(d->N) * K * 2;
     r.centred = (rf == RF_GMM && p.k.fam != SD_FAM_SPLIT) ? 1 : 0;
-    SD_HIP(sd_launch_ref_tables(r, d->N, s));
+    SD_TRY(add_ref_tables(r, d->N, pj));
   }
   a.ref_same_var = ws + L.ref_consts + static_cast<size_t>(d->N) * K * 2;
   if (rf == RF_GMM_BIG) {
@@ -595,17 +663,23 @@
   return 0;
 }
 
-static int run_sim(const SimPlan& p, const sdeng_desc* d, float* ws, SimArgs& a, hipStream_t s) {
+static int run_sim(const SimPlan& p, const sdeng_desc* d, float* ws, SimArgs& a, Prep& pj) {
+  hipStream_t s = pj.s;
   const Layout& L = p.L;
   const int DT = p.DT, dpad = 16 * DT;
-  SD_TRY(prepare_net(d, L, ws, DT, a, s, d->N, false, 0.0f));
-  SD_TRY(prepare_ref(p, d, ws, a, s));
+  SD_TRY(prepare_net(d, L, ws, DT, a, pj, d->N, false, 0.0f));
+  SD_TRY(prepare_ref(p, d, ws, a, pj));
   DistDev target, ref_dist, prior;
-  SD_TRY(build_dist(d->target, d->d, dpad, ws + L.target, target, s));
-  SD_TRY(build_dist(d->ref_dist, d->d, dpad, ws + L.ref_dist, ref_dist, s));
-  SD_TRY(build_dist(d->prior, d->d, dpad, ws + L.prior, prior, s));
+  SD_TRY(build_dist(d->target, d->d, dpad, ws + L.target, target, pj));
+  SD_TRY(build_dist(d->ref_dist, d->d, dpad, ws + L.ref_dist, ref_dist, pj));
+  SD_TRY(build_dist(d->prior, d->d, dpad, ws + L.prior, prior, pj));
   a.target = target;
   a.prior = prior;
+  if (p.sc == SC_LOGREG) {
+    float* unused;
+    SD_TRY(prepare_logreg(d, L, ws, DT, a, pj, &unused));
+  }
+  SD_TRY(pj.flush());
   const bool eubo = d->form == SDENG_FORM_EUBO;
   const bool tr = d->flags & SDENG_FLAG_TERM_REF, tt = d->flags & SDENG_FLAG_TERM_TARGET;
   if ((d->flags & SDENG_FLAG_INIT_LOGP) && !eubo) {
@@ -617,14 +691,22 @@
     SD_TRY(terminal(d, dpad, ref_dist, target, tr, tt, d->x_in, ws + L.rnd_init, s));
     a.rnd_init = ws + L.rnd_init;
   }
-  if (p.sc == SC_LOGREG) {
-    float* unused;
-    SD_TRY(prepare_logreg(d, L, ws, DT, a, s, &unused));
-  }
   SD_TRY(launch_timed(d, p.k, &a, s));
   if (!eubo && (tr || tt)) SD_TRY(terminal(d, dpad, ref_dist, target, tr, tt, d->x_out, d->rnd_out, s));
   if (eubo && (d->flags & SDENG_FLAG_INIT_LOGP)) SD_TRY(terminal(d, dpad, prior, prior, true, false, d->x_out, d->rnd_out, s));
   return 0;
+}
+
+static int add_x0(const sdeng_dist& ds, const Seed& seed, long long p0, int B, int d, float* out, Prep& pj) {
+  if (ds.kind == SDENG_DIST_GAUSS_FULL) {
+    SD_HIP(sd_launch_sample_x0_full(ds, seed.lo, seed.hi, p0, B, d, out, pj.s));
+    return 0;
+  }
+  const long long n = static_cast<long long>(B) * ((d + 3) / 4);
+  X0Args& x = pj.job(SD_PREP_X0, static_cast<int>((n + 255) / 256)).a.x0;
+  x.q.kind = ds.kind; x.q.loc = ds.loc; x.q.scale = ds.scale; x.q.p0 = ds.p0; x.q.p1 = ds.p1;
+  x.seed_lo = seed.lo; x.seed_hi = seed.hi; x.particle0 = p0; x.B = B; x.d = d; x.out = out;
+  return pj.add();
 }
 
 extern "C" int sdeng_simulate(const sdeng_desc* desc, void* stream) {
@@ -647,18 +729,19 @@
   a.xs_out = d->xs_out; a.noise_in = d->noise_in;
   a.trash = ws + p.L.trash;
   a.ntiles = (d->B + 15) / 16;
+  Prep pj(s, false);
   sdeng_desc dm;
   if (!d->x_in) {
     float* x0 = d->x0_out ? d->x0_out : ws + p.L.x0;
-    SD_HIP(sd_launch_sample_x0(d->x0_dist, seed.lo, seed.hi, d->particle0, d->B, d->d, x0, s));
+    SD_TRY(add_x0(d->x0_dist, seed, d->particle0, d->B, d->d, x0, pj));
     dm = *d;
     dm.x_in = x0;
     d = &dm;
     a.x_in = x0;
   }
-  if (p.k.fam == SD_FAM_CMCD) return run_cmcd(p, d, ws, a, s);
-  if (p.k.fam == SD_FAM_EULER) return run_euler(p, d, ws, a, s);
-  return run_sim(p, d, ws, a, s);
+  if (p.k.fam == SD_FAM_CMCD) return run_cmcd(p, d, ws, a, pj);
+  if (p.k.fam == SD_FAM_EULER) return run_euler(p, d, ws, a, pj);
+  return run_sim(p, d, ws, a, pj);
 }
 
 extern "C" int sdeng_sample_x0(const sdeng_dist* dist, uint64_t seed, int64_t particle0, int32_t B, int32_t d, float* out, void* stream) {
@@ -669,8 +752,9 @@
   tmp.x0_dist = *dist;
   SD_TRY(check_x0_dist(&tmp));
   const Seed sd = split_seed(seed);
-  SD_HIP(sd_launch_sample_x0(*dist, sd.lo, sd.hi, particle0, B, d, out, static_cast<hipStream_t>(stream)));
-  return 0;
+  Prep pj(static_cast<hipStream_t>(stream), true);
+  SD_TRY(add_x0(*dist, sd, particle0, B, d, out, pj));
+  return pj.flush();
 }
 
 extern "C" int sdeng_ctrl_forward(const sdeng_desc* d, float t_net, float score_gain, float lerp_w, const float* x, float* u_out,
@@ -698,9 +782,11 @@
   a.x_in = x; a.x_out = u_out;
   a.trash = ws + L.trash;
   a.ntiles = (d->B + 15) / 16;
-  SD_TRY(prepare_net(d, L, ws, DT, a, s, 1, true, t_net));
-  SD_TRY(build_dist(d->target, d->d, dpad, ws + L.target, a.target, s));
-  SD_TRY(build_dist(d->prior, d->d, dpad, ws + L.prior, a.prior, s));
+  Prep pj(s, false);
+  SD_TRY(prepare_net(d, L, ws, DT, a, pj, 1, true, t_net));
+  SD_TRY(build_dist(d->target, d->d, dpad, ws + L.target, a.target, pj));
+  SD_TRY(build_dist(d->prior, d->d, dpad, ws + L.prior, a.prior, pj));
+  SD_TRY(pj.flush());
   float host_coef[SDENG_NCOEF] = {0};
   host_coef[0] = t_net; host_coef[7] = score_gain; host_coef[8] = lerp_w;
   float* dev_coef = ws + L.logz;
@@ -728,12 +814,12 @@
 }
 struct VjpOut { float *a0, *a1, *a2, *d0, *d1, *d2, *dout; };
 static int prepare_vjp(const sdeng_desc* d, int DT, const VjpLayout& V, size_t total, bool pack, int n_times, int rows_per_time, const float* x,
-                       const VjpOut& o, size_t stheta_off, const float** stheta, VjpArgs& v, hipStream_t s) {
+                       const VjpOut& o, size_t stheta_off, const float** stheta, VjpArgs& v, Prep& pj) {
   const size_t need = total * sizeof(float);
   if (!d->workspace || d->workspace_bytes < need) return fail(SDENG_E_WORKSPACE, "workspace %zu bytes, need %zu", d->workspace_bytes, need);
   float* ws = static_cast<float*>(d->workspace);
-  if (pack) SD_TRY(pack_net(d, DT, ws, ws + V.wt, s));
-  SD_TRY(embed_times(d, n_times, false, 0.0f, ws + V.temb, ws + stheta_off, stheta, s));
+  if (pack) SD_TRY(pack_net(d, DT, ws, ws + V.wt, pj));
+  SD_TRY(embed_times(d, n_times, false, 0.0f, ws + V.temb, ws + stheta_off, stheta, pj));
   v.M = n_times * rows_per_time; v.B = rows_per_time; v.d = d->d; v.N = n_times;
   v.x = x; v.wpack = ws; v.wpack_t = ws + V.wt; v.temb = ws + V.temb;
   v.clip_model = d->net.clip_model;
@@ -757,10 +843,12 @@
   KernelKey k;
   SD_TRY(select_kernel(k, SD_FAM_VJP, DT, gx ? 1 : 0));
   const VjpLayout V = vjp_layout(DT, n_times);
+  Prep pj(s, false);
   VjpArgs a;
   memset(&a, 0, sizeof(a));
   const float* no_stheta;
-  SD_TRY(prepare_vjp(d, DT, V, V.total, !(d->flags & SDENG_FLAG_REUSE_PACK), n_times, rows_per_time, x, {a0, a1, a2, d0, d1, d2, dout}, 0, &no_stheta, a, s));
+  SD_TRY(prepare_vjp(d, DT, V, V.total, !(d->flags & SDENG_FLAG_REUSE_PACK), n_times, rows_per_time, x, {a0, a1, a2, d0, d1, d2, dout}, 0, &no_stheta, a, pj));
+  SD_TRY(pj.flush());
   a.cot = cot; a.gx = gx; a.u_out = u_out;
   a.ntiles = static_cast<int>((M + 15) / 16);
   SD_HIP(k.fn(&a, s));
@@ -823,8 +911,9 @@
   const AdjLayout A = adjoint_layout(d, DT);
   AdjArgs a;
   memset(&a, 0, sizeof(a));
+  Prep pj(s, false);
   SD_TRY(prepare_vjp(d, DT, A.v, A.total, true, d->N, d->B, adj->xs, {adj->a0, adj->a1, adj->a2, adj->d0, adj->d1, adj->d2, adj->dout}, A.stheta, &a.stheta,
-                     a.v, s));
+                     a.v, pj));
   float* ws = static_cast<float*>(d->workspace);
   if (d->ref.kind != SDENG_REF_NONE) {
     const int K = ref_components(d);
@@ -834,14 +923,14 @@
     r.tab = ws + A.tab; r.consts = ws + A.consts;
     r.same_var = ws + A.consts + static_cast<size_t>(d->N) * K * 2;
     r.centred = 0;
-    SD_HIP(sd_launch_ref_tables(r, d->N, s));
+    SD_TRY(add_ref_tables(r, d->N, pj));
     a.ref_tab = ws + A.tab; a.ref_consts = ws + A.consts; a.ref_k = K;
     a.ref_c1 = half_d_log_2pi(d->d);
   }
   a.has_score = has_score;
   if (score) {
     a.score_ext = adj->score;
-    if (!adj->score) SD_TRY(build_dist(d->target, d->d, dpad, ws + A.target, a.target, s));
+    if (!adj->score) SD_TRY(build_dist(d->target, d->d, dpad, ws + A.target, a.target, pj));
     a.scale_score = d->net.scale_score; a.clip_score = d->net.clip_score;
     a.ctrl_kind = d->net.ctrl_kind;
     a.prior_loc = d->prior.p0; a.prior_scale = d->net.ctrl_kind == SDENG_CTRL_LERP ? d->prior.p1 : 1.0f;
@@ -851,6 +940,7 @@
   a.coef = d->coef; a.noise = ito ? adj->noise : nullptr; a.w = adj->w; a.lam_in = adj->lam_in; a.lam_out = adj->lam_out;
   a.lin = d->form == SDENG_FORM_LIN ? 1 : 0;
   a.ntiles_b = (d->B + 15) / 16;
+  SD_TRY(pj.flush());
   SD_HIP(k.fn(&a, s));
   return 0;
 }
@@ -923,13 +1013,14 @@
   const CmcdAdjLayout A = cmcd_adjoint_layout(d, DT);
   CmcdAdjArgs a;
   memset(&a, 0, sizeof(a));
+  Prep pj(s, false);
   SD_TRY(prepare_vjp(d, DT, A.v, A.total, true, d->N + 1, d->B, adj->xs, {adj->a0, adj->a1, adj->a2, adj->d0, adj->d1, adj->d2, adj->dout}, A.stheta,
-                     &a.stheta, a.v, s));
+                     &a.stheta, a.v, pj));
   float* ws = static_cast<float*>(d->workspace);
-  if (tgt != CADJ_EXT) SD_TRY(build_dist(d->target, d->d, dpad, ws + A.target, a.target, s));
+  if (tgt != CADJ_EXT) SD_TRY(build_dist(d->target, d->d, dpad, ws + A.target, a.target, pj));
   if (d->prior.kind == SDENG_DIST_GAUSS_DIAG) {
     DistDev prior;
-    SD_TRY(build_dist(d->prior, d->d, dpad, ws + A.prior, prior, s));
+    SD_TRY(build_dist(d->prior, d->d, dpad, ws + A.prior, prior, pj));
     a.prior_tab = prior.tab;
   } else {
     a.iso_loc = d->prior.p0; a.inv_iso_var = 1.0f / d->prior.p3;
@@ -945,6 +1036,7 @@
   a.coef = d->coef; a.cbar = adj->cbar; a.w = adj->w; a.lam_in = adj->lam_in; a.lam_out = adj->lam_out;
   a.steps = d->N;
   a.ntiles_b = (d->B + 15) / 16;
+  SD_TRY(pj.flush());
   SD_HIP(k.fn(&a, s));
   return 0;
 }
@@ -959,7 +1051,9 @@
   const size_t need = dist_floats(*dist, dpad) * sizeof(float);
   if (need > 0 && (!workspace || workspace_bytes < need)) return fail(SDENG_E_WORKSPACE, "workspace %zu bytes, need %zu", workspace_bytes, need);
   DistDev dd;
-  SD_TRY(build_dist(*dist, d, dpad, static_cast<float*>(workspace), dd, s));
+  Prep pj(s, false);
+  SD_TRY(build_dist(*dist, d, dpad, static_cast<float*>(workspace), dd, pj));
+  SD_TRY(pj.flush());
   return dist_eval(dd, B, d, dpad, x, logp_out, score_out, s);
 }
 
@@ -992,16 +1086,18 @@
   float* ws = static_cast<float*>(workspace);
   MovesArgs a;
   memset(&a, 0, sizeof(a));
-  SD_TRY(build_dist(*target, d, dpad, ws, a.target.ds, s));
+  Prep pj(s, false);
+  SD_TRY(build_dist(*target, d, dpad, ws, a.target.ds, pj));
   a.target.d = d; a.target.dpad = dpad; a.target.B = B;
   a.prior.ds.kind = SDENG_DIST_NONE;
-  if (has_prior) SD_TRY(build_dist(*prior, d, dpad, ws + dist_floats(*target, dpad), a.prior.ds, s));
+  if (has_prior) SD_TRY(build_dist(*prior, d, dpad, ws + dist_floats(*target, dpad), a.prior.ds, pj));
   a.prior.d = d; a.prior.dpad = dpad; a.prior.B = B;
   a.B = B; a.d = d; a.K = n_moves; a.keep_from = keep_from; a.ula = unadjusted ? 1 : 0; a.target_acc = target_acceptance;
   a.t = t; a.x = x; a.lp = lp; a.grad = grad; a.step = step; a.z = z; a.u = u;
   const Seed sd = split_seed(seed);
   a.seed_lo = sd.lo; a.seed_hi = sd.hi; a.chain0 = chain0;
   a.samples = samples; a.acc_sum = acc_sum; a.acc_last = acc_last;
+  SD_TRY(pj.flush());
   SD_HIP(sd_launch_moves(a, move, s));
   return 0;
 }
```
